# junejunejune/c_orb_slam

Measured on AMD Instinct MI355X. Metric: tracking FPS + ORB matches/sec, KITTI-00 stereo; local-BA iter/sec, higher is better.
Workload: dtype u8

## Files before the change

### c_orb_slam_amd/csrc/ba.hpp

```cpp
#pragma once
#include <functional>
#include <hip/hip_runtime.h>

#include <cstdint>
#include <future>
#include <vector>

#include "../../include/orbslam_gpu.h"
#include "ba_struct.hpp"
#include "ba_struct_gpu.hpp"
#include "ba_types.hpp"
#include "comm.hpp"
#include "ldlt.hpp"
#include "orb_common.hpp"

namespace orbgpu {

constexpr int kBaTiledMinPoses = 24;

struct Se3 {
    double q[4];
    double t[3];
    double pad;
};
// ... 16 lines not shown
    double ni, currentChi, iniChi;
    double trialChi[kLmTrials], trialLam[kLmTrials], solveIni[kLmSolves], solveChi[kLmSolves];
};

struct LinArgs;

class BaEngine {
public:
    ~BaEngine();
    int init();
    int run(const ba_problem* P, const volatile bool* stop, ba_result* R, Comm* comm = nullptr,
            const BaMode* mode = nullptr);
    const BaTrace& trace() const { return trace_; }
    double last_ms[4] = {0, 0, 0, 0};
    int last_dist[4] = {0, 0, 0, 0};
    int last_lm[4] = {0, 0, 0, 0};
    bool edgesGrouped = false;
    bool edgesValidated = false;

private:
    int upload_problem(const ba_problem* P);
    int build_structure(int level);
    int gather_blocks(const std::vector<int64_t>& mine, std::vector<int64_t>* all);
    int optimize(int iterations, const volatile bool* stop, int* its);
    int lm_solve(int iteration, const volatile bool* stop, bool* terminate);
    bool device_lm(int iterations) const;
    int optimize_device(int iterations, const volatile bool* stop, int* its);
    void enqueue_lm_step(bool first);
    int enqueue_lm_step_comm(bool first);
    int allreduce_tiles(int n);
    void launch_scale(double lam, int use_dev, int own, const int* gate);
    void launch_trial_errors(const LinArgs& sys, const int* gate);
    DensePlan dense_;
    bool small_struct() const;
    bool host_lists() const;
    bool smallUp_ = false;
    int32_t *dKp_ = nullptr, *dPtOrd_ = nullptr;
    int32_t* dSmKid_ = nullptr;
    uint8_t* dSmFx_ = nullptr;
    char* dSmallIn_ = nullptr;
    bool deferredUpload_ = false;
    std::vector<char> deferArgs_;
    size_t deferBytes_ = 0;
    int issue_upload();
    double* dLmStage_ = nullptr;
    size_t lmStageCap_ = 0;
    int gate_edges(int final_check, uint8_t* erase);
    int carve(bool commit, size_t* total);
    bool stopped(const volatile bool* stop) const { return comm_ ? stopRed_ : (stop && *stop); }
    int reduce_stop(const volatile bool* stop);
    bool sharded() const { return comm_ && comm_->size() > 1; }
    bool dense_solver(int n) const;

    hipStream_t stream_ = nullptr;
    int nkf_ = 0, npt_ = 0, ne_ = 0;
    Se3 *dT_ = nullptr, *dTbak_ = nullptr;
    double *dX_ = nullptr, *dXbak_ = nullptr;
    EdgeDev* dE_ = nullptr;
    uint8_t *dLevel_ = nullptr, *dRobust_ = nullptr;
    double* dErr_ = nullptr;
    std::vector<int32_t> kfId_, ptId_;
    const int32_t* ePt_ = nullptr;
    const int32_t* eKf_ = nullptr;
    std::vector<uint8_t> kfFixed_, kfLocal_, level_, ptHasEdge_, kfHasEdge_;
    BaStructDev st_{};
    BaHostStruct hs_;
    GpuStructBuilder gs_;
    uint8_t* dKfFixed_ = nullptr;
    int32_t *dKfId_ = nullptr, *dPtId_ = nullptr;
    int32_t* dStruct_ = nullptr;
    size_t dStructCap_ = 0;
    double *dTerms_ = nullptr, *dRc_ = nullptr, *dHpp_ = nullptr, *dBp_ = nullptr, *dHll_ = nullptr, *dBl_ = nullptr;
    double *dB_ = nullptr, *dX2_ = nullptr, *dS_ = nullptr, *dBs_ = nullptr, *dDinv_ = nullptr, *dDb_ = nullptr;
    double *dEmat_ = nullptr, *dCb_ = nullptr, *dScal_ = nullptr, *dScratch_ = nullptr, *dHplA_ = nullptr;
    int32_t* dPePos_ = nullptr;
    Se3* dTn_ = nullptr;
    double* dXn_ = nullptr;
    std::vector<int32_t> hPePos_;
    int blkChunks_ = 1;
    double *tmpA0_ = nullptr, *tmpA1_ = nullptr, *tmpB0_ = nullptr, *tmpB1_ = nullptr;
    unsigned* dCounter_ = nullptr;
    SparseLdlt sp_;
    std::future<int> spEarly_;
    int spEarlyNP_ = -1;
    std::vector<int64_t> spEarlyKeys_;
    int start_early_pose_graph();
    std::future<int> spBuild_;
    int join_sp_build();
    bool tiled_ = false;
    bool distOk_ = false;
    void* arena_ = nullptr;
    size_t arenaCap_ = 0;
    double* hScal_ = nullptr;
    LmDev* dLm_ = nullptr;
    int* hLm_ = nullptr;
    hipEvent_t lmEv_[2] = {nullptr, nullptr};
    void* hStage_ = nullptr;
    size_t hStageCap_ = 0;
    bool uploadPending_ = false;
    void* hStage2_ = nullptr;
    size_t hStage2Cap_ = 0;
    bool stage2Pending_ = false;
    int stage2_reserve(size_t bytes);
    int h2d_sync(void* dst, const void* src, size_t bytes);
    int d2h_sync(void* dst, const void* src, size_t bytes);
    int d2h_poll(void* dst, const void* src, size_t bytes);
    int poll_stream();
    BaHostStruct hs2_;
    bool hsValid_ = false, refineNext_ = false;
    int signalSeq_ = 0;
    int stage_reserve(size_t bytes);
    size_t scratchN_ = 0;
    size_t ldsMax_ = 0;
    Comm* comm_ = nullptr;
    bool stopRed_ = false;
    int nEglob_ = 0, nLglob_ = 0;
    int nTiles_ = 0;
    void* dPack_ = nullptr;
    size_t packCap_ = 0;
    int2* dTiles_ = nullptr;
    double* dPackBuf_ = nullptr;
    BaMode mode_{};
    double lambda_ = 0, ni_ = 2;
    int nBad_ = 0;
    BaTrace trace_;
};

struct PoseEdgeDev;
struct PoseProbDev;

struct PoseProbDev;
class PoseEngine {
public:
    ~PoseEngine();
    int init();
    int run(int count, const pose_problem* P, float* Tcw_out, uint8_t* const* outlier, int* ninliers);
    int run_device(int count, const pose_problem* P, float* const* Tcw_out, uint8_t* const* outlier, int* ninliers);
    int run_frames_device(int count, const pose_frame* F, float* const* Tcw_out, uint8_t* const* outlier,
                          int* ninliers, hipStream_t s = nullptr, DeferredChain* chain = nullptr);
    hipStream_t stream() const { return stream_; }
    void set_timing(bool on) { timing_ = on; }
    int last_timing(float* ms);

private:
    int launch_device(int count, const int* Ns, const std::function<void(int, PoseProbDev&)>& fill,
                      float* const* Tcw_out, uint8_t* const* outlier, int* ninliers, hipStream_t s = nullptr,
                      DeferredChain* chain = nullptr);
    hipStream_t stream_ = nullptr;
    void* dArena_ = nullptr;
    void* hArena_ = nullptr;
    size_t cap_ = 0;
    hipEvent_t lastUse_ = nullptr;
    bool lastUseSet_ = false;
    bool timing_ = false, timed_ = false;
    hipEvent_t tA_ = nullptr, tB_ = nullptr;
};

int debug_ldlt(int n, const double* S, const double* b, double* x, int variant);
int debug_csum(const double* v, int n, double* out);
int debug_ldlt_factor(int n, const double* S, double* out);
int debug_wave_tree(const double* v64, double* out);
int debug_shared_div(const double* a, const double* b, int n, double* out);
int debug_set_csum_lds_max(int v);
int debug_set_scale_small_max(int v);
int debug_set_struct_gpu_min_edges(int v);
int debug_set_posegraph_check(int on);
int debug_prof(unsigned long long* out32);

}
```

### c_orb_slam_amd/csrc/capi_match.cpp

```cpp
#include <cstring>
#include <new>
#include <vector>

#include "capi_handles.hpp"

using orbgpu::FrameDev;
using orbgpu::Matcher;
using orbgpu::SearchDev;


namespace {

size_t al(size_t n) { return (n + 255) & ~(size_t)255; }

template <class T>
T* up(Matcher* m, const T* src, size_t count, hipStream_t s, int* err) {
    if (!src || count == 0) return nullptr;
    void* d = m->arena_alloc(count * sizeof(T));
    if (!d || hipMemcpyAsync(d, src, count * sizeof(T), hipMemcpyHostToDevice, s) != hipSuccess) {
        *err = ORB_E_HIP;
        return nullptr;
    }
    return (T*)d;
}

size_t frame_bytes(const orb_frame* f) {
    if (!f) return 0;
    return al((size_t)f->N * 28) + al((size_t)f->N * 32) + (f->uRight ? al((size_t)f->N * 4) : 0) +
           al((size_t)f->nlevels * 4) + al(64);
}

FrameDev frame_dev(Matcher* m, const orb_frame* f, bool dev, hipStream_t s, int* err) {
    FrameDev d;
    memset(&d, 0, sizeof(d));
    if (!f) return d;
    d.N = f->N;
    d.minX = f->minX; d.maxX = f->maxX; d.minY = f->minY; d.maxY = f->maxY;
    d.gridWInv = f->gridWInv; d.gridHInv = f->gridHInv;
    d.nlevels = f->nlevels;
    d.fx = f->fx; d.fy = f->fy; d.cx = f->cx; d.cy = f->cy; d.bf = f->bf; d.b = f->b;
    if (dev) {
        d.keysUn = (const orbgpu::orb_kp_dev*)f->keysUn;
        d.desc = f->desc;
        d.uRight = f->uRight;
        d.scale = f->scaleFactors;
        d.Tcw = f->Tcw;
    } else {
        d.keysUn = (const orbgpu::orb_kp_dev*)up(m, f->keysUn, (size_t)f->N, s, err);
        d.desc = up(m, f->desc, (size_t)f->N * 32, s, err);
        d.uRight = up(m, f->uRight, f->uRight ? (size_t)f->N : 0, s, err);
        d.scale = up(m, f->scaleFactors, (size_t)f->nlevels, s, err);
        d.Tcw = up(m, f->Tcw, 16, s, err);
    }
    return d;
}

bool frame_ok(const orb_frame* f) {
    return f && f->N >= 0 && f->N <= orbgpu::kMaxFrameKeys && (f->N == 0 || (f->keysUn && f->desc)) &&
           f->scaleFactors && f->Tcw && f->nlevels > 0;
}

}

extern "C" {

int ORBmatcher_create(float nnratio, int checkOri, ORBmatcher_h* out) {
    if (!out) return ORB_E_INVALID;
    *out = nullptr;
    auto* m = new (std::nothrow) Matcher(nnratio, checkOri != 0);
    if (!m) return ORB_E_INVALID;
    int rc = m->init_device();
    if (rc) {
        delete m;
        return rc == -4 ? ORB_E_NODEVICE : ORB_E_HIP;
    }
    *out = new ORBmatcher_t{m};
    return ORB_OK;
}

int ORBmatcher_destroy(ORBmatcher_h h) {
    if (!h) return ORB_E_INVALID;
    delete h->m;
    delete h;
    return ORB_OK;
}

int ORBmatcher_set_device_pointers(ORBmatcher_h h, int on) {
    if (!h) return ORB_E_INVALID;
    h->m->set_device_pointers(on != 0);
    return ORB_OK;
}

void* ORBmatcher_stream(ORBmatcher_h h) { return h ? (void*)h->m->stream() : nullptr; }

int ORBmatcher_enable_timing(ORBmatcher_h h, int on) {
    if (!h) return ORB_E_INVALID;
    return h->m->set_timing(on != 0) ? ORB_E_HIP : ORB_OK;
}

int ORBmatcher_set_deferred(ORBmatcher_h h, int on) {
    if (!h || !h->m->device_pointers()) return ORB_E_INVALID;
    if (!on && h->m->chain().on() && h->m->chain().finish(h->m->stream())) return ORB_E_HIP;
    h->m->chain().set(on != 0);
    return ORB_OK;
}

int ORBmatcher_finish(ORBmatcher_h h) {
    if (!h) return ORB_E_INVALID;
    return h->m->chain().finish(h->m->stream()) ? ORB_E_HIP : ORB_OK;
}

int ORBmatcher_chain_close(ORBmatcher_h h, long long* epoch) {
    if (!h || !epoch || !h->m->chain().on()) return ORB_E_INVALID;
    return h->m->chain().close(h->m->stream(), epoch) ? ORB_E_HIP : ORB_OK;
}

int ORBmatcher_chain_wait(ORBmatcher_h h, long long epoch) {
    if (!h) return ORB_E_INVALID;
    return h->m->chain().wait(epoch) ? ORB_E_HIP : ORB_OK;
}

int ORBmatcher_chain_finish(ORBmatcher_h h, long long epoch) {
    if (!h) return ORB_E_INVALID;
    return h->m->chain().finish_upto(epoch) ? ORB_E_HIP : ORB_OK;
}

int ORBmatcher_last_timings(ORBmatcher_h h, float* ms8, long long* counts8) {
    if (!h || !ms8 || !counts8) return ORB_E_INVALID;
    return h->m->timings(ms8, counts8) ? ORB_E_HIP : ORB_OK;
}

int ORBmatcher_DescriptorDistance(const uint8_t* a, const uint8_t* b) {
    if (!a || !b) return ORB_E_INVALID;
    int dist = 0;
    for (int i = 0; i < 8; i++) {
        uint32_t pa, pb;
        memcpy(&pa, a + 4 * i, 4);
        memcpy(&pb, b + 4 * i, 4);
        dist += __builtin_popcount(pa ^ pb);
    }
    return dist;
}

int ORBmatcher_SearchByProjection_LastFrame_batch(ORBmatcher_h h, int npairs, const orb_frame* cur,
                                                  int32_t* const* cur_mp, const orb_frame* last,
                                                  const orb_kp* const* last_keys, const int32_t* const* last_mp,
                                                  const uint8_t* const* last_outlier, const orb_mappoints* mps,
                                                  float th, int bMono, int* nmatches) {
    if (!h || npairs < 0 || !cur || !cur_mp || !last || !last_keys || !last_mp || !last_outlier || !mps || !nmatches)
        return ORB_E_INVALID;
    Matcher* m = h->m;
    const bool dev = m->device_pointers();
    hipStream_t s = m->stream();
    for (int p = 0; p < npairs; p++) {
        if (!frame_ok(&cur[p]) || !last[p].Tcw || last[p].N < 0 || (last[p].N > 0 && !last[p].keysUn)) return ORB_E_INVALID;
        if (last[p].N > 0 && (!last_keys[p] || !last_mp[p] || !last_outlier[p])) return ORB_E_INVALID;
        if (mps[p].n > 0 && (!mps[p].pos || !mps[p].desc || !mps[p].observations)) return ORB_E_INVALID;
        if (!dev) {
            for (int i = 0; i < last[p].N; i++)
                if (last_mp[p][i] >= mps[p].n) return ORB_E_INVALID;
            for (int i = 0; i < cur[p].N; i++)
                if (cur_mp[p][i] >= mps[p].n) return ORB_E_INVALID;
        }
    }
    int err = 0;
    std::vector<SearchDev> probs(npairs);
    if (!dev) {
        size_t need = 0;
        for (int p = 0; p < npairs; p++) {
            const int nl = last[p].N;
            need += frame_bytes(&cur[p]) + al((size_t)nl * 28) * 2 + al(64) + al((size_t)nl * 4) + al((size_t)nl) +
                    al((size_t)mps[p].n * 12) + al((size_t)mps[p].n * 32) + al((size_t)mps[p].n * 4) +
                    al((size_t)cur[p].N * 4) + al(4);
        }
        if (m->arena_reserve(need + (size_t)npairs * 4 + 4096)) return ORB_E_HIP;
    }
    if (dev && m->arena_reserve((size_t)npairs * 4 + 256)) return ORB_E_HIP;
    int* d_nm = nullptr;
    std::vector<int*> nm_dev(npairs, nullptr);
    for (int p = 0; p < npairs; p++) {
        SearchDev& P = probs[p];
        memset(&P, 0, sizeof(P));
        P.cur = frame_dev(m, &cur[p], dev, s, &err);
        const int nl = last[p].N;
        P.nq = nl;
        P.last.N = nl;
        if (dev) {
            P.last.keysUn = (const orbgpu::orb_kp_dev*)last[p].keysUn;
            P.last.Tcw = last[p].Tcw;
            P.lastKeys = (const orbgpu::orb_kp_dev*)last_keys[p];
            P.lastMP = last_mp[p];
            P.lastOutlier = last_outlier[p];
            P.mpPos = mps[p].pos;
            P.mpDesc = mps[p].desc;
            P.mpObs = mps[p].observations;
            P.curMP = cur_mp[p];
        } else {
            P.last.keysUn = (const orbgpu::orb_kp_dev*)up(m, last[p].keysUn, (size_t)nl, s, &err);
            P.last.Tcw = up(m, last[p].Tcw, 16, s, &err);
            P.lastKeys = (const orbgpu::orb_kp_dev*)up(m, last_keys[p], (size_t)nl, s, &err);
            P.lastMP = up(m, last_mp[p], (size_t)nl, s, &err);
            P.lastOutlier = up(m, last_outlier[p], (size_t)nl, s, &err);
            P.mpPos = up(m, mps[p].pos, (size_t)mps[p].n * 3, s, &err);
            P.mpDesc = up(m, mps[p].desc, (size_t)mps[p].n * 32, s, &err);
            P.mpObs = up(m, mps[p].observations, (size_t)mps[p].n, s, &err);
            P.curMP = (int*)m->arena_alloc((size_t)cur[p].N * 4 + 4);
            if (cur[p].N > 0 && hipMemcpyAsync(P.curMP, cur_mp[p], (size_t)cur[p].N * 4, hipMemcpyHostToDevice, s) != hipSuccess)
                err = ORB_E_HIP;
        }
        nm_dev[p] = nullptr;
    }
    if (err) return err;
    {
        void* d = dev ? m->count_buf((size_t)npairs * 4 + 4) : m->arena_alloc((size_t)npairs * 4 + 4);
        if (!d) return ORB_E_HIP;
        d_nm = (int*)d;
        for (int p = 0; p < npairs; p++) probs[p].nmatches = d_nm + p;
    }
    int rc = m->search_last(probs, th, bMono != 0);
    if (rc) return rc == -1 ? ORB_E_INVALID : ORB_E_HIP;
    if (dev) {
        if (m->d2h_counts(nmatches, d_nm, (size_t)npairs * 4)) return ORB_E_HIP;
        return m->end_call() ? ORB_E_HIP : ORB_OK;
    }
    if (hipMemcpyAsync(nmatches, d_nm, (size_t)npairs * 4, hipMemcpyDeviceToHost, s) != hipSuccess) return ORB_E_HIP;
    {
        for (int p = 0; p < npairs; p++)
            if (cur[p].N > 0 &&
                hipMemcpyAsync(cur_mp[p], probs[p].curMP, (size_t)cur[p].N * 4, hipMemcpyDeviceToHost, s) != hipSuccess)
                return ORB_E_HIP;
    }
    if (orbgpu::stream_wait(s) != hipSuccess) return ORB_E_HIP;
    return ORB_OK;
}

int ORBmatcher_SearchByProjection_LastFrame(ORBmatcher_h h, const orb_frame* cur, int32_t* cur_mp,
                                            const orb_frame* last, const orb_kp* last_keys, const int32_t* last_mp,
                                            const uint8_t* last_outlier, const orb_mappoints* mps, float th, int bMono,
                                            int* nmatches) {
    return ORBmatcher_SearchByProjection_LastFrame_batch(h, 1, cur, &cur_mp, last, &last_keys, &last_mp, &last_outlier,
                                                         mps, th, bMono, nmatches);
}

int ORBmatcher_SearchByProjection_MapPoints(ORBmatcher_h h, const orb_frame* F, int32_t* cur_mp, int n,
                                            const uint8_t* track_in_view, const float* proj_x, const float* proj_xr,
                                            const float* proj_y, const int32_t* level, const float* view_cos,
                                            const int32_t* mp_index, const orb_mappoints* mps, float th,
                                            int* nmatches) {
    if (!h || !frame_ok(F) || !cur_mp || n < 0 || !mps || !nmatches) return ORB_E_INVALID;
    if (n > 0 && (!track_in_view || !proj_x || !proj_xr || !proj_y || !level || !view_cos || !mp_index))
        return ORB_E_INVALID;
    Matcher* m = h->m;
    const bool dev = m->device_pointers();
    hipStream_t s = m->stream();
    if (!dev) {
        for (int j = 0; j < n; j++)
            if (track_in_view[j] && (mp_index[j] < 0 || mp_index[j] >= mps->n || level[j] < 0 || level[j] >= F->nlevels))
                return ORB_E_INVALID;
        for (int i = 0; i < F->N; i++)
            if (cur_mp[i] >= mps->n) return ORB_E_INVALID;
        size_t need = frame_bytes(F) + al((size_t)n) + 4 * al((size_t)n * 4) + al((size_t)n * 4) * 2 +
                      al((size_t)mps->n * 12) + al((size_t)mps->n * 32) + al((size_t)mps->n * 4) +
                      al((size_t)F->N * 4) + al(8);
        if (m->arena_reserve(need + 4096)) return ORB_E_HIP;
    } else {
        if (m->arena_reserve(4096)) return ORB_E_HIP;
    }
    int err = 0;
    std::vector<SearchDev> probs(1);
    SearchDev& P = probs[0];
    memset(&P, 0, sizeof(P));
    P.cur = frame_dev(m, F, dev, s, &err);
    P.nq = n;
    if (dev) {
        P.inView = track_in_view; P.projX = proj_x; P.projXR = proj_xr; P.projY = proj_y;
        P.level = level; P.viewCos = view_cos; P.mpIndex = mp_index;
        P.mpPos = mps->pos; P.mpDesc = mps->desc; P.mpObs = mps->observations;
        P.curMP = cur_mp;
    } else {
        P.inView = up(m, track_in_view, (size_t)n, s, &err);
        P.projX = up(m, proj_x, (size_t)n, s, &err);
        P.projXR = up(m, proj_xr, (size_t)n, s, &err);
        P.projY = up(m, proj_y, (size_t)n, s, &err);
        P.level = up(m, level, (size_t)n, s, &err);
        P.viewCos = up(m, view_cos, (size_t)n, s, &err);
        P.mpIndex = up(m, mp_index, (size_t)n, s, &err);
        P.mpPos = up(m, mps->pos, (size_t)mps->n * 3, s, &err);
        P.mpDesc = up(m, mps->desc, (size_t)mps->n * 32, s, &err);
        P.mpObs = up(m, mps->observations, (size_t)mps->n, s, &err);
        P.curMP = (int*)m->arena_alloc((size_t)F->N * 4 + 4);
        if (F->N > 0 && hipMemcpyAsync(P.curMP, cur_mp, (size_t)F->N * 4, hipMemcpyHostToDevice, s) != hipSuccess)
            err = ORB_E_HIP;
    }
    if (err) return err;
    int* d_nm = (int*)m->arena_alloc(8);
    P.nmatches = d_nm;
    int rc = m->search_local(probs, th);
    if (rc) return rc == -1 ? ORB_E_INVALID : ORB_E_HIP;
    if (hipMemcpyAsync(nmatches, d_nm, 4, hipMemcpyDeviceToHost, s) != hipSuccess) return ORB_E_HIP;
    if (!dev && F->N > 0 && hipMemcpyAsync(cur_mp, P.curMP, (size_t)F->N * 4, hipMemcpyDeviceToHost, s) != hipSuccess)
        return ORB_E_HIP;
    if (orbgpu::stream_wait(s) != hipSuccess) return ORB_E_HIP;
    return ORB_OK;
}

int Frame_isInFrustum_batch(ORBmatcher_h h, int count, const orb_frame* F, const orb_localmap* maps,
                            float viewingCosLimit, float logScaleFactor, uint8_t* const* in_view,
                            float* const* proj_x, float* const* proj_xr, float* const* proj_y, int32_t* const* level,
                            float* const* view_cos, int* nvisible) {
    if (!h || count < 0 || (count > 0 && (!F || !maps || !in_view || !proj_x || !proj_xr || !proj_y || !level ||
                                          !view_cos || !nvisible)))
        return ORB_E_INVALID;
    if (count == 0) return ORB_OK;
    Matcher* m = h->m;
    if (!m->device_pointers()) return ORB_E_INVALID;
    hipStream_t s = m->stream();
    size_t need = al((size_t)count * 4) + al(sizeof(orbgpu::FrustumDev) * count) + 4096;
    for (int p = 0; p < count; p++) {
        const orb_localmap& M = maps[p];
        if (!frame_ok(&F[p]) || !F[p].Tcw || M.n < 0) return ORB_E_INVALID;
        if (M.n > 0 && (!M.pos || !M.max_dist || !M.min_dist || !M.normal || !M.skip || !in_view[p] || !proj_x[p] ||
                        !proj_xr[p] || !proj_y[p] || !level[p] || !view_cos[p]))
            return ORB_E_INVALID;
        need += al((size_t)M.n * 4);
    }
    if (m->arena_reserve(need)) return ORB_E_HIP;
    int err = 0;
    int* d_nv = (int*)m->arena_alloc((size_t)count * 4);
    if (!d_nv || hipMemsetAsync(d_nv, 0, (size_t)count * 4, s) != hipSuccess) return ORB_E_HIP;
    std::vector<SearchDev> probs(count);
    std::vector<orbgpu::FrustumDev> fr(count);
    for (int p = 0; p < count; p++) {
        SearchDev& P = probs[p];
        memset(&P, 0, sizeof(P));
        P.cur = frame_dev(m, &F[p], true, s, &err);
        P.nq = maps[p].n;
        P.mpPos = maps[p].pos;
        orbgpu::FrustumDev& f = fr[p];
        f.maxDist = maps[p].max_dist;
        f.minDist = maps[p].min_dist;
        f.normal = maps[p].normal;
        f.skip = maps[p].skip;
        f.inView = in_view[p];
        f.projX = proj_x[p];
        f.projXR = proj_xr[p];
        f.projY = proj_y[p];
        f.level = level[p];
        f.viewCos = view_cos[p];
        f.mpIndex = (int*)m->arena_alloc((size_t)std::max(maps[p].n, 1) * 4);
        f.nvisible = d_nv + p;
        if (!f.mpIndex) return ORB_E_HIP;
    }
    if (err) return err;
    if (m->frustum(probs, fr, viewingCosLimit, logScaleFactor)) return ORB_E_HIP;
    if (hipMemcpyAsync(nvisible, d_nv, (size_t)count * 4, hipMemcpyDeviceToHost, s) != hipSuccess) return ORB_E_HIP;
    return orbgpu::stream_wait(s) == hipSuccess ? ORB_OK : ORB_E_HIP;
}

int ORBmatcher_SearchLocalPoints_batch(ORBmatcher_h h, int count, const orb_frame* F, int32_t* const* cur_mp,
                                       const orb_localmap* maps, float logScaleFactor, float th, float nnratio,
                                       int* nmatches, int* nvisible) {
    if (!h || count < 0 || (count > 0 && (!F || !cur_mp || !maps || !nmatches || !nvisible))) return ORB_E_INVALID;
    if (count == 0) return ORB_OK;
    Matcher* m = h->m;
    if (!m->device_pointers()) return ORB_E_INVALID;
    hipStream_t s = m->stream();
    size_t need = al((size_t)count * 8) + al(sizeof(orbgpu::FrustumDev) * count) + 4096;
    for (int p = 0; p < count; p++) {
        const orb_localmap& M = maps[p];
        if (!frame_ok(&F[p]) || !F[p].Tcw || M.n < 0 || !cur_mp[p]) return ORB_E_INVALID;
        if (M.n > 0 && (!M.pos || !M.desc || !M.observations || !M.max_dist || !M.min_dist || !M.normal || !M.skip))
            return ORB_E_INVALID;
        need += 7 * al((size_t)M.n * 4) + 256;
    }
    if (m->arena_reserve(need)) return ORB_E_HIP;
    int err = 0;
    int* d_cnt = (int*)m->count_buf((size_t)count * 8);
    if (!d_cnt) return ORB_E_HIP;
    if (hipMemsetAsync(d_cnt, 0, (size_t)count * 8, s) != hipSuccess) return ORB_E_HIP;
    std::vector<SearchDev> probs(count);
    std::vector<orbgpu::FrustumDev> fr(count);
    for (int p = 0; p < count; p++) {
        SearchDev& P = probs[p];
        memset(&P, 0, sizeof(P));
        P.cur = frame_dev(m, &F[p], true, s, &err);
        P.nq = maps[p].n;
        P.mpPos = maps[p].pos;
        P.mpDesc = maps[p].desc;
        P.mpObs = maps[p].observations;
        P.curMP = cur_mp[p];
        P.nmatches = d_cnt + p;
        orbgpu::FrustumDev& f = fr[p];
        memset(&f, 0, sizeof(f));
        f.maxDist = maps[p].max_dist;
        f.minDist = maps[p].min_dist;
        f.normal = maps[p].normal;
        f.skip = maps[p].skip;
        f.nvisible = d_cnt + count + p;
    }
    if (err) return err;
    const int rc = m->search_local_points(probs, fr, 0.5f, logScaleFactor, th, nnratio > 0.f ? nnratio : m->nnratio());
    if (rc) return rc == -1 ? ORB_E_INVALID : ORB_E_HIP;
    if (m->d2h_counts(nmatches, d_cnt, (size_t)count * 4) || m->d2h_counts(nvisible, d_cnt + count, (size_t)count * 4))
        return ORB_E_HIP;
    (void)s;
    return m->end_call() ? ORB_E_HIP : ORB_OK;
}

int ORBmatcher_SearchDense_batch(ORBmatcher_h h, int count, const uint8_t* const* qdesc, const int* nq,
                                 const uint8_t* const* tdesc, const int* nt, int32_t* const* best_idx,
                                 int32_t* const* best_dist, int32_t* const* second_dist) {
    if (!h || count < 0 || (count > 0 && (!qdesc || !nq || !tdesc || !nt || !best_idx || !best_dist || !second_dist)))
        return ORB_E_INVALID;
    for (int p = 0; p < count; p++) {
        if (nq[p] < 0 || nt[p] < 0) return ORB_E_INVALID;
        if (nq[p] > 0 && (!qdesc[p] || !best_idx[p] || !best_dist[p] || !second_dist[p])) return ORB_E_INVALID;
        if (nt[p] > 0 && !tdesc[p]) return ORB_E_INVALID;
    }
    if (count == 0) return ORB_OK;
    Matcher* m = h->m;
    const bool dev = m->device_pointers();
    hipStream_t s = m->stream();
    std::vector<orbgpu::DenseDev> probs;
    if (!dev) {
        size_t need = 4096;
        for (int p = 0; p < count; p++) need += al((size_t)nq[p] * 32) + al((size_t)nt[p] * 32) + 3 * al((size_t)nq[p] * 4);
        if (m->arena_reserve(need)) return ORB_E_HIP;
    }
    int err = 0;
    for (int p = 0; p < count; p++) {
        if (nq[p] == 0) continue;
        orbgpu::DenseDev d;
        d.nq = nq[p];
        d.nt = nt[p];
        if (dev) {
            d.q = qdesc[p];
            d.t = tdesc[p];
            d.best_idx = best_idx[p];
            d.best_dist = best_dist[p];
            d.second_dist = second_dist[p];
        } else {
            d.q = up(m, qdesc[p], (size_t)nq[p] * 32, s, &err);
            d.t = nt[p] ? up(m, tdesc[p], (size_t)nt[p] * 32, s, &err) : nullptr;
            d.best_idx = (int*)m->arena_alloc((size_t)nq[p] * 4);
            d.best_dist = (int*)m->arena_alloc((size_t)nq[p] * 4);
            d.second_dist = (int*)m->arena_alloc((size_t)nq[p] * 4);
            if (!d.best_idx || !d.best_dist || !d.second_dist) err = ORB_E_HIP;
        }
        probs.push_back(d);
    }
    if (err) return err;
    if (m->dense(probs)) return ORB_E_HIP;
    if (dev) return m->end_call() ? ORB_E_HIP : ORB_OK;
    for (int p = 0, k = 0; p < count; p++) {
        if (nq[p] == 0) continue;
        const orbgpu::DenseDev& d = probs[k++];
        if (hipMemcpyAsync(best_idx[p], d.best_idx, (size_t)nq[p] * 4, hipMemcpyDeviceToHost, s) != hipSuccess ||
            hipMemcpyAsync(best_dist[p], d.best_dist, (size_t)nq[p] * 4, hipMemcpyDeviceToHost, s) != hipSuccess ||
            hipMemcpyAsync(second_dist[p], d.second_dist, (size_t)nq[p] * 4, hipMemcpyDeviceToHost, s) != hipSuccess)
            return ORB_E_HIP;
    }
    return orbgpu::stream_wait(s) == hipSuccess ? ORB_OK : ORB_E_HIP;
}

int ORBmatcher_last_dense_timing(ORBmatcher_h h, float* ms, long long* pairs) {
    if (!h || !ms || !pairs) return ORB_E_INVALID;
    return h->m->dense_timing(ms, pairs) ? ORB_E_HIP : ORB_OK;
}

int ORBmatcher_SearchCandidates(ORBmatcher_h h, const uint8_t* qdesc, int nq, const uint8_t* tdesc, int nt,
                                const int32_t* off, const int32_t* cand, int32_t* dist, int32_t* best_idx,
                                int32_t* best_dist, int32_t* second_dist) {
    if (!h || nq < 0 || nt < 0 || !off) return ORB_E_INVALID;
    if (nq == 0) return ORB_OK;
    if (!qdesc || !best_idx || !best_dist || !second_dist) return ORB_E_INVALID;
    Matcher* m = h->m;
    const bool dev = m->device_pointers();
    hipStream_t s = m->stream();
    if (dev) {
        int rc = m->candidates(qdesc, nq, tdesc, nt, off, cand, dist, best_idx, best_dist, second_dist);
        if (rc) return ORB_E_HIP;
        return orbgpu::stream_wait(s) == hipSuccess ? ORB_OK : ORB_E_HIP;
    }
    const int ncand = off[nq];
    if (off[0] != 0 || ncand < 0) return ORB_E_INVALID;
    for (int q = 0; q < nq; q++)
        if (off[q + 1] < off[q]) return ORB_E_INVALID;
    for (int k = 0; k < ncand; k++)
        if (cand[k] < 0 || cand[k] >= nt) return ORB_E_INVALID;
    size_t need = al((size_t)nq * 32) + al((size_t)nt * 32) + al((size_t)(nq + 1) * 4) + 2 * al((size_t)ncand * 4 + 4) +
                  3 * al((size_t)nq * 4);
    if (m->arena_reserve(need + 4096)) return ORB_E_HIP;
    int err = 0;
    const uint8_t* dq = up(m, qdesc, (size_t)nq * 32, s, &err);
    const uint8_t* dt = up(m, tdesc, (size_t)nt * 32, s, &err);
    const int* doff = up(m, off, (size_t)nq + 1, s, &err);
    const int* dc = up(m, cand, (size_t)ncand, s, &err);
    int* dd = (int*)m->arena_alloc((size_t)ncand * 4 + 4);
    int* dbi = (int*)m->arena_alloc((size_t)nq * 4);
    int* dbd = (int*)m->arena_alloc((size_t)nq * 4);
    int* dsd = (int*)m->arena_alloc((size_t)nq * 4);
    if (err || !dd || !dbi || !dbd || !dsd) return ORB_E_HIP;
    if (m->candidates(dq, nq, dt, nt, doff, dc, dd, dbi, dbd, dsd)) return ORB_E_HIP;
    if (dist && ncand > 0 && hipMemcpyAsync(dist, dd, (size_t)ncand * 4, hipMemcpyDeviceToHost, s) != hipSuccess)
        return ORB_E_HIP;
    if (hipMemcpyAsync(best_idx, dbi, (size_t)nq * 4, hipMemcpyDeviceToHost, s) != hipSuccess ||
        hipMemcpyAsync(best_dist, dbd, (size_t)nq * 4, hipMemcpyDeviceToHost, s) != hipSuccess ||
        hipMemcpyAsync(second_dist, dsd, (size_t)nq * 4, hipMemcpyDeviceToHost, s) != hipSuccess)
        return ORB_E_HIP;
    return orbgpu::stream_wait(s) == hipSuccess ? ORB_OK : ORB_E_HIP;
}

}
```

### c_orb_slam_amd/csrc/capi_stereo.cpp

```cpp
#include <algorithm>
#include <cmath>
#include <cstring>
#include <vector>

#include "capi_handles.hpp"
#include "stereo.hpp"

namespace {
size_t al(size_t n) { return (n + 255) & ~(size_t)255; }

template <class T>
T* up(orbgpu::Matcher* m, const T* src, size_t count, hipStream_t s, int* err) {
    if (!src || count == 0) return nullptr;
    void* d = m->arena_alloc(count * sizeof(T));
    if (!d || hipMemcpyAsync(d, src, count * sizeof(T), hipMemcpyHostToDevice, s) != hipSuccess) {
        *err = ORB_E_HIP;
        return nullptr;
    }
    return (T*)d;
}
}

extern "C" {

int ORBmatcher_ComputeStereoMatches_batch(ORBmatcher_h h, ORBextractor_h left, ORBextractor_h right, int npairs,
                                          const int* NL, const orb_kp* const* keysL, const uint8_t* const* descL,
                                          const int* NR, const orb_kp* const* keysR,
                                          const uint8_t* const* descR, float mbf, float mb,
                                          float* const* uRight, float* const* depth, int* nmatches) {
    return ORBmatcher_ComputeStereoMatches_batch_at(h, left, 0, right, 0, npairs, NL, keysL, descL, NR, keysR, descR,
                                                    mbf, mb, uRight, depth, nmatches);
}

int ORBmatcher_ComputeStereoMatches_batch_at(ORBmatcher_h h, ORBextractor_h left, int first_left,
                                             ORBextractor_h right, int first_right, int npairs, const int* NL,
                                             const orb_kp* const* keysL, const uint8_t* const* descL, const int* NR,
                                             const orb_kp* const* keysR, const uint8_t* const* descR, float mbf,
                                             float mb, float* const* uRight, float* const* depth, int* nmatches) {
    if (!h || !left || !right || npairs < 0 || first_left < 0 || first_right < 0 || !NL || !keysL || !descL || !NR ||
        !keysR || !descR || !uRight || !depth || !nmatches)
        return ORB_E_INVALID;
    if (npairs == 0) return ORB_OK;
    const orbgpu::Extractor* EL = left->ex;
    const orbgpu::Extractor* ER = right->ex;
    if (!EL->pyramid_base() || !ER->pyramid_base() || first_left + npairs > EL->last_batch() ||
        first_right + npairs > ER->last_batch())
        return ORB_E_INVALID;
    const auto& LL = EL->levels();
    const auto& LR = ER->levels();
    if (LL.size() != LR.size() || (int)LL.size() > orbgpu::kStereoMaxLevels) return ORB_E_INVALID;
    for (size_t l = 0; l < LL.size(); l++)
        if (LL[l].w != LR[l].w || LL[l].h != LR[l].h || LL[l].pitch != LR[l].pitch || LL[l].off != LR[l].off)
            return ORB_E_INVALID;
    if (!(mb > 0.0f)) return ORB_E_INVALID;
    for (int p = 0; p < npairs; p++) {
        if (NL[p] < 0 || NR[p] < 0 || NL[p] > orbgpu::kStereoMaxKeys || NR[p] > 65535) return ORB_E_INVALID;
        if ((NL[p] && (!keysL[p] || !descL[p] || !uRight[p] || !depth[p])) || (NR[p] && (!keysR[p] || !descR[p])))
            return ORB_E_INVALID;
    }
    orbgpu::Matcher* m = h->m;
    const bool dev = m->device_pointers();
    hipStream_t s = m->stream();
    if (orbgpu::stream_wait(EL->stream()) != hipSuccess ||
        (ER != EL && orbgpu::stream_wait(ER->stream()) != hipSuccess))
        return ORB_E_HIP;
    orbgpu::StereoParams P;
    std::memset(&P, 0, sizeof(P));
    for (size_t l = 0; l < LL.size(); l++) {
        P.lv[l].off = (long long)LL[l].off;
        P.lv[l].pitch = LL[l].pitch;
        P.lv[l].w = LL[l].w;
        P.lv[l].h = LL[l].h;
        P.scale[l] = EL->scale()[l];
        P.invScale[l] = EL->inv_scale()[l];
    }
    P.mbf = mbf;
    P.mb = mb;
    P.rows0 = LL[0].h;
    if (P.rows0 > orbgpu::kStereoMaxRows) return ORB_E_INVALID;
    const int band = (int)std::ceil(4.0f * EL->scale()[LL.size() - 1]) + 3;
    size_t need = al(sizeof(orbgpu::StereoDev) * npairs) + al(4 * (size_t)npairs);
    int maxNL = 0;
    for (int p = 0; p < npairs; p++) {
        need += al(4 * (size_t)NL[p]) + al(4 * ((size_t)P.rows0 + 1)) + al(8 * (size_t)NR[p] * band + 8);
        if (!dev) need += al(28 * (size_t)NL[p]) + al(32 * (size_t)NL[p]) + al(28 * (size_t)NR[p]) +
                          al(32 * (size_t)NR[p]) + 2 * al(4 * (size_t)NL[p]);
        maxNL = std::max(maxNL, NL[p]);
    }
    if (m->arena_reserve(need + 4096)) return ORB_E_HIP;
    int err = 0;
    std::vector<orbgpu::StereoDev> probs(npairs);
    int* d_kept = (int*)(dev ? m->count_buf(4 * (size_t)npairs) : m->arena_alloc(4 * (size_t)npairs));
    for (int p = 0; p < npairs; p++) {
        orbgpu::StereoDev& S = probs[p];
        S.NL = NL[p];
        S.NR = NR[p];
        S.pyrL = EL->pyramid_base() + (size_t)(first_left + p) * EL->pyramid_image_bytes();
        S.pyrR = ER->pyramid_base() + (size_t)(first_right + p) * ER->pyramid_image_bytes();
        S.sad = (int*)m->arena_alloc(4 * (size_t)NL[p] + 4);
        S.rowStart = (int*)m->arena_alloc(4 * ((size_t)P.rows0 + 1));
        S.rowIdx = (int2*)m->arena_alloc(8 * (size_t)NR[p] * band + 8);
        if (!S.sad || !S.rowStart || !S.rowIdx) return ORB_E_HIP;
        S.kept = d_kept + p;
        if (dev) {
            S.kL = (const orbgpu::orb_kp_dev*)keysL[p];
            S.dL = descL[p];
            S.kR = (const orbgpu::orb_kp_dev*)keysR[p];
            S.dR = descR[p];
            S.uRight = uRight[p];
            S.depth = depth[p];
        } else {
            S.kL = (const orbgpu::orb_kp_dev*)up(m, keysL[p], (size_t)NL[p], s, &err);
            S.dL = up(m, descL[p], 32 * (size_t)NL[p], s, &err);
            S.kR = (const orbgpu::orb_kp_dev*)up(m, keysR[p], (size_t)NR[p], s, &err);
            S.dR = up(m, descR[p], 32 * (size_t)NR[p], s, &err);
            S.uRight = (float*)m->arena_alloc(4 * (size_t)NL[p] + 4);
            S.depth = (float*)m->arena_alloc(4 * (size_t)NL[p] + 4);
        }
    }
    if (err || !d_kept) return ORB_E_HIP;
    auto* d_probs = (orbgpu::StereoDev*)m->arena_alloc(sizeof(orbgpu::StereoDev) * npairs);
    if (!d_probs) return ORB_E_HIP;
    if (hipMemcpyAsync(d_probs, m->h2d_src(probs.data(), sizeof(orbgpu::StereoDev) * npairs),
                       sizeof(orbgpu::StereoDev) * npairs, hipMemcpyHostToDevice, s) != hipSuccess)
        return ORB_E_HIP;
    if (orbgpu::stereo_launch(d_probs, npairs, maxNL, P, s, m)) return ORB_E_HIP;
    if (dev) {
        if (m->d2h_counts(nmatches, d_kept, 4 * (size_t)npairs)) return ORB_E_HIP;
        return m->end_call() ? ORB_E_HIP : ORB_OK;
    }
    if (hipMemcpyAsync(nmatches, d_kept, 4 * (size_t)npairs, hipMemcpyDeviceToHost, s) != hipSuccess)
        return ORB_E_HIP;
    if (!dev)
        for (int p = 0; p < npairs; p++)
            if (NL[p] && (hipMemcpyAsync(uRight[p], probs[p].uRight, 4 * (size_t)NL[p], hipMemcpyDeviceToHost, s) !=
                              hipSuccess ||
                          hipMemcpyAsync(depth[p], probs[p].depth, 4 * (size_t)NL[p], hipMemcpyDeviceToHost, s) !=
                              hipSuccess))
                return ORB_E_HIP;
    return orbgpu::stream_wait(s) == hipSuccess ? ORB_OK : ORB_E_HIP;
}

int ORBmatcher_ComputeStereoMatches(ORBmatcher_h h, ORBextractor_h left, ORBextractor_h right, int index, int NL,
                                    const orb_kp* keysL, const uint8_t* descL, int NR, const orb_kp* keysR,
                                    const uint8_t* descR, float mbf, float mb, float* uRight, float* depth,
                                    int* nmatches) {
    if (!h || !left || !right || index < 0) return ORB_E_INVALID;
    if (index != 0) return ORB_E_INVALID;
    return ORBmatcher_ComputeStereoMatches_batch(h, left, right, 1, &NL, &keysL, &descL, &NR, &keysR, &descR, mbf,
                                                 mb, &uRight, &depth, nmatches);
}

int Frame_UnprojectStereo_batch_device(ORBmatcher_h h, int count, const orb_unproject* U) {
    if (!h || count < 0 || (count > 0 && !U)) return ORB_E_INVALID;
    if (count == 0) return ORB_OK;
    std::vector<orbgpu::UnprojDev> P((size_t)count);
    int maxN = 0;
    for (int f = 0; f < count; f++) {
        const orb_unproject& Q = U[f];
        if (Q.N < 0 || (Q.N > 0 && (!Q.keysUn || !Q.depth || !Q.Twc || !Q.x3D))) return ORB_E_INVALID;
        orbgpu::UnprojDev& d = P[f];
        d.N = Q.N;
        d.keys = (const orbgpu::orb_kp_dev*)Q.keysUn;
        d.depth = Q.depth;
        d.Twc = Q.Twc;
        d.fx = Q.fx; d.fy = Q.fy; d.cx = Q.cx; d.cy = Q.cy;
        d.invfx = 1.0f / Q.fx;
        d.invfy = 1.0f / Q.fy;
        d.x3D = Q.x3D;
        d.mp = Q.mp;
        maxN = std::max(maxN, Q.N);
    }
    (void)maxN;
    return orbgpu::unproject_batch(P.data(), count, h->m->stream()) ? ORB_E_HIP : ORB_OK;
}

static int fill_undist(const orb_undistort& q, orbgpu::UndistDev& d) {
    if (q.N < 0 || q.N > (1 << 24) || (q.N > 0 && (!q.keys || !q.keysUn))) return ORB_E_INVALID;
    if (q.ndist != 4 && q.ndist != 5 && q.ndist != 8) return ORB_E_INVALID;
    std::memset(&d, 0, sizeof(d));
    d.N = q.N;
    d.keys = (const orbgpu::orb_kp_dev*)q.keys;
    d.keysUn = (orbgpu::orb_kp_dev*)q.keysUn;
    d.has_dist = q.dist[0] != 0.0f;
    for (int i = 0; i < 9; i++) d.A[i] = (double)q.K[i];
    for (int i = 0; i < 8; i++) d.k[i] = i < q.ndist ? (double)q.dist[i] : 0.0;
    return ORB_OK;
}

int Frame_UndistortKeyPoints_batch(ORBmatcher_h h, int count, const orb_undistort* U) {
    if (!h || count < 0 || (count > 0 && !U)) return ORB_E_INVALID;
    if (count == 0) return ORB_OK;
    std::vector<orbgpu::UndistDev> P((size_t)count);
    for (int f = 0; f < count; f++)
        if (int e = fill_undist(U[f], P[f])) return e;
    hipStream_t s = h->m->stream();
    if (h->m->device_pointers()) return orbgpu::undistort_batch(P.data(), count, s) ? ORB_E_HIP : ORB_OK;
    size_t tot = 0;
    for (int f = 0; f < count; f++) tot += (size_t)P[f].N;
    if (tot == 0) return ORB_OK;
    void* d = nullptr;
    if (hipMalloc(&d, 2 * tot * sizeof(orb_kp)) != hipSuccess) return ORB_E_HIP;
    orbgpu::orb_kp_dev* dk = (orbgpu::orb_kp_dev*)d;
    int rc = ORB_OK;
    size_t o = 0;
    for (int f = 0; f < count && rc == ORB_OK; f++) {
        if (P[f].N && hipMemcpyAsync(dk + o, U[f].keys, P[f].N * sizeof(orb_kp), hipMemcpyHostToDevice, s) != hipSuccess)
            rc = ORB_E_HIP;
        P[f].keys = dk + o;
        P[f].keysUn = dk + tot + o;
        o += (size_t)P[f].N;
    }
    if (rc == ORB_OK && orbgpu::undistort_batch(P.data(), count, s)) rc = ORB_E_HIP;
    o = 0;
    for (int f = 0; f < count && rc == ORB_OK; f++) {
        if (P[f].N && hipMemcpyAsync(U[f].keysUn, dk + tot + o, P[f].N * sizeof(orb_kp), hipMemcpyDeviceToHost, s) !=
                          hipSuccess)
            rc = ORB_E_HIP;
        o += (size_t)P[f].N;
    }
    if (orbgpu::stream_wait(s) != hipSuccess) rc = ORB_E_HIP;
    (void)hipFree(d);
    return rc;
}

int Frame_UndistortKeyPoints(ORBmatcher_h h, const orb_undistort* U) {
    if (!h || !U) return ORB_E_INVALID;
    if (h->m->device_pointers()) {
        const int e = Frame_UndistortKeyPoints_batch(h, 1, U);
        if (e) return e;
        return orbgpu::stream_wait(h->m->stream()) == hipSuccess ? ORB_OK : ORB_E_HIP;
    }
    return Frame_UndistortKeyPoints_batch(h, 1, U);
}

int Frame_ComputeImageBounds(ORBmatcher_h h, int cols, int rows, const float* K, const float* dist, int ndist,
                             float* bounds) {
    if (!h || !K || !dist || !bounds || cols <= 0 || rows <= 0) return ORB_E_INVALID;
    if (ndist != 4 && ndist != 5 && ndist != 8) return ORB_E_INVALID;
    if (dist[0] != 0.0f) {
        orb_kp c[4];
        std::memset(c, 0, sizeof(c));
        c[1].x = (float)cols;
        c[2].y = (float)rows;
        c[3].x = (float)cols; c[3].y = (float)rows;
        orb_kp u[4];
        orb_undistort q;
        std::memset(&q, 0, sizeof(q));
        q.N = 4;
        q.keys = c;
        q.keysUn = u;
        std::memcpy(q.K, K, sizeof(q.K));
        for (int i = 0; i < ndist; i++) q.dist[i] = dist[i];
        q.ndist = ndist;
        const bool dev = h->m->device_pointers();
        h->m->set_device_pointers(false);
        const int e = Frame_UndistortKeyPoints_batch(h, 1, &q);
        h->m->set_device_pointers(dev);
        if (e) return e;
        bounds[0] = std::min(u[0].x, u[2].x);
        bounds[1] = std::max(u[1].x, u[3].x);
        bounds[2] = std::min(u[0].y, u[1].y);
        bounds[3] = std::max(u[2].y, u[3].y);
    } else {
        bounds[0] = 0.0f;
        bounds[1] = (float)cols;
        bounds[2] = 0.0f;
        bounds[3] = (float)rows;
    }
    bounds[4] = static_cast<float>(64) / static_cast<float>(bounds[1] - bounds[0]);
    bounds[5] = static_cast<float>(48) / static_cast<float>(bounds[3] - bounds[2]);
    return ORB_OK;
}

int MapPoint_CreateStereo_batch_device(ORBmatcher_h h, int count, const orb_newpoints* Q) {
    if (!h || count < 0 || (count > 0 && !Q)) return ORB_E_INVALID;
    if (count == 0) return ORB_OK;
    std::vector<orbgpu::UnprojDev> P((size_t)count);
    for (int f = 0; f < count; f++) {
        const orb_newpoints& q = Q[f];
        if (q.N < 0 || (q.N > 0 && (!q.keysUn || !q.depth || !q.Twc || !q.x3D || !q.row || !q.normal ||
                                    !q.max_dist || !q.min_dist || !q.scaleFactors || q.nlevels <= 0)))
            return ORB_E_INVALID;
        orbgpu::UnprojDev& d = P[f];
        std::memset(&d, 0, sizeof(d));
        d.N = q.N;
        d.keys = (const orbgpu::orb_kp_dev*)q.keysUn;
        d.depth = q.depth;
        d.Twc = q.Twc;
        d.fx = q.fx; d.fy = q.fy; d.cx = q.cx; d.cy = q.cy;
        d.invfx = 1.0f / q.fx;
        d.invfy = 1.0f / q.fy;
        d.x3D = q.x3D;
        d.mp = q.row;
        d.mp_base = q.row_base;
        d.normal = q.normal;
        d.maxDist = q.max_dist;
        d.minDist = q.min_dist;
        d.scale = q.scaleFactors;
        d.nlevels = q.nlevels;
    }
    return orbgpu::unproject_batch(P.data(), count, h->m->stream()) ? ORB_E_HIP : ORB_OK;
}

int Tracking_PrepareLocalSearch_batch_device(ORBmatcher_h h, int count, const orb_localprep* Q) {
    if (!h || count < 0 || (count > 0 && !Q)) return ORB_E_INVALID;
    if (count == 0) return ORB_OK;
    orbgpu::Matcher* m = h->m;
    std::vector<orbgpu::LocalPrepDev> P((size_t)count);
    for (int f = 0; f < count; f++) {
        const orb_localprep& q = Q[f];
        if (q.N < 0 || q.n < 0 || (q.N > 0 && (!q.cur_mp || !q.outlier)) || (q.n > 0 && (!q.row || !q.skip)))
            return ORB_E_INVALID;
        P[f] = orbgpu::LocalPrepDev{q.N, q.cur_mp, q.outlier, q.n, q.row, q.skip};
    }
    if (m->arena_reserve(sizeof(orbgpu::LocalPrepDev) * count + 256)) return ORB_E_HIP;
    void* d = m->arena_alloc(sizeof(orbgpu::LocalPrepDev) * count);
    hipStream_t s = m->stream();
    if (!d || hipMemcpyAsync(d, m->h2d_src(P.data(), sizeof(orbgpu::LocalPrepDev) * count),
                             sizeof(orbgpu::LocalPrepDev) * count, hipMemcpyHostToDevice, s) != hipSuccess)
        return ORB_E_HIP;
    if (orbgpu::local_prep_batch((const orbgpu::LocalPrepDev*)d, count, s)) return ORB_E_HIP;
    return m->end_call() ? ORB_E_HIP : ORB_OK;
}

}
```

### c_orb_slam_amd/csrc/octree.hip

```cpp
#include "octree.hpp"

#include <cstdlib>

namespace orbgpu {

constexpr int OCT_TMAX = 1024;
constexpr int kOctCellsMax = kOctKMax / 2;

struct OctShared {
    int16_t x0[2 * kOctNMax], y0[2 * kOctNMax], x1[2 * kOctNMax], y1[2 * kOctNMax];
    uint16_t cnt[2 * kOctNMax], seq[2 * kOctNMax], kbeg[2 * kOctNMax];
    int16_t prv[2 * kOctNMax], nxt[2 * kOctNMax];
    int ia[4 * kOctNMax];
    uint16_t vpos[4 * kOctNMax];
    uint16_t er[kOctNMax], eidx[kOctNMax];
    uint16_t vs[kOctNMax], vs2[kOctNMax];
    uint32_t sk[kOctNMax];
    uint16_t knode[kOctKMax], arena[kOctKMax];
    alignas(16) uint16_t tmp[kOctKMax];
    int wsum[OCT_TMAX / 64];
    int head, size, nfree, m, newm, seqctr, flag;
};

template <int T, class Flag, class Put>
// ... 331 lines not shown
                mm, [&](int j) { return (int)S.cnt[S.vs2[j]]; }, [&](int j, int ex) { S.er[j] = (uint16_t)ex; },
                S.wsum);
            auto owner = [&](int t) {
                int lo = 0, hi = mm - 1;
                while (lo < hi) {
                    const int mid = (lo + hi + 1) >> 1;
                    if ((int)S.er[mid] <= t) lo = mid;
                    else hi = mid - 1;
                }
                return lo;
            };
            for (int t = tid; t < tot; t += T) {
                const int j = owner(t), p = S.vs2[j], pos = S.kbeg[p] + (t - S.er[j]);
                const int k = arena[pos];
                const int q = oct_quadrant(S, p, src[k]);
                tmp[t] = (uint16_t)k;
                knode[t] = (uint16_t)(4 * j + q);
                atomicAdd(&S.ia[4 * j + q], 1);
            }
            __syncthreads();
            for (int j = tid; j < mm; j += T) {
                int start = S.kbeg[S.vs2[j]];
#pragma unroll
                for (int q = 0; q < 4; q++) {
                    S.vpos[4 * j + q] = (uint16_t)start;
                    start += S.ia[4 * j + q];
                    S.ia[4 * j + q] = 0;
                }
            }
            __syncthreads();
            for (int t = tid; t < tot; t += T) {
                const int v = knode[t];
                arena[S.vpos[v] + atomicAdd(&S.ia[v], 1)] = tmp[t];
            }
            __syncthreads();
            ORBGPU_PROF_MARK(4);
            if (tid == 0) {
                int head = S.head, size = S.size, nfree = S.nfree, seqctr = S.seqctr, newm = 0, flag = 0;
                for (int j = mm - 1; j >= 0; j--) {
                    const int p = S.vs2[j];
                    int c4[4];
#pragma unroll
                    for (int q = 0; q < 4; q++) c4[q] = S.ia[4 * j + q];
                    for (int q = 0; q < 4; q++) {
                        const int c = c4[q];
                        if (c > 0) {
                            const int id = nfree++;
                            if (nfree > 2 * kOctNMax || id == cur) {
                                flag = 1;
                                break;
                            }
                            int a0, b0, a1, b1;
                            oct_child_rect(S, p, q, a0, b0, a1, b1);
                            S.x0[id] = (int16_t)a0;
                            S.y0[id] = (int16_t)b0;
                            S.x1[id] = (int16_t)a1;
                            S.y1[id] = (int16_t)b1;
                            S.cnt[id] = (uint16_t)c;
                            S.seq[id] = (uint16_t)(seqctr++);
                            S.kbeg[id] = S.vpos[4 * j + q];
                            S.prv[id] = -1;
                            S.nxt[id] = (int16_t)head;
                            if (head >= 0) S.prv[head] = (int16_t)id;
                            head = id;
                            size++;
                            if (c > 1) S.vs[newm++] = (uint16_t)id;
                        }
                    }
                    if (flag) break;
                    const int pp = S.prv[p], pn = S.nxt[p];
                    if (pp >= 0) S.nxt[pp] = (int16_t)pn;
                    else head = pn;
                    if (pn >= 0) S.prv[pn] = (int16_t)pp;
                    S.prv[p] = -2;
                    size--;
                    if (size >= N) break;
                }
                S.head = head;
                S.size = size;
                S.nfree = nfree;
                S.seqctr = seqctr;
                S.newm = newm;
                S.flag = flag;
            }
            __syncthreads();
            ORBGPU_PROF_MARK(5);
            if (S.flag) {
                if (tid == 0) {
                    jobcnt[job] = 0;
                    atomicOr(err, 8);
                }
                return;
            }
            if (S.size >= N || S.size == prevSize) break;
            if (tid == 0) S.m = S.newm;
            __syncthreads();
        }
        const int n2 = S.nfree - nb;
        const int sz = oct_scan<T>(
            n2 + Sz,
            [&](int u) {
                const int id = u < n2 ? nb + n2 - 1 - u : cur + (u - n2);
                return S.prv[id] != -2;
            },
            [&](int u, int r) { S.vpos[r] = (uint16_t)(u < n2 ? nb + n2 - 1 - u : cur + (u - n2)); }, S.wsum);
        if (sz > jcap) {
            if (tid == 0) {
                jobcnt[job] = 0;
                atomicOr(err, 16);
            }
            return;
        }
        for (int i = tid; i < sz; i += T) {
            const int id = S.vpos[i];
            const int kb = S.kbeg[id], kc = S.cnt[id];
            for (int t = 0; t < kc; t++) tmp[kb + t] = (uint16_t)i;
            S.ia[i] = -1;
        }
        __syncthreads();
        for (int pos = tid; pos < n; pos += T) {
            const int k = arena[pos];
            atomicMax(&S.ia[tmp[pos]], oct_best_key(src[k], k));
        }
        __syncthreads();
        for (int i = tid; i < sz; i += T) {
            const int k = 0xffff - (S.ia[i] & 0xffff);
            jobsel[(size_t)job * jcap + i] = src[k];
        }
        if (tid == 0) jobcnt[job] = sz;
        ORBGPU_PROF_MARK(6);
        return;
    }
    if (Sz > jcap) {
        if (tid == 0) {
            jobcnt[job] = 0;
            atomicOr(err, 16);
        }
        return;
    }
    for (int i = tid; i < Sz; i += T) S.ia[i] = -1;
    __syncthreads();
    for (int k = tid; k < n; k += T) atomicMax(&S.ia[knode[k]], oct_best_key(src[k], k));
    __syncthreads();
    for (int i = tid; i < Sz; i += T) {
        const int k = 0xffff - (S.ia[i] & 0xffff);
        jobsel[(size_t)job * jcap + i] = src[k];
    }
    if (tid == 0) jobcnt[job] = Sz;
    ORBGPU_PROF_MARK(7);
}

__global__ void __launch_bounds__(64) k_sel_build(const uint32_t* __restrict__ jobsel, const int* __restrict__ jobcnt,
                                                  int nlevels, int jcap, int cap, int2* __restrict__ sel, int selcap,
                                                  int* __restrict__ nout, int* __restrict__ err) {
    const int b = blockIdx.x, lane = threadIdx.x;
    const int c = lane < nlevels ? jobcnt[b * nlevels + lane] : 0;
    int incl = c;
#pragma unroll
    for (int o = 1; o < 64; o <<= 1) {
        const int y = __shfl_up(incl, o, 64);
        if (lane >= o) incl += y;
    }
    const int total = __shfl(incl, 63, 64);
    if (lane == 0) {
        nout[b] = total;
        if (total > cap || total > selcap) atomicOr(err, 1);
    }
    if (total > cap || total > selcap) return;
    for (int l = 0; l < nlevels; l++) {
        const int cl = __shfl(c, l, 64), off = __shfl(incl - c, l, 64);
        const uint32_t* js = jobsel + (size_t)(b * nlevels + l) * jcap;
        for (int i = lane; i < cl; i += 64)
            sel[(size_t)b * selcap + off + i] = make_int2((int)js[i], (b << 20) | (l << 16) | (off + i));
    }
}

int octree_prof_read(unsigned long long* out16) {
#ifdef ORBGPU_PROF
    unsigned long long v[32];
    ORB_HIP_CHECK(hipMemcpyFromSymbol(v, HIP_SYMBOL(g_orbgpu_prof), sizeof(v)));
    for (int i = 0; i < 16; i++) out16[i] = v[i];
    unsigned long long z[32] = {};
    ORB_HIP_CHECK(hipMemcpyToSymbol(HIP_SYMBOL(g_orbgpu_prof), z, sizeof(z)));
    return 0;
#else
    (void)out16;
    return -1;
#endif
}

int octree_launch(const OctInput& in, int B, int nlevels, const OctLevelDev* lv, uint32_t* jobsel, int* jobcnt, int jcap,
                  uint16_t* gscratch, size_t gstride, int cap, int2* sel, int selcap, int* nout, int* err,
                  hipStream_t s) {
    static const int nt = [] {
        const char* e = getenv("ORBGPU_OCT_T");
        const int v = e ? atoi(e) : 512;
        return v == 256 || v == 1024 ? v : 512;
    }();
    if (nt == 1024)
        hipLaunchKernelGGL(k_octree<1024>, dim3(B * nlevels), dim3(1024), 0, s, in, nlevels, lv, jobsel, jobcnt,
                           jcap, gscratch, gstride, err);
    else if (nt == 512)
        hipLaunchKernelGGL(k_octree<512>, dim3(B * nlevels), dim3(512), 0, s, in, nlevels, lv, jobsel, jobcnt,
                           jcap, gscratch, gstride, err);
    else
        hipLaunchKernelGGL(k_octree<256>, dim3(B * nlevels), dim3(256), 0, s, in, nlevels, lv, jobsel, jobcnt,
                           jcap, gscratch, gstride, err);
    hipLaunchKernelGGL(k_sel_build, dim3(B), dim3(64), 0, s, (const uint32_t*)jobsel, (const int*)jobcnt, nlevels,
                       jcap, cap, sel, selcap, nout, err);
    ORB_HIP_CHECK(hipGetLastError());
    return 0;
}

}
```

### c_orb_slam_amd/csrc/octree.hpp

```cpp
#pragma once
#include <hip/hip_runtime.h>

#include <cstdint>

#include "orb_common.hpp"

namespace orbgpu {

constexpr int kOctNMax = 640;
constexpr int kOctKMax = 4096;

struct OctLevelDev {
    int minX, maxX, minY, maxY, N;
};

int octree_prof_read(unsigned long long* out16);

struct OctInput {
    const uint32_t* slots;
    size_t slots_per_image;
    const int* counts;
    const int* cell_slot;
    const int* lcb;
    int ncells;
    uint32_t* packed;
    int* g_total;
};

int octree_launch(const OctInput& in, int B, int nlevels, const OctLevelDev* lv, uint32_t* jobsel, int* jobcnt, int jcap,
                  uint16_t* gscratch, size_t gstride, int cap, int2* sel, int selcap, int* nout, int* err,
                  hipStream_t s);

}
```

### c_orb_slam_amd/csrc/orb_extract.hip

```cpp
#include "orb_extract.hpp"

#include <algorithm>
#include <atomic>
#include <chrono>
#include <cmath>
#include <cstring>
#include <thread>

namespace orbgpu {

__constant__ int8_t c_pattern[256 * 4];
__constant__ int8_t c_disc[2 * 1024];
__constant__ int c_ndisc;
__constant__ int c_umax[16];
__constant__ int c_gauss[7];

static const int8_t kPattern[256 * 4] = {
#include "brief_pattern.inc"
};

__device__ __forceinline__ int xcd_tile(int bid, int nb) { return (bid & 7) * (nb >> 3) + (bid >> 3); }
static inline unsigned grid8(int n) { return (unsigned)((n + 7) & ~7); }
constexpr int kFastSplitLevel = 3;

// ... 1353 lines not shown
            const LevelHost& D = levels_[l];
            auto refl = [](int p, int len) {
                if (len == 1) return 0;
                while (p < 0 || p >= len) p = p < 0 ? -p : 2 * len - p - 2;
                return p;
            };
          for (int v = 0; v < 2; v++) {
            ptile_begin_[v * (nlevels_ + 1) + l] = (int)ptiles_.size();
            auto make = [&](int py0, int px0, int nrow, PyrTile& t) {
                int r0 = 1 << 30, r1 = -1, c0 = 1 << 30, c1 = -1;
                for (int py = py0; py < std::min(py0 + nrow, D.ph); py++) {
                    const int y = refl(py - kEdge, dh);
                    r0 = std::min(r0, yr[2 * y]);
                    r1 = std::max(r1, yr[2 * y + 1]);
                }
                for (int px = px0; px < std::min(px0 + PT_W, D.pitch); px++) {
                    const int x = refl(px - kEdge, dw);
                    c0 = std::min(c0, xofs[x]);
                    c1 = std::max(c1, xofs[x] + 1);
                }
                t.py0 = py0; t.px0 = px0; t.nrow = std::min(nrow, D.ph - py0);
                t.sr0 = r0; t.nsr = r1 - r0 + 1;
                t.sc0 = (c0 + kEdge) & ~3;
                t.nsw = (c1 + kEdge - t.sc0) / 4 + 1;
                return (size_t)t.nsr * t.nsw * 4 <= (size_t)kPyrLdsMax;
            };
            int nrow = kPyrTileH[v];
            for (bool ok = false; !ok;) {
                ok = true;
                for (int py0 = 0; py0 < D.ph && ok; py0 += nrow)
                    for (int px0 = 0; px0 < D.pitch && ok; px0 += PT_W) {
                        PyrTile t;
                        ok = make(py0, px0, nrow, t);
                    }
                if (!ok && --nrow < 1) return -1;
            }
            size_t lds = 0;
            for (int py0 = 0; py0 < D.ph; py0 += nrow)
                for (int px0 = 0; px0 < D.pitch; px0 += PT_W) {
                    PyrTile t;
                    make(py0, px0, nrow, t);
                    if ((size_t)(t.sc0 + 4 * t.nsw) > (size_t)levels_[l - 1].pitch) return -1;
                    lds = std::max(lds, (size_t)t.nsr * t.nsw * 4);
                    ptiles_.push_back(t);
                }
            plds_[v * nlevels_ + l] = (int)lds;
            ptile_th_[v * nlevels_ + l] = nrow;
            ptile_n_[v * nlevels_ + l] = (int)ptiles_.size() - ptile_begin_[v * (nlevels_ + 1) + l];
          }
        }
        yrAll[l] = yr;
        xofsAll_[l] = xofs;
        xalAll_[l] = xal;
        tab_off_[l][0] = push(xofs.data(), xofs.size() * 4);
        tab_off_[l][1] = push(xal.data(), xal.size() * 2);
        tab_off_[l][2] = push(yr.data(), yr.size() * 4);
        tab_off_[l][3] = push(yb.data(), yb.size() * 2);
    }
    if (plan_chain(yrAll)) return -1;
    auto F = [](void*& p) { if (p) (void)hipFree(p); p = nullptr; };
    F(d_pyr_); F(d_blur_); F(d_slots_); F(d_counts_); F(d_cells_); F(d_tiles_); F(d_lcb_); F(d_work_); F(d_groups_);
    F(d_cellslot_);
    work_B_ = -1;
    F(d_packed_); F(d_hdr_); F(d_sel_); F(d_levels_); F(d_tabs_); F(d_ptiles_);
    const int B = maxB_;
    if (d_chain_) (void)hipFree(d_chain_);
    d_chain_ = nullptr;
    if (chain_) {
        ORB_HIP_CHECK(hipMalloc(&d_chain_, chainTab_.size()));
        ORB_HIP_CHECK(hipMemcpy(d_chain_, chainTab_.data(), chainTab_.size(), hipMemcpyHostToDevice));
    }
    ORB_HIP_CHECK(hipMalloc(&d_ptiles_, std::max<size_t>(ptiles_.size(), 1) * sizeof(PyrTile)));
    if (!ptiles_.empty())
        ORB_HIP_CHECK(hipMemcpy(d_ptiles_, ptiles_.data(), ptiles_.size() * sizeof(PyrTile), hipMemcpyHostToDevice));
    if (d_flowcnt_) (void)hipFree(d_flowcnt_);
    d_flowcnt_ = nullptr;
    for (int v = 0; v < 2; v++) {
        ptile_th_[v * nlevels_] = kPyrTileH[v];
        int nb = 0, lds = 0;
        for (int l = 0; l < nlevels_; l++) {
            nb += (levels_[l].ph + ptile_th_[v * nlevels_ + l] - 1) / ptile_th_[v * nlevels_ + l];
            lds = std::max(lds, plds_[v * nlevels_ + l]);
        }
        flowBands_[v] = nb;
        flowLds_[v] = lds;
    }
    ORB_HIP_CHECK(hipMalloc(&d_flowcnt_, (size_t)std::max(flowBands_[0], flowBands_[1]) * B * 4));
    ORB_HIP_CHECK(hipMalloc(&d_pyr_, img_bytes_ * B));
    ORB_HIP_CHECK(hipMalloc(&d_blur_, blur_bytes_ * B));
    ORB_HIP_CHECK(hipMemset(d_blur_, 0, blur_bytes_ * B));
    ORB_HIP_CHECK(hipMalloc(&d_slots_, slots_per_image_ * 4 * B));
    ORB_HIP_CHECK(hipMalloc(&d_counts_, cells_.size() * 4 * B));
    ORB_HIP_CHECK(hipMalloc(&d_cells_, cells_.size() * sizeof(CellDesc)));
    ORB_HIP_CHECK(hipMemcpy(d_cells_, cells_.data(), cells_.size() * sizeof(CellDesc), hipMemcpyHostToDevice));
    ORB_HIP_CHECK(hipMalloc(&d_groups_, groups_.size() * sizeof(CellGroup)));
    ORB_HIP_CHECK(hipMemcpy(d_groups_, groups_.data(), groups_.size() * sizeof(CellGroup), hipMemcpyHostToDevice));
    ORB_HIP_CHECK(hipMalloc(&d_tiles_, tiles_.size() * sizeof(BlurTile)));
    ORB_HIP_CHECK(hipMemcpy(d_tiles_, tiles_.data(), tiles_.size() * sizeof(BlurTile), hipMemcpyHostToDevice));
    {
        std::vector<int> cs(cells_.size());
        for (size_t c = 0; c < cells_.size(); c++) cs[c] = cells_[c].slot_off;
        ORB_HIP_CHECK(hipMalloc(&d_cellslot_, std::max<size_t>(cs.size(), 1) * 4));
        ORB_HIP_CHECK(hipMemcpy(d_cellslot_, cs.data(), cs.size() * 4, hipMemcpyHostToDevice));
    }
    ORB_HIP_CHECK(hipMalloc(&d_lcb_, level_cell_begin_.size() * 4));
    ORB_HIP_CHECK(hipMemcpy(d_lcb_, level_cell_begin_.data(), level_cell_begin_.size() * 4, hipMemcpyHostToDevice));
    if (slots_per_image_ * B > ((size_t)1 << 30)) return -1;
    packed_cap_ = (int)(slots_per_image_ * B);
    ORB_HIP_CHECK(hipMalloc(&d_packed_, (size_t)packed_cap_ * 4));
    ORB_HIP_CHECK(hipMalloc(&d_hdr_, (size_t)B * (nlevels_ + 2) * 4 + 64));
    d_gtotal_ = (int*)((char*)d_hdr_ + (size_t)B * (nlevels_ + 2) * 4);
    d_gtotal_alias_ = true;
    sel_cap_ = B * std::max(nfeatures_ * 2 + 64, 256);
    ORB_HIP_CHECK(hipMalloc(&d_sel_, (size_t)sel_cap_ * sizeof(int2)));
    std::vector<LevelDev> ld(nlevels_);
    for (int l = 0; l < nlevels_; l++) {
        ld[l].off = levels_[l].off;
        ld[l].pitch = levels_[l].pitch;
        ld[l].scale = scale_[l];
        ld[l].boff = levels_[l].boff;
        ld[l].bpitch = levels_[l].bpitch;
        ld[l].kp_size = (float)(int)(kPatch * scale_[l]);
    }
    if (nlevels_ > kMaxLevels) return -1;
    for (int l = 0; l < nlevels_; l++) levelArgs_.lv[l] = ld[l];
    ORB_HIP_CHECK(hipMalloc(&d_levels_, ld.size() * sizeof(LevelDev)));
    ORB_HIP_CHECK(hipMemcpy(d_levels_, ld.data(), ld.size() * sizeof(LevelDev), hipMemcpyHostToDevice));
    ORB_HIP_CHECK(hipMalloc(&d_tabs_, std::max<size_t>(tabs.size(), 16)));
    if (!tabs.empty()) ORB_HIP_CHECK(hipMemcpy(d_tabs_, tabs.data(), tabs.size(), hipMemcpyHostToDevice));
    F(d_jobsel_); F(d_jobcnt_); F(d_octlv_); F(d_gscr_); F(d_nout_);
    jcap_ = 0;
    std::vector<OctLevelDev> ol(nlevels_);
    for (int l = 0; l < nlevels_; l++) {
        ol[l].minX = kEdge - 3;
        ol[l].maxX = levels_[l].w - kEdge + 3;
        ol[l].minY = kEdge - 3;
        ol[l].maxY = levels_[l].h - kEdge + 3;
        ol[l].N = nPerLevel_[l];
        jcap_ = std::max(jcap_, nPerLevel_[l] + 8);
    }
    if (jcap_ > kOctNMax) return -1;
    selcap_ = jcap_ * nlevels_;
    ORB_HIP_CHECK(hipMalloc(&d_octlv_, ol.size() * sizeof(OctLevelDev)));
    ORB_HIP_CHECK(hipMemcpy(d_octlv_, ol.data(), ol.size() * sizeof(OctLevelDev), hipMemcpyHostToDevice));
    ORB_HIP_CHECK(hipMalloc(&d_jobsel_, (size_t)B * nlevels_ * jcap_ * 4));
    ORB_HIP_CHECK(hipMalloc(&d_jobcnt_, (size_t)B * nlevels_ * 4));
    ORB_HIP_CHECK(hipMalloc(&d_gscr_, (size_t)packed_cap_ * 3 * 2));
    ORB_HIP_CHECK(hipMalloc(&d_nout_, (size_t)(B + 1) * 4));
    ORB_HIP_CHECK(hipFree(d_sel_));
    d_sel_ = nullptr;
    sel_cap_ = selcap_ * B;
    ORB_HIP_CHECK(hipMalloc(&d_sel_, (size_t)sel_cap_ * sizeof(int2)));
    if (h_nout_) (void)hipHostFree(h_nout_);
    ORB_HIP_CHECK(hipHostMalloc((void**)&h_nout_, (size_t)(B + 1) * 4));
    geomW_ = W;
    geomH_ = H;
    return 0;
}

int Extractor::extract(const uint8_t* imgs, int B, int W, int H, int step, size_t img_stride,
                       bool imgs_on_device, orb_kp* kps, uint8_t* desc, int cap, bool out_on_device,
                       int* n_out, const uint8_t* const* list) {
    if (B <= 0 || B > maxB_ || W <= 0 || H <= 0) return -1;
    if (W > maxW_ || H > maxH_) return -1;
    if (int e = setup_geometry(W, H)) return e;
    hipStream_t s = stream_;
    const uint8_t* src = imgs;
    if (!imgs_on_device) {
        const size_t need = img_stride * (B - 1) + (size_t)step * (H - 1) + W;
        if (need > in_cap_) {
            if (d_in_) (void)hipFree(d_in_);
            ORB_HIP_CHECK(hipMalloc(&d_in_, need));
            in_cap_ = need;
        }
        if (h_in_) ORB_HIP_CHECK(hipEventSynchronize(ev_[0]));
        if (need > h_in_cap_) {
            if (h_in_) (void)hipHostFree(h_in_);
            h_in_ = nullptr;
            h_in_cap_ = 0;
            ORB_HIP_CHECK(hipHostMalloc(&h_in_, need));
            h_in_cap_ = need;
        }
        if (list) {
            const size_t one = (size_t)step * (H - 1) + W;
            for (int b = 0; b < B; b++) std::memcpy((uint8_t*)h_in_ + img_stride * b, list[b], one);
        } else {
            std::memcpy(h_in_, imgs, need);
        }
        ORB_HIP_CHECK(hipMemcpyAsync(d_in_, h_in_, need, hipMemcpyHostToDevice, s));
        src = (const uint8_t*)d_in_;
    }
    ORB_HIP_CHECK(hipEventRecord(ev_[0], s));
    const int ncells = (int)cells_.size();
    if (work_B_ != B && build_work(B)) return -2;
    const bool split = fastSplit_ && work_part_[0] > 0 && work_part_[1] > 0;
    {
        const LevelHost& L0 = levels_[0];
        const int n = (L0.pitch / 16) * L0.ph;
        const bool flow = flow_ && !split && !chain_;
        if (flow) {
            const int v = B >= 8 ? 1 : 0;
            ORB_HIP_CHECK(hipMemsetAsync(d_flowcnt_, 0, (size_t)flowBands_[v] * B * 4, s));
            const FlowArgs A = flow_args(v, B);
            int tasks = 0;
            for (int l = 0; l < nlevels_; l++) tasks += B * A.L[l].ntiles;
            auto kern = v ? k_pyr_flow<kPyrTileH[1]> : k_pyr_flow<kPyrTileH[0]>;
            hipLaunchKernelGGL(kern, dim3(tasks), dim3(256), flowLds_[v], s, src, img_stride, step, W, H,
                               (uint8_t*)d_pyr_, img_bytes_, A, (const PyrTile*)d_ptiles_, (const uint8_t*)d_tabs_,
                               d_flowcnt_, 1, d_gtotal_, (int*)d_nout_ + B);
        } else {
            hipLaunchKernelGGL(k_pyr_level0, dim3((n + 255) / 256, B), dim3(256), 0, s, src, img_stride, step, W, H,
                               (uint8_t*)d_pyr_, img_bytes_, L0.pitch, L0.ph, d_gtotal_, (int*)d_nout_ + B);
        }
        const int lend = flow ? 1 : chain_ && !split ? chainFrom_ : nlevels_;
        for (int l = 1; l < lend; l++) {
            if (split && l == kFastSplitLevel) {
                ORB_HIP_CHECK(hipEventRecord(evPyrA_, s));
                ORB_HIP_CHECK(hipStreamWaitEvent(side_, evPyrA_, 0));
                hipLaunchKernelGGL(k_fast_cells, dim3(work_part_[0]), dim3(256), 0, side_, (const uint8_t*)d_pyr_,
                                   img_bytes_, (const CellGroup*)d_groups_, iniTh_, minTh_, (uint32_t*)d_slots_,
                                   slots_per_image_, (int*)d_counts_, ncells, (const int*)d_work_);
                ORB_HIP_CHECK(hipEventRecord(evFastA_, side_));
            }
            const LevelHost& L = levels_[l];
            const LevelHost& P = levels_[l - 1];
            const uint8_t* T = (const uint8_t*)d_tabs_;
            const int v = B >= 8 ? 1 : 0, pb = v * (nlevels_ + 1) + l;
            const int nt = ptile_n_[v * nlevels_ + l];
            auto kern = v ? k_pyr_resize<kPyrTileH[1]> : k_pyr_resize<kPyrTileH[0]>;
            hipLaunchKernelGGL(kern, dim3(grid8(nt), B), dim3(256), plds_[v * nlevels_ + l], s, (uint8_t*)d_pyr_, img_bytes_,
                               P.off, P.pitch, L.off, L.pitch, L.ph, L.w, L.h,
                               (const int*)(T + tab_off_[l][0]), (const short2*)(T + tab_off_[l][1]),
                               (const int2*)(T + tab_off_[l][2]), (const short2*)(T + tab_off_[l][3]),
                               (const PyrTile*)d_ptiles_ + ptile_begin_[pb], nt);
        }
        if (!flow && lend < nlevels_) {
            const uint8_t* T = (const uint8_t*)d_chain_;
            const LevelHost& P = levels_[lend - 1];
            hipLaunchKernelGGL(k_pyr_chain, dim3(chainK_, B), dim3(256), chainLds_, s, (uint8_t*)d_pyr_, img_bytes_,
                               (long long)P.off, P.pitch, P.w, (const ChainLevel*)T, nlevels_ - lend,
                               (const int4*)(T + chainStripOff_), (const uint16_t*)(T + chainRowOff_),
                               (const uint8_t*)d_tabs_, chainSrcLds_, chainSrcRp_);
        }
    }
    ORB_HIP_CHECK(hipGetLastError());
    ORB_HIP_CHECK(hipEventRecord(ev_[1], s));
    static const bool blurEarly = [] {
        const char* e = getenv("ORBGPU_BLUR_EARLY");
        return e && e[0] == '1';
    }();
    if (blurEarly && !evBlur_)
        hipLaunchKernelGGL(k_blur7, dim3(grid8((int)tiles_.size()), B), dim3(256), 0, s, (const uint8_t*)d_pyr_,
                           (uint8_t*)d_blur_, img_bytes_, blur_bytes_, (const BlurTile*)d_tiles_, (int)tiles_.size());
    if (evBlur_) {
        ORB_HIP_CHECK(hipStreamWaitEvent(side_, ev_[1], 0));
        hipLaunchKernelGGL(k_blur7, dim3(grid8((int)tiles_.size()), B), dim3(256), 0, side_, (const uint8_t*)d_pyr_,
                           (uint8_t*)d_blur_, img_bytes_, blur_bytes_, (const BlurTile*)d_tiles_, (int)tiles_.size());
        ORB_HIP_CHECK(hipEventRecord(evBlur_, side_));
    }
    if (split) {
        hipLaunchKernelGGL(k_fast_cells, dim3(work_part_[1]), dim3(256), 0, s, (const uint8_t*)d_pyr_, img_bytes_,
                           (const CellGroup*)d_groups_, iniTh_, minTh_, (uint32_t*)d_slots_, slots_per_image_,
                           (int*)d_counts_, ncells, (const int*)d_work_ + work_part_[0]);
        ORB_HIP_CHECK(hipStreamWaitEvent(s, evFastA_, 0));
    } else {
        hipLaunchKernelGGL(k_fast_cells, dim3(work_n_), dim3(256), 0, s, (const uint8_t*)d_pyr_, img_bytes_,
                           (const CellGroup*)d_groups_, iniTh_, minTh_, (uint32_t*)d_slots_, slots_per_image_,
                           (int*)d_counts_, ncells, (const int*)d_work_);
    }
    ORB_HIP_CHECK(hipGetLastError());
    ORB_HIP_CHECK(hipEventRecord(ev_[3], s));
    ORB_HIP_CHECK(hipEventRecord(ev_[4], s));
    int* d_err = (int*)d_nout_ + B;
    OctInput oin{(const uint32_t*)d_slots_, slots_per_image_, (const int*)d_counts_, (const int*)d_cellslot_,
                 (const int*)d_lcb_, ncells, (uint32_t*)d_packed_, d_gtotal_};
    if (int e = octree_launch(oin, B, nlevels_, (const OctLevelDev*)d_octlv_, (uint32_t*)d_jobsel_, (int*)d_jobcnt_,
                              jcap_, (uint16_t*)d_gscr_, (size_t)packed_cap_, cap, (int2*)d_sel_, selcap_,
                              (int*)d_nout_, d_err, s))
        return e;
    ORB_HIP_CHECK(hipEventRecord(ev_[5], s));
    if (evBlur_)
        ORB_HIP_CHECK(hipStreamWaitEvent(s, evBlur_, 0));
    else if (!blurEarly)
        hipLaunchKernelGGL(k_blur7, dim3(grid8((int)tiles_.size()), B), dim3(256), 0, s, (const uint8_t*)d_pyr_,
                           (uint8_t*)d_blur_, img_bytes_, blur_bytes_, (const BlurTile*)d_tiles_, (int)tiles_.size());
    ORB_HIP_CHECK(hipEventRecord(ev_[2], s));
    orb_kp_dev* okps = (orb_kp_dev*)kps;
    uint8_t* odesc = desc;
    if (!out_on_device) {
        const size_t nk = (size_t)B * cap;
        if (nk > out_cap_) {
            if (d_kps_) (void)hipFree(d_kps_);
            if (d_desc_) (void)hipFree(d_desc_);
            ORB_HIP_CHECK(hipMalloc(&d_kps_, nk * sizeof(orb_kp_dev)));
            ORB_HIP_CHECK(hipMalloc(&d_desc_, nk * 32));
            out_cap_ = nk;
        }
        okps = (orb_kp_dev*)d_kps_;
        odesc = (uint8_t*)d_desc_;
    }
    {
        const int gx = (selcap_ + 3) / 4;
        const int nwg = B >= 8 ? gx * 8 * ((B + 7) / 8) : gx * B;
        hipLaunchKernelGGL(k_orient_desc, dim3(nwg), dim3(256), 0, s, (const uint8_t*)d_pyr_,
                           (const uint8_t*)d_blur_, img_bytes_, blur_bytes_, (const int2*)d_sel_, selcap_,
                           (const int*)d_nout_, levelArgs_, okps, odesc, cap, gx, B);
    }
    ORB_HIP_CHECK(hipGetLastError());
    ORB_HIP_CHECK(hipMemcpyAsync(h_nout_, d_nout_, (size_t)(B + 1) * 4, hipMemcpyDeviceToHost, s));
    ORB_HIP_CHECK(hipEventRecord(ev_[6], s));
    ORB_HIP_CHECK(stream_wait(s));
    const int err = h_nout_[B];
    for (int b = 0; b < B; b++) n_out[b] = h_nout_[b];
    if (err & 1) return -3;
    if (err) return -1;
    if (!out_on_device) {
        for (int b = 0; b < B; b++) {
            if (n_out[b] == 0) continue;
            ORB_HIP_CHECK(hipMemcpyAsync(kps + (size_t)b * cap, okps + (size_t)b * cap, (size_t)n_out[b] * sizeof(orb_kp_dev),
                                         hipMemcpyDeviceToHost, s));
            ORB_HIP_CHECK(hipMemcpyAsync(desc + (size_t)b * cap * 32, odesc + (size_t)b * cap * 32, (size_t)n_out[b] * 32,
                                         hipMemcpyDeviceToHost, s));
        }
        ORB_HIP_CHECK(stream_wait(s));
    }
    last_B_ = B;
    return 0;
}

int Extractor::corner_total(long long* total) {
    if (last_B_ <= 0 || !d_gtotal_) return -1;
    int v = 0;
    ORB_HIP_CHECK(hipStreamSynchronize(stream_));
    ORB_HIP_CHECK(hipMemcpy(&v, d_gtotal_, 4, hipMemcpyDeviceToHost));
    *total = v;
    return 0;
}

int Extractor::get_blurred(int index, int level, uint8_t* dst, int dst_step, int* w, int* h) {
    if (level < 0 || level >= nlevels_ || index < 0 || index >= last_B_ || !d_blur_) return -1;
    const LevelHost& L = levels_[level];
    *w = L.w;
    *h = L.h;
    if (!dst) return 0;
    ORB_HIP_CHECK(hipMemcpy2D(dst, dst_step, (const uint8_t*)d_blur_ + (size_t)index * blur_bytes_ + L.boff, L.bpitch,
                              L.w, L.h, hipMemcpyDeviceToHost));
    return 0;
}

int debug_prof_extract(unsigned long long* out32) {
#ifdef ORBGPU_PROF
    ORB_HIP_CHECK(hipMemcpyFromSymbol(out32, HIP_SYMBOL(g_orbgpu_prof), sizeof(unsigned long long) * 16));
    unsigned long long z[32] = {};
    ORB_HIP_CHECK(hipMemcpyToSymbol(HIP_SYMBOL(g_orbgpu_prof), z, sizeof(z)));
    return octree_prof_read(out32 + 16);
#else
    (void)out32;
    return -1;
#endif
}

int Extractor::timings(float* ms6) {
    float t[6] = {0};
    (void)hipEventElapsedTime(&t[0], ev_[0], ev_[1]);
    (void)hipEventElapsedTime(&t[1], ev_[5], ev_[2]);
    (void)hipEventElapsedTime(&t[2], ev_[1], ev_[3]);
    (void)hipEventElapsedTime(&t[3], ev_[3], ev_[4]);
    (void)hipEventElapsedTime(&t[4], ev_[4], ev_[5]);
    (void)hipEventElapsedTime(&t[5], ev_[2], ev_[6]);
    for (int i = 0; i < 6; i++) ms6[i] = t[i];
    return 0;
}

int Extractor::get_level(int index, int level, uint8_t* dst, int dst_step, int* w, int* h) {
    if (level < 0 || level >= nlevels_ || index < 0 || index >= last_B_ || !d_pyr_) return -1;
    const LevelHost& L = levels_[level];
    *w = L.w;
    *h = L.h;
    if (!dst) return 0;
    ORB_HIP_CHECK(hipMemcpy2D(dst, dst_step, (const uint8_t*)d_pyr_ + (size_t)index * img_bytes_ + L.off, L.pitch,
                              L.pw, L.ph, hipMemcpyDeviceToHost));
    return 0;
}

}
```

### c_orb_slam_amd/csrc/orb_extract.hpp

```cpp
#pragma once
#include <atomic>
#include <condition_variable>
#include <cstddef>
#include <cstdint>
#include <mutex>
#include <thread>
#include <vector>
#include <array>

#include "orb_common.hpp"
#include "octree.hpp"
#include "../../include/orbslam_gpu.h"

namespace orbgpu {

struct orb_kp_dev {
    float x, y, size, angle, response;
    int32_t octave, class_id;
};
static_assert(sizeof(orb_kp_dev) == 28, "cv::KeyPoint layout");

struct CellDesc {
    int r0, r1, c0, c1;
    int offx, offy;
    int pitch, cap, slot_off, level;
    long long lvl_off;
};

struct CellGroup {
    int r0, c0, rows, cols;
    int rsplit, csplit;
    int pitch, pad;
    long long lvl_off;
    int cell[4], cap[4], slot_off[4];
    int xadd[4], yadd[4];
};

struct BlurTile {
    long long off, boff;
    int pitch, bpitch, w, h, tx, ty;
};

constexpr int PT_W = 256, kPyrLdsMax = 48 * 1024;
struct PyrTile {
    int py0, px0, nrow, sr0, nsr, sc0, nsw, pad;
};

struct ChainLevel {
    long long off;
    int w, h, pitch, rp, lds, xofs, xal, yr, yb, nph;
};
constexpr int kChainLdsMax = 64 * 1024;

struct FlowLevel {
    long long off;
    int pitch, ph, w, h;
    int task0, ntiles;
    int tile0;
    int band0, th, ncol;
    int xofs, xal, yr, yb;
};
struct FlowArgs {
    FlowLevel L[16];
    int nl, nbands;
};

struct LevelDev {
    long long off, boff;
    int pitch, bpitch;
    float scale, kp_size;
};
constexpr int kMaxLevels = 16;
struct LevelArgs {
    LevelDev lv[kMaxLevels];
};

struct LevelHost {
    int w, h, pw, ph, pitch, bpitch;
    size_t off, boff;
};

class Extractor {
public:
    Extractor(int nfeatures, float scaleFactor, int nlevels, int iniTh, int minTh);
    ~Extractor();
    int init_device(int maxW, int maxH, int maxBatch);
    int extract(const uint8_t* imgs, int B, int W, int H, int step, size_t img_stride, bool imgs_on_device,
                orb_kp* kps, uint8_t* desc, int cap, bool out_on_device, int* n_out,
                const uint8_t* const* list = nullptr);
    int get_level(int index, int level, uint8_t* dst, int dst_step, int* w, int* h);
    int get_blurred(int index, int level, uint8_t* dst, int dst_step, int* w, int* h);
    int timings(float* ms6);
    int corner_total(long long* total);
    hipStream_t stream() const { return stream_; }
    int reserve_cus(int one_in_n);
    int share_stream(Extractor* with);
    int build_work(int B);
    const uint8_t* pyramid_base() const { return (const uint8_t*)d_pyr_; }
    size_t pyramid_image_bytes() const { return img_bytes_; }
    const std::vector<LevelHost>& levels() const { return levels_; }
    int last_batch() const { return last_B_; }

    int nlevels() const { return nlevels_; }
    float scale_factor() const { return scaleFactor_; }
    const std::vector<float>& scale() const { return scale_; }
    const std::vector<float>& inv_scale() const { return invScale_; }
    const std::vector<float>& sigma2() const { return sigma2_; }
    const std::vector<float>& inv_sigma2() const { return invSigma2_; }
    const std::vector<int>& n_per_level() const { return nPerLevel_; }

private:
    static void gaussian_taps(int taps[7]);
    int setup_geometry(int W, int H);
    void release();

    int nfeatures_;
    double scaleFactorD_;
    float scaleFactor_;
    int nlevels_, iniTh_, minTh_;
    std::vector<float> scale_, invScale_, sigma2_, invSigma2_;
    std::vector<int> nPerLevel_, umax_;

    int maxW_ = 0, maxH_ = 0, maxB_ = 0;
    int geomW_ = -1, geomH_ = -1;
    std::vector<LevelHost> levels_;
    LevelArgs levelArgs_{};
    std::vector<CellDesc> cells_;
    std::vector<CellGroup> groups_;
    std::vector<int> level_cell_begin_;
    std::vector<BlurTile> tiles_;
    std::vector<PyrTile> ptiles_;
    std::vector<int> ptile_begin_, ptile_n_, plds_;
    std::vector<int> ptile_th_;
    bool flow_ = false;
    int* d_flowcnt_ = nullptr;
    int flowBands_[2] = {0, 0}, flowLds_[2] = {0, 0};
    FlowArgs flow_args(int v, int B) const;
    int plan_chain(const std::vector<std::vector<int>>& yr);
    bool chain_ = false;
    int chainK_ = 0, chainLds_ = 0, chainFrom_ = 0, chainSrcLds_ = 0, chainSrcRp_ = 0;
    std::vector<std::vector<int>> xofsAll_;
    std::vector<std::vector<short>> xalAll_;
    size_t chainStripOff_ = 0, chainRowOff_ = 0;
    std::vector<uint8_t> chainTab_;
    void* d_chain_ = nullptr;
    void* d_cellslot_ = nullptr;
    std::vector<std::array<size_t, 4>> tab_off_;
    size_t img_bytes_ = 0, blur_bytes_ = 0, slots_per_image_ = 0;
    int packed_cap_ = 0, sel_cap_ = 0;
    int last_B_ = 0;

    hipStream_t stream_ = nullptr;
    bool ownStream_ = true;
    int lent_ = 0;
    hipEvent_t ev_[7] = {};
    hipStream_t side_ = nullptr;
    hipEvent_t evBlur_ = nullptr;
    bool fastSplit_ = false;
    hipEvent_t evPyrA_ = nullptr, evFastA_ = nullptr;
    void *d_in_ = nullptr, *d_pyr_ = nullptr, *d_blur_ = nullptr, *d_slots_ = nullptr, *d_counts_ = nullptr;
    void *d_ptiles_ = nullptr;
    void *d_cells_ = nullptr, *d_tiles_ = nullptr, *d_lcb_ = nullptr, *d_packed_ = nullptr, *d_hdr_ = nullptr;
    void *d_sel_ = nullptr, *d_levels_ = nullptr, *d_tabs_ = nullptr, *d_kps_ = nullptr, *d_desc_ = nullptr;
    int* d_gtotal_ = nullptr;
    void* d_work_ = nullptr;
    void* d_groups_ = nullptr;
    int work_B_ = -1, work_n_ = 0;
    int work_part_[2] = {0, 0};
    bool d_gtotal_alias_ = false;
    size_t in_cap_ = 0, out_cap_ = 0;
    void* h_in_ = nullptr;
    size_t h_in_cap_ = 0;
    void *d_jobsel_ = nullptr, *d_jobcnt_ = nullptr, *d_octlv_ = nullptr, *d_gscr_ = nullptr, *d_nout_ = nullptr;
    int jcap_ = 0, selcap_ = 0;
    int* h_nout_ = nullptr;

};

int debug_prof_extract(unsigned long long* out32);

}
```

### c_orb_slam_amd/csrc/orb_match.hip

```cpp
#define ORBGPU_PROF_BLOCK 20
#include "orb_match.hpp"

#include <chrono>
#include <cstdlib>

#include <cstring>

#include "detmath.hpp"

namespace orbgpu {

constexpr int TH_HIGH = 100;
constexpr int kSelectLocalThreads = 1024;
constexpr int HISTO_LENGTH = 30;

__device__ __forceinline__ int hamming32(const uint8_t* a, const uint8_t* b) {
    const uint4* pa = reinterpret_cast<const uint4*>(a);
    const uint4* pb = reinterpret_cast<const uint4*>(b);
    const uint4 a0 = pa[0], a1 = pa[1], b0 = pb[0], b1 = pb[1];
    return __popc(a0.x ^ b0.x) + __popc(a0.y ^ b0.y) + __popc(a0.z ^ b0.z) + __popc(a0.w ^ b0.w) +
           __popc(a1.x ^ b1.x) + __popc(a1.y ^ b1.y) + __popc(a1.z ^ b1.z) + __popc(a1.w ^ b1.w);
}

struct Desc32 {
// ... 605 lines not shown
        cnt[s] = -1;
        ch[s] = -1;
#pragma unroll
        for (int j = 0; j < 4; j++) tk[s][j] = 0u;
        if (qs[s] >= 0) {
            const int q = qs[s];
            const int c = P.qinfo[q].x;
            cnt[s] = c;
            if (c > 0) {
                if (obs_of(q)) obsm |= 1u << s;
                const int4* t4 = reinterpret_cast<const int4*>(P.topk + (size_t)q * kTopK);
                const int4 a = t4[0], b = t4[1];
                tk[s][0] = ((uint32_t)a.x << 16) | (uint32_t)a.y;
                tk[s][1] = ((uint32_t)a.z << 16) | (uint32_t)a.w;
                tk[s][2] = ((uint32_t)b.x << 16) | (uint32_t)b.y;
                tk[s][3] = ((uint32_t)b.z << 16) | (uint32_t)b.w;
            }
        }
    }
    __syncthreads();
    ORBGPU_PROF_MARK(LAST ? 0 : 8);
    constexpr int need = LAST ? 1 : 2;
    auto decide = [&](int s) -> int {
        const int q = qs[s];
        const int c = cnt[s];
        if (c <= 0) return -1;
        const int kk = c < kTopK ? c : kTopK;
        int bestDist = 256, bestIdx = -1, bestDist2 = 256, idx2 = -1, nfree = 0;
#pragma unroll
        for (int j = 0; j < 4; j++) {
            if (j < kk && nfree < need) {
                const int idx = (int)(tk[s][j] & 0xffffu), d = (int)(tk[s][j] >> 16);
                if (!(s_occ0[idx] != 0 || s_owner[idx] < q)) {
                    if (nfree == 0) { bestDist = d; bestIdx = idx; }
                    else { bestDist2 = d; idx2 = idx; }
                    nfree++;
                }
            }
        }
        if (nfree < need && kk > 4)
            return select_slow<LAST>(Pp, q, c, s_occ0, s_owner, s_oct, th, bF, bB, nnratio);
        if (bestDist > TH_HIGH) return -1;
        if (!LAST) {
            const int bestLevel = s_oct[bestIdx];
            const int bestLevel2 = idx2 >= 0 ? (int)s_oct[idx2] : -1;
            if (bestLevel == bestLevel2 && (float)bestDist > nnratio * (float)bestDist2) return -1;
        }
        return bestIdx;
    };
    auto decide_g = [&](int q) -> int {
        const int c = P.qinfo[q].x;
        return c > 0 ? select_slow<LAST>(Pp, q, c, s_occ0, s_owner, s_oct, th, bF, bB, nnratio) : -1;
    };
    for (int k = NT * Q + tid; k < nact; k += NT) {
        const int q = list ? list[k] : k;
        P.qinfo[q].z = (P.qinfo[q].x > 0 && obs_of(q)) ? 1 : 0;
        P.qinfo[q].y = decide_g(q);
    }
#pragma unroll
    for (int s = 0; s < Q; s++) ch[s] = decide(s);
    for (int round = 0; round <= nq; round++) {
        __syncthreads();
        for (int i = tid; i < N; i += NT) s_owner[i] = INT_MAX;
        if (tid == 0) s_changed = 0;
        __syncthreads();
#pragma unroll
        for (int s = 0; s < Q; s++)
            if (ch[s] >= 0 && ((obsm >> s) & 1u)) atomicMin(&s_owner[ch[s]], qs[s]);
        for (int k = NT * Q + tid; k < nact; k += NT) {
            const int q = list ? list[k] : k;
            const int4 qi = P.qinfo[q];
            if (qi.y >= 0 && qi.z) atomicMin(&s_owner[qi.y], q);
        }
        __syncthreads();
        bool chg = false;
#pragma unroll
        for (int s = 0; s < Q; s++) {
            const int c = decide(s);
            if (c != ch[s]) { ch[s] = c; chg = true; }
        }
        for (int k = NT * Q + tid; k < nact; k += NT) {
            const int q = list ? list[k] : k;
            const int c = decide_g(q);
            if (c != P.qinfo[q].y) { P.qinfo[q].y = c; chg = true; }
        }
        if (chg) s_changed = 1;
        __syncthreads();
        ORBGPU_PROF_COUNT(LAST ? 6 : 14);
        if (!s_changed) break;
    }
    ORBGPU_PROF_MARK(LAST ? 1 : 9);
    int nm = 0;
#pragma unroll
    for (int s = 0; s < Q; s++)
        if (ch[s] >= 0) { atomicMax(&s_lastq[ch[s]], qs[s]); nm++; }
    for (int k = NT * Q + tid; k < nact; k += NT) {
        const int q = list ? list[k] : k;
        const int c = P.qinfo[q].y;
        if (c >= 0) { atomicMax(&s_lastq[c], q); nm++; }
    }
    atomicAdd(&s_nm, nm);
    __syncthreads();
    if (LAST && checkOri) {
        int bins[Q];
#pragma unroll
        for (int s = 0; s < Q; s++) {
            bins[s] = -1;
            const int bi = ch[s];
            if (bi < 0) continue;
            float rot = P.last.keysUn[qs[s]].angle - P.cur.keysUn[bi].angle;
            if (rot < 0.0f) rot += 360.0f;
            int bin = (int)roundf(rot * (1.0f / HISTO_LENGTH));
            if (bin == HISTO_LENGTH) bin = 0;
            atomicAdd(&s_hsz[bin], 1);
            bins[s] = bin;
        }
        __syncthreads();
        if (tid == 0) {
            int max1 = 0, max2 = 0, max3 = 0, ind1 = -1, ind2 = -1, ind3 = -1;
            for (int i = 0; i < HISTO_LENGTH; i++) {
                const int sz = s_hsz[i];
                if (sz > max1) { max3 = max2; max2 = max1; max1 = sz; ind3 = ind2; ind2 = ind1; ind1 = i; }
                else if (sz > max2) { max3 = max2; max2 = sz; ind3 = ind2; ind2 = i; }
                else if (sz > max3) { max3 = sz; ind3 = i; }
            }
            if (max2 < 0.1f * (float)max1) { ind2 = -1; ind3 = -1; }
            else if (max3 < 0.1f * (float)max1) { ind3 = -1; }
            s_ind[0] = ind1;
            s_ind[1] = ind2;
            s_ind[2] = ind3;
        }
        __syncthreads();
        const int ind1 = s_ind[0], ind2 = s_ind[1], ind3 = s_ind[2];
        int removed = 0;
#pragma unroll
        for (int s = 0; s < Q; s++) {
            if (ch[s] < 0) continue;
            const int b = bins[s];
            if (b != ind1 && b != ind2 && b != ind3) {
                s_rm[ch[s]] = 1;
                removed++;
            }
        }
        atomicAdd(&s_rmcnt, removed);
    }
    __syncthreads();
    ORBGPU_PROF_MARK(LAST ? 2 : 10);
    for (int i = tid; i < N; i += NT) {
        const int lq = s_lastq[i];
        if (s_rm[i]) P.curMP[i] = -1;
        else if (lq >= 0) P.curMP[i] = LAST ? P.lastMP[lq] : P.mpIndex[lq];
    }
    if (tid == 0) *P.nmatches = s_nm - s_rmcnt;
    ORBGPU_PROF_MARK(LAST ? 3 : 11);
}

__global__ void __launch_bounds__(256) k_csr_hamming(const uint8_t* __restrict__ q, int nq, const uint8_t* __restrict__ t,
                                                     const int* __restrict__ off, const int* __restrict__ cand,
                                                     int* __restrict__ dist, int* __restrict__ best_idx,
                                                     int* __restrict__ best_dist, int* __restrict__ second_dist,
                                                     unsigned long long* counters) {
    const int lane = threadIdx.x & 63;
    const int qi = blockIdx.x * 4 + (threadIdx.x >> 6);
    if (qi >= nq) return;
    const int b = off[qi], e = off[qi + 1];
    const uint8_t* qd = q + 32 * (size_t)qi;
    unsigned long long k1 = ~0ull, k2 = ~0ull;
    for (int k = b + lane; k < e; k += 64) {
        const int d = hamming32(qd, t + 32 * (size_t)cand[k]);
        if (dist) dist[k] = d;
        const unsigned long long key = ((unsigned long long)d << 32) | (unsigned)(k - b);
        if (key < k1) { k2 = k1; k1 = key; }
        else if (key < k2) k2 = key;
    }
    for (int o = 32; o > 0; o >>= 1) {
        const unsigned long long o1 = __shfl_xor(k1, o, 64), o2 = __shfl_xor(k2, o, 64);
        const unsigned long long n1 = o1 < k1 ? o1 : k1;
        const unsigned long long hi = o1 < k1 ? k1 : o1;
        unsigned long long n2 = o2 < k2 ? o2 : k2;
        n2 = hi < n2 ? hi : n2;
        k1 = n1;
        k2 = n2;
    }
    if (lane == 0) {
        if (counters) {
            const int sl = blockIdx.x & (kCountSlots - 1);
            atomicAdd(&counters[4 * kCountSlots + sl], (unsigned long long)(e - b));
            atomicAdd(&counters[5 * kCountSlots + sl], 1ull);
        }
        best_idx[qi] = k1 == ~0ull ? -1 : cand[b + (int)(k1 & 0xffffffffu)];
        best_dist[qi] = k1 == ~0ull ? 256 : (int)(k1 >> 32);
        second_dist[qi] = k2 == ~0ull ? 256 : (int)(k2 >> 32);
    }
}

constexpr int kDenseBlock = 256;
constexpr int kDenseQ = 256;

struct DenseJob {
    int prob, q0, t0, part;
};

template <int TB>
__global__ void __launch_bounds__(kDenseQ) k_dense_hamming(const DenseDev* __restrict__ probs,
                                                           const DenseJob* __restrict__ jobs,
                                                           unsigned long long* __restrict__ part,
                                                           unsigned long long* counters) {
    __shared__ uint4 tl[TB * 2];
    const DenseJob J = jobs[blockIdx.x];
    const DenseDev P = probs[J.prob];
    const int tid = threadIdx.x;
    const int nt = min(TB, P.nt - J.t0);
    const uint4* src = reinterpret_cast<const uint4*>(P.t + 32 * (size_t)J.t0);
    for (int k = tid; k < 2 * nt; k += kDenseQ) tl[k] = src[k];
    const int qi = J.q0 + tid;
    uint4 a0 = make_uint4(0, 0, 0, 0), a1 = a0;
    if (qi < P.nq) {
        a0 = reinterpret_cast<const uint4*>(P.q + 32 * (size_t)qi)[0];
        a1 = reinterpret_cast<const uint4*>(P.q + 32 * (size_t)qi)[1];
    }
    __syncthreads();
    unsigned b1 = 0xffffffffu, b2 = 0xffffffffu;
    auto dist = [&](const uint4& t0, const uint4& t1) {
        return __popc(a0.x ^ t0.x) + __popc(a0.y ^ t0.y) + __popc(a0.z ^ t0.z) + __popc(a0.w ^ t0.w) +
               __popc(a1.x ^ t1.x) + __popc(a1.y ^ t1.y) + __popc(a1.z ^ t1.z) + __popc(a1.w ^ t1.w);
    };
    auto take = [&](unsigned key) {
        b2 = min(b2, max(b1, key));
        b1 = min(b1, key);
    };
    int j = 0;
    for (; j + 4 <= nt; j += 4) {
        const uint4 t0 = tl[2 * j], t1 = tl[2 * j + 1], t2 = tl[2 * j + 2], t3 = tl[2 * j + 3];
        const uint4 t4 = tl[2 * j + 4], t5 = tl[2 * j + 5], t6 = tl[2 * j + 6], t7 = tl[2 * j + 7];
        const unsigned d0 = dist(t0, t1), d1 = dist(t2, t3), d2 = dist(t4, t5), d3 = dist(t6, t7);
        take((d0 << 16) | (unsigned)j);
        take((d1 << 16) | (unsigned)(j + 1));
        take((d2 << 16) | (unsigned)(j + 2));
        take((d3 << 16) | (unsigned)(j + 3));
    }
    for (; j < nt; j++) take((dist(tl[2 * j], tl[2 * j + 1]) << 16) | (unsigned)j);
    if (qi < P.nq) {
        unsigned long long* o = part + 2 * ((size_t)J.part * kDenseQ + tid);
        o[0] = b1 == 0xffffffffu ? ~0ull : ((unsigned long long)(b1 >> 16) << 32) | (unsigned)(J.t0 + (int)(b1 & 0xffffu));
        o[1] = b2 == 0xffffffffu ? ~0ull : ((unsigned long long)(b2 >> 16) << 32) | 0xffffffffu;
    }
    if (counters && tid == 0) {
        const int sl = blockIdx.x & (kCountSlots - 1);
        atomicAdd(&counters[6 * kCountSlots + sl], (unsigned long long)nt * (unsigned long long)min(kDenseQ, P.nq - J.q0));
    }
}

__global__ void __launch_bounds__(256) k_dense_merge(const DenseDev* __restrict__ probs, const int* __restrict__ qjob,
                                                     const DenseJob* __restrict__ jobs, int nblk_per_q,
                                                     const unsigned long long* __restrict__ part, int nq_blocks,
                                                     int njobs) {
    const int g = blockIdx.x * blockDim.x + threadIdx.x;
    const int qb = g / kDenseQ, tq = g % kDenseQ;
    if (qb >= nq_blocks) return;
    const DenseJob J0 = jobs[qjob[qb]];
    const DenseDev P = probs[J0.prob];
    const int qi = J0.q0 + tq;
    if (qi >= P.nq) return;
    unsigned long long k1 = ~0ull, k2 = ~0ull;
    for (int b = 0; b < nblk_per_q && qjob[qb] + b < njobs; b++) {
        const DenseJob J = jobs[qjob[qb] + b];
        if (J.prob != J0.prob || J.q0 != J0.q0) break;
        const unsigned long long* o = part + 2 * ((size_t)J.part * kDenseQ + tq);
        const unsigned long long o1 = o[0], o2 = o[1];
        const unsigned long long n1 = o1 < k1 ? o1 : k1, hi = o1 < k1 ? k1 : o1;
        unsigned long long n2 = o2 < k2 ? o2 : k2;
        n2 = hi < n2 ? hi : n2;
        k1 = n1;
        k2 = n2;
    }
    P.best_idx[qi] = k1 == ~0ull ? -1 : (int)(k1 & 0xffffffffu);
    P.best_dist[qi] = k1 == ~0ull ? 256 : (int)(k1 >> 32);
    P.second_dist[qi] = k2 == ~0ull ? 256 : (int)(k2 >> 32);
}

__global__ void __launch_bounds__(256) k_area_count(const SearchDev* __restrict__ probs, const AreaQuery* __restrict__ q,
                                                    int nq, int* __restrict__ cnt) {
    const int i = blockIdx.x * blockDim.x + threadIdx.x;
    if (i >= nq) return;
    const AreaQuery a = q[i];
    int c = 0;
    if (a.qd >= 0) {
        QueryWin w{a.x, a.y, a.r, a.minLevel, a.maxLevel};
        for_features_in_area(probs[0], w, [&](int) { c++; });
    }
    cnt[i] = c;
}

__global__ void __launch_bounds__(256) k_area_fill(const SearchDev* __restrict__ probs, const AreaQuery* __restrict__ q,
                                                   int nq, const uint8_t* __restrict__ qdesc, const int* __restrict__ off,
                                                   int2* __restrict__ out) {
    const int i = blockIdx.x * blockDim.x + threadIdx.x;
    if (i >= nq) return;
    const AreaQuery a = q[i];
    if (a.qd < 0) return;
    const SearchDev& P = probs[0];
    const uint8_t* d0 = qdesc + 32 * (size_t)a.qd;
    int k = off[i];
    QueryWin w{a.x, a.y, a.r, a.minLevel, a.maxLevel};
    for_features_in_area(P, w, [&](int idx) { out[k++] = make_int2(idx, hamming32(d0, P.cur.desc + 32 * (size_t)idx)); });
}

int Matcher::area_candidates(const SearchDev& frame, const AreaQuery* d_q, int nq, const uint8_t* d_qdesc,
                             std::vector<int>& off, std::vector<int2>& cand) {
    off.assign((size_t)nq + 1, 0);
    cand.clear();
    if (frame.cur.N > kMaxFrameKeys || frame.cur.N < 0) return -1;
    const size_t grid = ((size_t)(kGridCells + 1 + frame.cur.N) * 4 + 255) & ~(size_t)255;
    const size_t need = grid + 2 * (((size_t)nq + 1) * 4 + 256) + sizeof(SearchDev) + 256;
    if (need > scratch_cap_) {
        if (d_scratch_) (void)hipFree(d_scratch_);
        scratch_cap_ = need * 2;
        ORB_HIP_CHECK(hipMalloc(&d_scratch_, scratch_cap_));
    }
    char* s = (char*)d_scratch_;
    SearchDev P = frame;
    P.gridStart = (int*)s;
    P.gridIdx = P.gridStart + kGridCells + 1;
    s += grid;
    int* d_cnt = (int*)s;
    s += (((size_t)nq + 1) * 4 + 255) & ~(size_t)255;
    int* d_off = (int*)s;
    s += (((size_t)nq + 1) * 4 + 255) & ~(size_t)255;
    SearchDev* dp = (SearchDev*)s;
    ORB_HIP_CHECK(hipMemcpyAsync(dp, &P, sizeof(SearchDev), hipMemcpyHostToDevice, stream_));
    hipLaunchKernelGGL(k_build_grid, dim3(1), dim3(256), grid_lds_bytes(frame.cur.N), stream_, dp, 0);
    if (nq == 0) return stream_wait(stream_) == hipSuccess ? 0 : -2;
    hipLaunchKernelGGL(k_area_count, dim3((nq + 255) / 256), dim3(256), 0, stream_, dp, d_q, nq, d_cnt);
    ORB_HIP_CHECK(hipGetLastError());
    ORB_HIP_CHECK(hipMemcpyAsync(off.data() + 1, d_cnt, sizeof(int) * nq, hipMemcpyDeviceToHost, stream_));
    ORB_HIP_CHECK(stream_wait(stream_));
    for (int i = 0; i < nq; i++) off[i + 1] += off[i];
    const int total = off[nq];
    cand.resize((size_t)std::max(total, 1));
    if (total == 0) return 0;
    if ((size_t)total * sizeof(int2) > cand_cap_) {
        if (d_cand_) (void)hipFree(d_cand_);
        cand_cap_ = (size_t)total * sizeof(int2) * 2;
        ORB_HIP_CHECK(hipMalloc(&d_cand_, cand_cap_));
    }
    ORB_HIP_CHECK(hipMemcpyAsync(d_off, off.data(), sizeof(int) * ((size_t)nq + 1), hipMemcpyHostToDevice, stream_));
    hipLaunchKernelGGL(k_area_fill, dim3((nq + 255) / 256), dim3(256), 0, stream_, dp, d_q, nq, d_qdesc, d_off,
                       (int2*)d_cand_);
    ORB_HIP_CHECK(hipGetLastError());
    ORB_HIP_CHECK(hipMemcpyAsync(cand.data(), d_cand_, sizeof(int2) * (size_t)total, hipMemcpyDeviceToHost, stream_));
    ORB_HIP_CHECK(stream_wait(stream_));
    return 0;
}

Matcher::~Matcher() {
    for (int i = 0; i < 16; i++)
        if (ev_[i]) (void)hipEventDestroy(ev_[i]);
    if (d_count_) (void)hipFree(d_count_);
    if (d_cand_) (void)hipFree(d_cand_);
    if (d_dense_) (void)hipFree(d_dense_);
    if (d_scratch_) (void)hipFree(d_scratch_);
    if (d_probs_) (void)hipFree(d_probs_);
    if (d_arena_) (void)hipFree(d_arena_);
    if (stream_) (void)hipStreamDestroy(stream_);
}

int Matcher::init_device() {
    int n = 0;
    if (hipGetDeviceCount(&n) != hipSuccess || n <= 0) return -4;
    const char* pe = std::getenv("ORBGPU_MATCH_STREAM_PRIO");
    if (pe && pe[0] == '1') {
        int lo = 0, hi = 0;
        ORB_HIP_CHECK(hipDeviceGetStreamPriorityRange(&lo, &hi));
        ORB_HIP_CHECK(hipStreamCreateWithPriority(&stream_, hipStreamNonBlocking, hi));
    } else {
        ORB_HIP_CHECK(hipStreamCreateWithFlags(&stream_, hipStreamNonBlocking));
    }
    return 0;
}

int Matcher::arena_reserve(size_t bytes) {
    arena_used_ = 0;
    if (bytes <= arena_cap_) return 0;
    if (d_arena_) (void)hipFree(d_arena_);
    d_arena_ = nullptr;
    arena_cap_ = 0;
    ORB_HIP_CHECK(hipMalloc(&d_arena_, bytes));
    arena_cap_ = bytes;
    return 0;
}

void* Matcher::arena_alloc(size_t bytes) {
    bytes = (bytes + 255) & ~(size_t)255;
    if (arena_used_ + bytes > arena_cap_) return nullptr;
    void* p = (char*)d_arena_ + arena_used_;
    arena_used_ += bytes;
    return p;
}

static inline int cand_gx(int maxq, int nt) { return (maxq + nt - 1) / nt; }
static inline dim3 cand_grid(int maxq, int nt, int np) { return xcd_grid(cand_gx(maxq, nt), np); }

int Matcher::run(std::vector<SearchDev>& probs, float th, bool bMono, bool lastMode, float nnratio) {
    const int np = (int)probs.size();
    if (np == 0) return 0;
    size_t need = 0;
    int maxq = 0, maxN = 1;
    const bool vis = frustum_ != nullptr;
    for (auto& p : probs) {
        if (p.cur.N > kMaxFrameKeys || p.cur.N < 0 || p.nq < 0) return -1;
        maxN = std::max(maxN, p.cur.N);
        need += ((size_t)(kGridCells + 1 + p.cur.N) * 4 + 255) & ~(size_t)255;
        need += ((size_t)p.nq * (kTopK * 8 + 16 + 8) + 255) & ~(size_t)255;
        if (vis) need += ((size_t)p.nq * 4 + 255) & ~(size_t)255;
        maxq = std::max(maxq, p.nq);
    }
    if (vis) need += ((size_t)np * 4 + 255) & ~(size_t)255;
    if (need > scratch_cap_) {
        if (d_scratch_) (void)hipFree(d_scratch_);
        scratch_cap_ = need * 2;
        ORB_HIP_CHECK(hipMalloc(&d_scratch_, scratch_cap_));
    }
    char* s = (char*)d_scratch_;
    int* visCounts = nullptr;
    if (vis) {
        visCounts = (int*)s;
        s += ((size_t)np * 4 + 255) & ~(size_t)255;
    }
    for (size_t k = 0; k < probs.size(); k++) {
        SearchDev& p = probs[k];
        p.gridStart = (int*)s;
        p.gridIdx = p.gridStart + kGridCells + 1;
        s += ((size_t)(kGridCells + 1 + p.cur.N) * 4 + 255) & ~(size_t)255;
        p.topk = (int2*)s;
        p.qinfo = (int4*)(p.topk + (size_t)p.nq * kTopK);
        p.hist = (int2*)(p.qinfo + p.nq);
        s += ((size_t)p.nq * (kTopK * 8 + 16 + 8) + 255) & ~(size_t)255;
        p.visList = nullptr;
        p.visCount = nullptr;
        if (vis) {
            p.visList = (int*)s;
            p.visCount = visCounts + k;
            s += ((size_t)p.nq * 4 + 255) & ~(size_t)255;
        }
    }
    if (vis) ORB_HIP_CHECK(hipMemsetAsync(visCounts, 0, (size_t)np * 4, stream_));
    const size_t pb = sizeof(SearchDev) * np;
    if (pb > probs_cap_) {
        if (d_probs_) (void)hipFree(d_probs_);
        probs_cap_ = pb * 2;
        ORB_HIP_CHECK(hipMalloc(&d_probs_, probs_cap_));
    }
    ORB_HIP_CHECK(hipMemcpyAsync(d_probs_, h2d_src(probs.data(), pb), pb, hipMemcpyHostToDevice, stream_));
    SearchDev* dp = (SearchDev*)d_probs_;
    if (frustum_ && maxq > 0) {
        mark(8);
        hipLaunchKernelGGL(k_frustum, cand_grid(maxq, 256, np), dim3(256), 0, stream_, (const SearchDev*)dp,
                           frustum_, frustumCos_, frustumLsf_, np, cand_gx(maxq, 256));
        mark(9);
    }
    if (timing_) {
        if (int e = zero_counters(0, 2)) return e;
        mark(0);
    }
    hipLaunchKernelGGL(k_build_grid, dim3(np), dim3(256), grid_lds_bytes(maxN), stream_, dp, 1);
    mark(1);
    if (maxq > 0) {
        if (lastMode) {
            if (maxN <= kStageMaxN && stage_threads() == 256)
                hipLaunchKernelGGL((k_candidates<true, true, 256>), cand_grid(maxq, 256, np), dim3(256), kStageLds,
                                   stream_, dp, np, cand_gx(maxq, 256), th, (int)bMono, counters());
            else if (maxN <= kStageMaxN)
                hipLaunchKernelGGL((k_candidates<true, true, kStageThreads>), cand_grid(maxq, kStageThreads, np),
                                   dim3(kStageThreads), kStageLds,
                                   stream_, dp, np, cand_gx(maxq, kStageThreads), th, (int)bMono, counters());
            else
                hipLaunchKernelGGL((k_candidates<true, false, 256>), cand_grid(maxq, 256, np), dim3(256), 0, stream_, dp,
                                   np, cand_gx(maxq, 256), th, (int)bMono, counters());
            mark(2);
            hipLaunchKernelGGL((k_select_r<true, 512, kSelQLast>), dim3(np), dim3(512), select_lds_bytes(maxN), stream_, dp,
                               th, (int)bMono, nnratio, (int)checkOri_, maxN);
        } else {
            if (maxN <= kStageMaxN && cand_local_stage() && stage_threads() == 256)
                hipLaunchKernelGGL((k_candidates<false, true, 256>), cand_grid(maxq, 256, np), dim3(256), kStageLds,
                                   stream_, dp, np, cand_gx(maxq, 256), th, 0, counters());
            else if (maxN <= kStageMaxN && cand_local_stage())
                hipLaunchKernelGGL((k_candidates<false, true, kStageThreads>), cand_grid(maxq, kStageThreads, np),
                                   dim3(kStageThreads), kStageLds,
                                   stream_, dp, np, cand_gx(maxq, kStageThreads), th, 0, counters());
            else
                hipLaunchKernelGGL((k_candidates<false, false, 256>), cand_grid(maxq, 256, np), dim3(256), 0, stream_, dp,
                                   np, cand_gx(maxq, 256), th, 0, counters());
            mark(2);
            if (select_local_threads() == 512)
                hipLaunchKernelGGL((k_select_r<false, 512, 2 * kSelQLocal>), dim3(np), dim3(512), select_lds_bytes(maxN),
                                   stream_, dp, th, 0, nnratio, 0, maxN);
            else
                hipLaunchKernelGGL((k_select_r<false, kSelectLocalThreads, kSelQLocal>), dim3(np),
                                   dim3(kSelectLocalThreads), select_lds_bytes(maxN), stream_, dp, th, 0, nnratio, 0, maxN);
        }
    } else {
        mark(2);
    }
    mark(3);
    ORB_HIP_CHECK(hipGetLastError());
    return 0;
}

int Matcher::search_last(std::vector<SearchDev>& probs, float th, bool bMono) {
    return run(probs, th, bMono, true, nnratio_);
}

int Matcher::frustum(std::vector<SearchDev>& probs, const std::vector<FrustumDev>& fr, float viewingCosLimit,
                     float logScaleFactor) {
    const int np = (int)probs.size();
    int maxq = 0;
    for (auto& p : probs) maxq = std::max(maxq, p.nq);
    if (np == 0 || maxq == 0) return 0;
    const size_t pb = sizeof(SearchDev) * np;
    if (pb > probs_cap_) {
        if (d_probs_) (void)hipFree(d_probs_);
        probs_cap_ = pb * 2;
        ORB_HIP_CHECK(hipMalloc(&d_probs_, probs_cap_));
    }
    FrustumDev* dfr = (FrustumDev*)arena_alloc(sizeof(FrustumDev) * np);
    if (!dfr) return -2;
    ORB_HIP_CHECK(hipMemcpyAsync(d_probs_, probs.data(), pb, hipMemcpyHostToDevice, stream_));
    ORB_HIP_CHECK(hipMemcpyAsync(dfr, fr.data(), sizeof(FrustumDev) * np, hipMemcpyHostToDevice, stream_));
    mark(8);
    hipLaunchKernelGGL(k_frustum, cand_grid(maxq, 256, np), dim3(256), 0, stream_, (const SearchDev*)d_probs_, dfr,
                       viewingCosLimit, logScaleFactor, np, cand_gx(maxq, 256));
    mark(9);
    ORB_HIP_CHECK(hipGetLastError());
    return 0;
}

int Matcher::search_local_points(std::vector<SearchDev>& probs, std::vector<FrustumDev>& fr, float viewingCosLimit,
                                 float logScaleFactor, float th, float nnratio) {
    const int np = (int)probs.size();
    if (np == 0) return 0;
    int maxq = 0;
    for (auto& p : probs) maxq = std::max(maxq, p.nq);
    if (maxq > 0) {
        size_t need = sizeof(FrustumDev) * np + 256;
        for (auto& p : probs) need += 7 * ((((size_t)p.nq * 4) + 255) & ~(size_t)255);
        char* base = (char*)arena_alloc(need);
        if (!base) return -2;
        char* o = base + ((sizeof(FrustumDev) * np + 255) & ~(size_t)255);
        for (int k = 0; k < np; k++) {
            const size_t b = (((size_t)probs[k].nq * 4) + 255) & ~(size_t)255;
            FrustumDev& f = fr[k];
            f.inView = (uint8_t*)o; o += b;
            f.projX = (float*)o; o += b;
            f.projXR = (float*)o; o += b;
            f.projY = (float*)o; o += b;
            f.level = (int*)o; o += b;
            f.viewCos = (float*)o; o += b;
            f.mpIndex = (int*)o; o += b;
            SearchDev& P = probs[k];
            P.inView = f.inView; P.projX = f.projX; P.projXR = f.projXR; P.projY = f.projY;
            P.level = f.level; P.viewCos = f.viewCos; P.mpIndex = f.mpIndex;
        }
        ORB_HIP_CHECK(hipMemcpyAsync(base, h2d_src(fr.data(), sizeof(FrustumDev) * np), sizeof(FrustumDev) * np,
                                     hipMemcpyHostToDevice, stream_));
        frustum_ = (const FrustumDev*)base;
        frustumCos_ = viewingCosLimit;
        frustumLsf_ = logScaleFactor;
    }
    const int rc = run(probs, th, false, false, nnratio);
    frustum_ = nullptr;
    return rc;
}
int Matcher::search_local(std::vector<SearchDev>& probs, float th) { return run(probs, th, false, false, nnratio_); }

int Matcher::candidates(const uint8_t* q, int nq, const uint8_t* t, int nt, const int* off, const int* cand, int* dist,
                        int* best_idx, int* best_dist, int* second_dist) {
    (void)nt;
    if (nq <= 0) return 0;
    if (timing_) {
        if (int e = zero_counters(4, 2)) return e;
        mark(12);
    }
    hipLaunchKernelGGL(k_csr_hamming, dim3((nq + 3) / 4), dim3(256), 0, stream_, q, nq, t, off, cand, dist, best_idx,
                       best_dist, second_dist, counters());
    mark(13);
    ORB_HIP_CHECK(hipGetLastError());
    return 0;
}

static int dense_block() {
    static const int v = [] {
        const char* e = std::getenv("ORBGPU_DENSE_TB");
        const int b = e ? std::atoi(e) : kDenseBlock;
        return b == 64 || b == 128 ? b : kDenseBlock;
    }();
    return v;
}

int Matcher::dense(const std::vector<DenseDev>& probs) {
    const int np = (int)probs.size();
    if (np == 0) return 0;
    const int TB = dense_block();
    std::vector<DenseJob> jobs;
    std::vector<int> qjob;
    int maxBlk = 0;
    for (int p = 0; p < np; p++) {
        const int nb = std::max(1, (probs[p].nt + TB - 1) / TB);
        maxBlk = std::max(maxBlk, nb);
        for (int q0 = 0; q0 < probs[p].nq; q0 += kDenseQ) {
            qjob.push_back((int)jobs.size());
            for (int b = 0; b < nb; b++) jobs.push_back(DenseJob{p, q0, b * TB, (int)jobs.size()});
        }
    }
    const size_t bP = (sizeof(DenseDev) * np + 255) & ~(size_t)255, bJ = (sizeof(DenseJob) * jobs.size() + 255) & ~(size_t)255;
    const size_t bQ = (sizeof(int) * qjob.size() + 255) & ~(size_t)255;
    const size_t bPart = sizeof(unsigned long long) * 2 * kDenseQ * std::max<size_t>(jobs.size(), 1);
    const size_t need = bP + bJ + bQ + bPart;
    if (need > dense_cap_) {
        if (d_dense_) (void)hipFree(d_dense_);
        d_dense_ = nullptr;
        dense_cap_ = 0;
        ORB_HIP_CHECK(hipMalloc(&d_dense_, need * 2));
        dense_cap_ = need * 2;
    }
    char* b = (char*)d_dense_;
    DenseDev* dP = (DenseDev*)b;
    DenseJob* dJ = (DenseJob*)(b + bP);
    int* dQ = (int*)(b + bP + bJ);
    unsigned long long* dPart = (unsigned long long*)(b + bP + bJ + bQ);
    std::vector<char> h(bP + bJ + bQ, 0);
    std::memcpy(h.data(), probs.data(), sizeof(DenseDev) * np);
    if (!jobs.empty()) std::memcpy(h.data() + bP, jobs.data(), sizeof(DenseJob) * jobs.size());
    if (!qjob.empty()) std::memcpy(h.data() + bP + bJ, qjob.data(), sizeof(int) * qjob.size());
    ORB_HIP_CHECK(hipMemcpyAsync(b, h2d_src(h.data(), h.size()), h.size(), hipMemcpyHostToDevice, stream_));
    if (timing_) {
        if (int e = zero_counters(6, 1)) return e;
        mark(14);
    }
    if (!jobs.empty()) {
        if (TB == 64)
            hipLaunchKernelGGL(k_dense_hamming<64>, dim3((unsigned)jobs.size()), dim3(kDenseQ), 0, stream_,
                               (const DenseDev*)dP, (const DenseJob*)dJ, dPart, counters());
        else if (TB == 128)
            hipLaunchKernelGGL(k_dense_hamming<128>, dim3((unsigned)jobs.size()), dim3(kDenseQ), 0, stream_,
                               (const DenseDev*)dP, (const DenseJob*)dJ, dPart, counters());
        else
            hipLaunchKernelGGL(k_dense_hamming<kDenseBlock>, dim3((unsigned)jobs.size()), dim3(kDenseQ), 0, stream_,
                               (const DenseDev*)dP, (const DenseJob*)dJ, dPart, counters());
    }
    if (!qjob.empty())
        hipLaunchKernelGGL(k_dense_merge, dim3((unsigned)((qjob.size() * kDenseQ + 255) / 256)), dim3(256), 0, stream_,
                           (const DenseDev*)dP, (const int*)dQ, (const DenseJob*)dJ, maxBlk, dPart, (int)qjob.size(),
                           (int)jobs.size());
    mark(15);
    ORB_HIP_CHECK(hipGetLastError());
    if (!chain_.on()) ORB_HIP_CHECK(stream_wait(stream_));
    return 0;
}

int Matcher::dense_timing(float* ms, long long* pairs) {
    *ms = -1.0f;
    *pairs = -1;
    if (!d_count_) return 0;
    ORB_HIP_CHECK(stream_wait(stream_));
    if (evSet_[14] && evSet_[15]) (void)hipEventElapsedTime(ms, ev_[14], ev_[15]);
    std::vector<unsigned long long> c(kCountSlots);
    ORB_HIP_CHECK(hipMemcpy(c.data(), d_count_ + 6 * kCountSlots, sizeof(unsigned long long) * kCountSlots,
                            hipMemcpyDeviceToHost));
    *pairs = 0;
    for (unsigned long long v : c) *pairs += (long long)v;
    return 0;
}

int Matcher::set_timing(bool on) {
    if (on && !d_count_) {
        for (int i = 0; i < 16; i++) ORB_HIP_CHECK(hipEventCreate(&ev_[i]));
        ORB_HIP_CHECK(hipMalloc(&d_count_, sizeof(unsigned long long) * 8 * kCountSlots));
        ORB_HIP_CHECK(hipMemset(d_count_, 0, sizeof(unsigned long long) * 8 * kCountSlots));
    }
    timing_ = on;
    return 0;
}

void Matcher::mark(int i) {
    if (!timing_) return;
    (void)hipEventRecord(ev_[i], stream_);
    evSet_[i] = true;
}

int Matcher::zero_counters(int first, int n) {
    ORB_HIP_CHECK(hipMemsetAsync(d_count_ + (size_t)first * kCountSlots, 0, sizeof(unsigned long long) * n * kCountSlots,
                                 stream_));
    return 0;
}

int Matcher::timings(float* ms8, long long* cnt8) {
    for (int i = 0; i < 8; i++) {
        ms8[i] = -1.0f;
        cnt8[i] = -1;
    }
    if (!d_count_) return 0;
    ORB_HIP_CHECK(stream_wait(stream_));
    const int pairs[8][2] = {{0, 1}, {1, 2}, {2, 3}, {4, 5}, {5, 6}, {6, 7}, {12, 13}, {8, 9}};
    for (int k = 0; k < 8; k++) {
        const int a = pairs[k][0], b = pairs[k][1];
        if (evSet_[a] && evSet_[b]) (void)hipEventElapsedTime(&ms8[k], ev_[a], ev_[b]);
    }
    std::vector<unsigned long long> c(8 * kCountSlots);
    ORB_HIP_CHECK(hipMemcpy(c.data(), d_count_, sizeof(unsigned long long) * c.size(), hipMemcpyDeviceToHost));
    for (int i = 0; i < 8; i++) {
        cnt8[i] = 0;
        for (int k = 0; k < kCountSlots; k++) cnt8[i] += (long long)c[(size_t)i * kCountSlots + k];
    }
    return 0;
}

int debug_prof_match(unsigned long long* out32) {
#ifdef ORBGPU_PROF
// ... 12 lines not shown
```

### c_orb_slam_amd/csrc/orb_match.hpp

```cpp
#pragma once
#include <cstdint>
#include <vector>

#include "orb_common.hpp"
#include "orb_extract.hpp"

namespace orbgpu {

constexpr int kGridCols = 64;
constexpr int kGridRows = 48;
constexpr int kGridCells = kGridCols * kGridRows;
constexpr int kTopK = 8;
constexpr int kMaxFrameKeys = 4096;

struct FrameDev {
    int N;
    const orb_kp_dev* keysUn;
    const uint8_t* desc;
    const float* uRight;
    float minX, maxX, minY, maxY, gridWInv, gridHInv;
    const float* scale;
    int nlevels;
    float fx, fy, cx, cy, bf, b;
    const float* Tcw;
};

struct SearchDev {
    FrameDev cur;
    FrameDev last;
    const orb_kp_dev* lastKeys;
    const int* lastMP;
    const uint8_t* lastOutlier;
    const uint8_t* inView;
    const float* projX;
    const float* projXR;
    const float* projY;
    const int* level;
    const float* viewCos;
    const int* mpIndex;
    int nq;
    const float* mpPos;
    const uint8_t* mpDesc;
    const int* mpObs;
    int* curMP;
    int* nmatches;
    int* gridStart;
    int* gridIdx;
    int2* topk;
    int4* qinfo;
    int2* hist;
    int* visList;
    int* visCount;
};

struct FrustumDev {
    const float* maxDist;
    const float* minDist;
    const float* normal;
    const uint8_t* skip;
    uint8_t* inView;
    float* projX;
    float* projXR;
    float* projY;
    int* level;
    float* viewCos;
    int* mpIndex;
    int* nvisible;
};

struct DenseDev {
    const uint8_t* q;
    const uint8_t* t;
    int nq, nt;
    int* best_idx;
    int* best_dist;
    int* second_dist;
};

struct AreaQuery {
    float x, y, r;
    int minLevel, maxLevel;
    int qd;
};

constexpr int kCountSlots = 64;

class Matcher {
public:
    Matcher(float nnratio, bool checkOri) : nnratio_(nnratio), checkOri_(checkOri) {}
    ~Matcher();
    int init_device();
    void set_device_pointers(bool on) { device_ptrs_ = on; }
    bool device_pointers() const { return device_ptrs_; }
    int search_last(std::vector<SearchDev>& probs, float th, bool bMono);
    int search_local(std::vector<SearchDev>& probs, float th);
    int search_local_points(std::vector<SearchDev>& probs, std::vector<FrustumDev>& fr, float viewingCosLimit,
                            float logScaleFactor, float th, float nnratio);
    int frustum(std::vector<SearchDev>& probs, const std::vector<FrustumDev>& fr, float viewingCosLimit,
                float logScaleFactor);
    int candidates(const uint8_t* q, int nq, const uint8_t* t, int nt, const int* off, const int* cand, int* dist,
                   int* best_idx, int* best_dist, int* second_dist);
    int dense(const std::vector<DenseDev>& probs);
    int dense_timing(float* ms, long long* pairs);
    hipStream_t stream() const { return stream_; }
    DeferredChain& chain() { return chain_; }
    const void* h2d_src(const void* host, size_t bytes) { return chain_.on() ? chain_.stage(host, bytes) : host; }
    void* count_buf(size_t bytes) { return chain_.on() ? chain_.dev_counts(bytes) : arena_alloc(bytes); }
    int d2h_counts(void* user, const void* dev, size_t bytes) {
        if (chain_.on()) {
            chain_.land_dev(user, dev, bytes);
            return 0;
        }
        ORB_HIP_CHECK(hipMemcpyAsync(user, dev, bytes, hipMemcpyDeviceToHost, stream_));
        return 0;
    }
    int end_call() {
        if (chain_.on()) return 0;
        ORB_HIP_CHECK(hipStreamSynchronize(stream_));
        return 0;
    }
    float nnratio() const { return nnratio_; }
    bool check_ori() const { return checkOri_; }

    int area_candidates(const SearchDev& frame, const AreaQuery* d_q, int nq, const uint8_t* d_qdesc,
                        std::vector<int>& off, std::vector<int2>& cand);
    int arena_reserve(size_t bytes);
    void* arena_alloc(size_t bytes);

    int set_timing(bool on);
    bool timing() const { return timing_; }
    int timings(float* ms8, long long* cnt8);
    void mark(int i);
    unsigned long long* counters() const { return timing_ ? d_count_ : nullptr; }
    int zero_counters(int first, int n);

private:
    int run(std::vector<SearchDev>& probs, float th, bool bMono, bool lastMode, float nnratio);
    float nnratio_;
    bool checkOri_;
    bool device_ptrs_ = false;
    hipStream_t stream_ = nullptr;
    DeferredChain chain_;
    void* d_scratch_ = nullptr;
    size_t scratch_cap_ = 0;
    void* d_probs_ = nullptr;
    size_t probs_cap_ = 0;
    void* d_arena_ = nullptr;
    size_t arena_cap_ = 0, arena_used_ = 0;
    void* d_cand_ = nullptr;
    size_t cand_cap_ = 0;
    void* d_dense_ = nullptr;
    size_t dense_cap_ = 0;
    bool timing_ = false;
    const FrustumDev* frustum_ = nullptr;
    float frustumCos_ = 0.5f, frustumLsf_ = 0.f;
    hipEvent_t ev_[16] = {};
    bool evSet_[16] = {};
    unsigned long long* d_count_ = nullptr;
};

int debug_prof_match(unsigned long long* out32);

}
```

### c_orb_slam_amd/csrc/pose_opt.hip

```cpp
#include <algorithm>
#include <cstdlib>
#include <cstring>
#include <functional>
#include <vector>

#include "ba.hpp"
#include "ba_math.hpp"
#include "orb_common.hpp"

namespace orbgpu {

struct PoseEdgeDev {
    float Xw[3], obs[3];
    float info;
    int meta;
};

struct PoseProbDev {
    int ne, e0;
    int nbad, N;
    Se3 T0;
    Se3 T;
    double fx, fy, cx, cy, bf;
    const float* Tcw;
// ... 278 lines not shown
    }
    if (!(sign == 1 || sign == 0)) return false;
    double y[6];
#pragma unroll
    for (int i = 0; i < 6; i++) y[i] = bs[ord[i]];
#pragma unroll
    for (int i = 0; i < 6; i++)
#pragma unroll
        for (int j = 0; j < i; j++) y[i] -= A[i * 6 + j] * y[j];
    {
        double den[6], q[6];
#pragma unroll
        for (int i = 0; i < 6; i++) den[i] = A[i * 6 + i];
        lane_div<6>(y, den, q);
#pragma unroll
        for (int i = 0; i < 6; i++) y[i] = fabs(A[i * 6 + i]) > DBL_MIN ? q[i] : 0.0;
    }
#pragma unroll
    for (int i = 5; i >= 0; i--)
#pragma unroll
        for (int j = 5; j > i; j--) y[i] -= A[j * 6 + i] * y[j];
#pragma unroll
    for (int j = 0; j < 6; j++) {
        double v = 0.0;
#pragma unroll
        for (int p = 0; p < 6; p++)
            if (ord[p] == j) v = y[p];
        x[j] = v;
    }
    return true;
}

__device__ __forceinline__ bool pose_solve_l(const double* Hs, const double* bs, double lambda, double* x,
                                             double* scr) {
    double dv[6];
#pragma unroll
    for (int i = 0; i < 6; i++) dv[i] = fabs(Hs[DIAG21[i]] + lambda);
    bool distinct = true;
    int rank[6];
#pragma unroll
    for (int j = 0; j < 6; j++) {
        int r = 0;
        distinct = distinct && dv[j] == dv[j];
#pragma unroll
        for (int i = 0; i < 6; i++)
            if (i != j) {
                r += dv[i] > dv[j] ? 1 : 0;
                distinct = distinct && dv[i] != dv[j];
            }
        rank[j] = r;
    }
    int ord[6];
#pragma unroll
    for (int r = 0; r < 6; r++) {
        int o = 0;
#pragma unroll
        for (int j = 0; j < 6; j++) o = rank[j] == r ? j : o;
        ord[r] = o;
    }
    const double a00 = Hs[DIAG21[ord[0]]] + lambda;
    if (!distinct || !(fabs(a00) > 0.0)) {
        double Hd[36], bb[6];
#pragma unroll
        for (int r = 0, q = 0; r < 6; r++)
#pragma unroll
            for (int cc = r; cc < 6; cc++, q++) {
                double h = Hs[q];
                if (cc == r) h += lambda;
                Hd[r * 6 + cc] = h;
                Hd[cc * 6 + r] = h;
            }
#pragma unroll
        for (int j = 0; j < 6; j++) bb[j] = bs[j];
        return ldlt_pivot6(Hd, bb, x);
    }
    const int lane = threadIdx.x & 63, row = lane < 6 ? lane : 5;
    int orow = ord[0];
#pragma unroll
    for (int p = 1; p < 6; p++) orow = row == p ? ord[p] : orow;
    double a[6];
#pragma unroll
    for (int c = 0; c < 6; c++) {
        const int i0 = min(orow, ord[c]), i1 = max(orow, ord[c]);
        double h = Hs[i0 * 6 - (i0 * (i0 - 1)) / 2 + (i1 - i0)];
        if (row == c) h += lambda;
        a[c] = h;
    }
    double d[6];
    bool anyNeg = false;
#pragma unroll
    for (int k = 0; k < 6; k++) {
        if (k > 0) {
            double tmp[6];
#pragma unroll
            for (int j = 0; j < k; j++) tmp[j] = d[j] * lane_bcast(a[j], k);
            double u = 0;
#pragma unroll
            for (int j = 0; j < k; j++) u += a[j] * tmp[j];
            const double ak = a[k] - u;
            a[k] = row >= k ? ak : a[k];
        }
        const double akk = lane_bcast(a[k], k);
        d[k] = akk;
        if (k < 5) {
            const double q = a[k] / akk;
            a[k] = (fabs(akk) > 0.0 && row > k) ? q : a[k];
        }
        anyNeg = anyNeg || akk < 0;
    }
    if (anyNeg) return false;
    double y = bs[orow];
#pragma unroll
    for (int j = 0; j < 5; j++) {
        const double yj = lane_bcast(y, j);
        const double v = y - a[j] * yj;
        y = row > j ? v : y;
    }
    double arr = a[0];
#pragma unroll
    for (int c = 1; c < 6; c++) arr = row == c ? a[c] : arr;
    {
        const double q = y / arr;
        y = fabs(arr) > DBL_MIN ? q : 0.0;
    }
    if (lane < 6)
#pragma unroll
        for (int c = 0; c < 6; c++) scr[lane * 6 + c] = a[c];
    __builtin_amdgcn_s_waitcnt(0xc07f);
    __builtin_amdgcn_wave_barrier();
    double col[6];
#pragma unroll
    for (int j = 0; j < 6; j++) col[j] = scr[j * 6 + row];
#pragma unroll
    for (int j = 5; j >= 1; j--) {
        const double xj = lane_bcast(y, j);
        const double v = y - col[j] * xj;
        y = row < j ? v : y;
    }
    double yb[6];
#pragma unroll
    for (int p = 0; p < 6; p++) yb[p] = lane_bcast(y, p);
#pragma unroll
    for (int j = 0; j < 6; j++) {
        double v = 0.0;
#pragma unroll
        for (int p = 0; p < 6; p++)
            if (ord[p] == j) v = yb[p];
        x[j] = v;
    }
    return true;
}

template <int NT>
__global__ void __launch_bounds__(NT) k_pose_opt(PoseProbDev* probs, const PoseEdgeDev* __restrict__ Eall,
                                                 double* errAll, uint8_t* outlAll) {
    ORBGPU_LATENCY_WAVE();
    constexpr int kPosePer = kPoseMaxEdges / NT;
    PoseProbDev& P = probs[blockIdx.x];
    const int ne = P.ne;
    const PoseEdgeDev* E = Eall + P.e0;
    (void)errAll;
    uint8_t* outl = outlAll + P.e0;
    __shared__ uint8_t fl[kPoseMaxEdges];
    __shared__ uint16_t aE[kPoseMaxEdges];
    __shared__ double cs[28][kPoseMaxEdges / 64];
    __shared__ double red[32];
    constexpr int kPoseSpec = 3;
    __shared__ Se3 T, Terr, Tbase, Tc[kPoseSpec + 1];
    __shared__ double xc[kPoseSpec + 1][6];
    __shared__ int okc[kPoseSpec + 1];
    __shared__ double scrSolve[kPoseSpec + 1][36];
    __shared__ double xs[6], Hs[21], bs[6], sysN[28];
    __shared__ double lambda, ni, currentChi, iniChi;
    __shared__ int nA, nBadLM, qmax, again, term, nBad, haveSys, specPass, wsum[16];
    const int tid = threadIdx.x;
    const double dM = (double)(float)sqrt(5.991), dS = (double)(float)sqrt(7.815);
    if (ne < 0) {
        if (tid == 0 && P.ninl) *P.ninl = -1;
        return;
    }
    if (ne < 3) {
        if (tid == 0) {
            P.T = P.T0;
            P.nbad = -1;
            if (P.ninl) *P.ninl = 0;
        }
        if (P.Tcw_out) {
            if (tid < 16) P.Tcw_out[tid] = P.Tcw[tid];
            for (int i = tid; i < ne; i += blockDim.x) P.outlier[E[i].meta & 0x7fffffff] = 0;
            if (tid < 16) __threadfence_system();
        }
        return;
    }
    for (int i = tid; i < ne; i += blockDim.x) {
        fl[i] = 2;
        outl[i] = 0;
    }
    __syncthreads();
    const float chi2Mono = 5.991f, chi2Stereo = 7.815f;
    for (int it = 0; it < 4; it++) {
        if (tid == 0) {
            T = P.T0;
            for (int j = 0; j < 6; j++) xs[j] = 0.0;
        }
        {
            const int base = tid * kPosePer;
            int c = 0;
            for (int j = 0; j < kPosePer; j++) c += (base + j < ne && (fl[base + j] & 1) == 0) ? 1 : 0;
            int incl = c;
            for (int o = 1; o < 64; o <<= 1) {
                const int t = __shfl_up(incl, o, 64);
                if ((tid & 63) >= o) incl += t;
            }
            if ((tid & 63) == 63) wsum[tid >> 6] = incl;
            __syncthreads();
            int off = 0;
            for (int w = 0; w < (tid >> 6); w++) off += wsum[w];
            int pos = off + incl - c;
            for (int j = 0; j < kPosePer; j++)
                if (base + j < ne && (fl[base + j] & 1) == 0) aE[pos++] = (uint16_t)(base + j);
            if (tid == blockDim.x - 1) nA = off + incl;
            __syncthreads();
        }
        const int na = nA;
        const int myIdx = tid < na ? aE[tid] : 0;
        const PoseEdgeD myE = pose_edge_load(E, myIdx, dM, dS);
        if (na > 0) {
            ORBGPU_PROF_START;
            auto sys_terms = [&](const PoseEdgeD& e, int i, const Se3& X, double* v) {
                double p[3];
                se3_map(X, e.X, p);
                const SharedDiv dz(p[2]);
                double e3[3];
                pose_err_p(e, p, dz, P, e3);
                const double c = pose_chi2(e, e3);
                const bool rb = (fl[i] & 2) != 0;
                v[0] = pose_rho0(e, c, rb);
                const double x = p[0], y = p[1], invz = dz.div(1.0), invz_2 = invz * invz;
                double J[18];
                J[0] = ((x * y) * invz_2) * P.fx;
                J[1] = (-(1 + ((x * x) * invz_2))) * P.fx;
                J[2] = (y * invz) * P.fx;
                J[3] = (-invz) * P.fx;
                J[4] = 0;
                J[5] = (x * invz_2) * P.fx;
                J[6] = (1 + ((y * y) * invz_2)) * P.fy;
                J[7] = (((-x) * y) * invz_2) * P.fy;
                J[8] = ((-x) * invz) * P.fy;
                J[9] = 0;
                J[10] = (-invz) * P.fy;
                J[11] = (y * invz_2) * P.fy;
                J[12] = J[0] - ((P.bf * y) * invz_2);
                J[13] = J[1] + ((P.bf * x) * invz_2);
                J[14] = J[2];
                J[15] = J[3];
                J[16] = 0;
                J[17] = J[5] - (P.bf * invz_2);
#pragma unroll
                for (int j = 12; j < 18; j++) J[j] = e.stereo ? J[j] : 0.0;
                double r1 = 1.;
                if (rb && !(c <= e.dsqr)) r1 = e.delta / sqrt(c);
                const double wgt = rb ? r1 * e.info : e.info;
                double omr[3];
#pragma unroll
                for (int kk = 0; kk < 3; kk++) {
                    omr[kk] = -(e.info * e3[kk]);
                    if (rb) omr[kk] *= r1;
                }
#pragma unroll
                for (int r = 0; r < 6; r++) {
                    double sb = 0;
#pragma unroll
                    for (int kk = 0; kk < 3; kk++) sb += J[kk * 6 + r] * omr[kk];
                    v[22 + r] = sb;
#pragma unroll
                    for (int cc = r; cc < 6; cc++) {
                        double hh = 0;
#pragma unroll
                        for (int kk = 0; kk < 3; kk++) hh += (J[kk * 6 + r] * wgt) * J[kk * 6 + cc];
                        v[1 + r * 6 - (r * (r - 1)) / 2 + (cc - r)] = hh;
                    }
                }
            };
            if (tid == 0) haveSys = 0;
            __syncthreads();
            int kit = 0;
            bool sysPhase = true;
            for (;;) {
                if (!sysPhase) {
                    ORBGPU_PROF_MARK(10);
                    if (tid < 64 * (kPoseSpec + 1)) {
                        const int L = tid >> 6;
                        double ls = lambda, ns = ni;
                        for (int j = 0; j < L; j++) {
                            ls *= ns;
                            ns *= 2;
                        }
                        double xn[6];
#ifndef ORBGPU_POSE_SOLVE_W
                        const bool ok = pose_solve_l(Hs, bs, ls, xn, scrSolve[L]);
#else
                        const bool ok = pose_solve_w(Hs, bs, ls, xn);
#endif
                        ORBGPU_PROF_MARK(5);
                        ORBGPU_PROF_COUNT(9);
                        double xl[6];
#pragma unroll
                        for (int j = 0; j < 6; j++) xl[j] = (ok || L > 0) ? xn[j] : xs[j];
                        Se3 r = Tbase;
                        if (ok || L == 0) {
                            Se3 d;
                            se3_exp(xl, d);
                            se3_mul(d, Tbase, r);
                        }
                        if ((tid & 63) == 0) {
                            Tc[L] = r;
#pragma unroll
                            for (int j = 0; j < 6; j++) xc[L][j] = xl[j];
                            okc[L] = ok ? 1 : 0;
                        }
                    }
                    __syncthreads();
                    ORBGPU_PROF_MARK(2);
                } else {
                    ORBGPU_PROF_MARK(0);
                    ORBGPU_PROF_COUNT(8);
                }
                auto trial = [&](int j, double tempChi) {
                    if (!okc[j]) tempChi = DBL_MAX;
#pragma unroll
                    for (int q = 0; q < 6; q++) xs[q] = xc[j][q];
                    double rho = currentChi - tempChi;
                    double sv[6];
                    for (int q = 0; q < 6; q++) sv[q] = xs[q] * (lambda * xs[q] + bs[q]);
                    double scale = tree64_local([&](int q) { return sv[q]; }, 6);
                    scale += 1e-3;
                    rho /= scale;
                    Terr = Tc[j];
                    if (rho > 0 && isfinite(tempChi)) {
                        const double a3 = 2 * rho - 1;
                        double alpha = 1. - (a3 * a3) * a3;
                        alpha = fmin(alpha, 2. / 3.);
                        const double scaleFactor = fmax(1. / 3., alpha);
                        lambda *= scaleFactor;
                        ni = 2;
                        currentChi = tempChi;
                        T = Tc[j];
                        if (j == 0) haveSys = 1;
                    } else {
                        lambda *= ni;
                        ni *= 2;
                        T = Tbase;
                    }
                    qmax++;
                    again = (rho < 0 && qmax < 10) ? 1 : 0;
                    if (!again) {
                        if (qmax == 10 || rho == 0) {
                            term = 1;
                        } else {
                            if ((iniChi - currentChi) * 1e3 < iniChi) nBadLM++;
                            else nBadLM = 0;
                            term = nBadLM >= 3 ? 1 : 0;
                        }
                    }
                };
                {
                    const Se3& X = sysPhase ? T : Tc[0];
                    pose_pass_post<28>([&](const PoseEdgeD& e, int i, double* v) { sys_terms(e, i, X, v); }, na, aE, E,
                                       dM, dS, cs, red, myE, myIdx, [&] {
                                           if (!sysPhase) {
                                               trial(0, red[0]);
                                               specPass = again && okc[1] ? 1 : 0;
                                           }
                                       });
                }
                if (sysPhase) {
                    ORBGPU_PROF_MARK(1);
                    if (tid < 28) {
                        if (tid == 0) currentChi = iniChi = red[0];
                        else if (tid < 22) Hs[tid - 1] = red[tid];
                        else bs[tid - 22] = red[tid];
                    }
                } else {
                    ORBGPU_PROF_MARK(3);
                    if (haveSys && tid < 28) sysN[tid] = red[tid];
                    if (specPass) {
                        pose_pass<kPoseSpec>([&](const PoseEdgeD& e, int i, double* v) {
#pragma unroll
                            for (int L = 1; L <= kPoseSpec; L++) {
                                double e3[3];
                                pose_err(e, Tc[L], P, e3);
                                v[L - 1] = pose_rho0(e, pose_chi2(e, e3), (fl[i] & 2) != 0);
                            }
                        }, na, aE, E, dM, dS, cs, red, myE, myIdx);
                        if (tid == 0)
                            for (int j = 1; j <= kPoseSpec && again && okc[j]; j++) trial(j, red[j - 1]);
                        __syncthreads();
                    }
                    ORBGPU_PROF_MARK(4);
                    if (again) continue;
                    __syncthreads();
                    if (term || ++kit == 10) break;
                    if (!haveSys) {
                        sysPhase = true;
                        continue;
                    }
                    if (tid < 28) {
                        if (tid == 0) currentChi = iniChi = sysN[0];
                        else if (tid < 22) Hs[tid - 1] = sysN[tid];
                        else bs[tid - 22] = sysN[tid];
                    }
                }
                __syncthreads();
                if (tid == 0) {
                    if (kit == 0) {
                        double mx = 0.;
                        for (int j = 0; j < 6; j++) mx = fmax(fabs(Hs[DIAG21[j]]), mx);
                        lambda = 1e-5 * mx;
                        ni = 2;
                        nBadLM = 0;
                    }
                    qmax = 0;
                    haveSys = 0;
                    Tbase = T;
                }
                sysPhase = false;
                __syncthreads();
            }
        }
        if (tid == 0) nBad = 0;
        __syncthreads();
        int mybad = 0;
        for (int i = tid; i < ne; i += blockDim.x) {
            const PoseEdgeD e = pose_edge_load(E, i, dM, dS);
            double e3[3];
            pose_err(e, outl[i] ? T : Terr, P, e3);
            const float chi2 = (float)pose_chi2(e, e3);
            uint8_t f = fl[i];
            if (chi2 > (e.stereo ? chi2Stereo : chi2Mono)) {
                outl[i] = 1;
                f |= 1;
                mybad++;
            } else {
                outl[i] = 0;
                f &= 2;
            }
            if (it == 2) f &= 1;
            fl[i] = f;
        }
        if (mybad) atomicAdd(&nBad, mybad);
        __syncthreads();
        if (ne < 10) break;
    }
    if (tid == 0) {
        P.T = T;
        P.nbad = nBad;
        if (P.ninl) *P.ninl = ne - nBad;
    }
    if (P.Tcw_out) {
        if (tid == 0) {
            double R[9];
            quat_to_R(T.q, R);
            float* o = P.Tcw_out;
            for (int r = 0; r < 3; r++) {
                for (int c = 0; c < 3; c++) o[r * 4 + c] = (float)R[r * 3 + c];
                o[r * 4 + 3] = (float)T.t[r];
            }
            o[12] = o[13] = o[14] = 0.f;
            o[15] = 1.f;
            __threadfence_system();
        }
        for (int i = tid; i < ne; i += blockDim.x) P.outlier[E[i].meta & 0x7fffffff] = outl[i];
    }
}

constexpr int kPackThreads = 256;
__global__ void __launch_bounds__(kPackThreads) k_pose_pack(PoseProbDev* probs, PoseEdgeDev* Eall) {
    ORBGPU_LATENCY_WAVE();
    PoseProbDev& P = probs[blockIdx.x];
    const int N = P.N, tid = threadIdx.x;
    PoseEdgeDev* E = Eall + P.e0;
    __shared__ int wsum[kPackThreads / 64], base;
    if (tid == 0) {
        base = 0;
        double R[9];
        for (int r = 0; r < 3; r++)
            for (int c = 0; c < 3; c++) R[r * 3 + c] = (double)P.Tcw[r * 4 + c];
        quat_from_R(R, P.T0.q);
        for (int r = 0; r < 3; r++) P.T0.t[r] = (double)P.Tcw[r * 4 + 3];
        P.T0.pad = 0;
        se3_normalize(P.T0);
    }
    __syncthreads();
    for (int c0 = 0; c0 < N; c0 += kPackThreads) {
        const int i = c0 + tid;
        const int f = i < N ? (P.mpidx ? (P.mpidx[i] >= 0 ? 1 : 0) : (P.has_mp[i] ? 1 : 0)) : 0;
        int incl = f;
        for (int o = 1; o < 64; o <<= 1) {
            const int t = __shfl_up(incl, o, 64);
            if ((tid & 63) >= o) incl += t;
        }
        if ((tid & 63) == 63) wsum[tid >> 6] = incl;
        __syncthreads();
        int off = base;
        for (int w = 0; w < (tid >> 6); w++) off += wsum[w];
        if (f) {
            const int k = off + incl - 1;
            if (k < kPoseMaxEdges) {
                PoseEdgeDev e;
                if (P.mpidx) {
                    const size_t m = (size_t)P.mpidx[i];
                    for (int j = 0; j < 3; j++) e.Xw[j] = P.mp_pos[3 * m + j];
                    e.obs[0] = P.keys[7 * (size_t)i];
                    e.obs[1] = P.keys[7 * (size_t)i + 1];
                    e.obs[2] = P.uR[i];
                    const int oct = min(max(__float_as_int(P.keys[7 * (size_t)i + 5]), 0), P.nlev - 1);
                    e.info = P.isig_tab[oct];
                } else {
                    for (int j = 0; j < 3; j++) {
                        e.Xw[j] = P.Xw[3 * i + j];
                        e.obs[j] = P.obs[3 * i + j];
                    }
                    e.info = P.inv_sigma2[i];
                }
                e.meta = i | (!(e.obs[2] < 0) ? (int)0x80000000u : 0);
                E[k] = e;
            }
        }
        __syncthreads();
        if (tid == kPackThreads - 1) base = off + incl;
        __syncthreads();
    }
    if (tid == 0) P.ne = base > kPoseMaxEdges ? -1 : base;
}

int PoseEngine::run_device(int count, const pose_problem* P, float* const* Tcw_out, uint8_t* const* outlier,
                           int* ninliers) {
    std::vector<int> Ns(count);
    for (int f = 0; f < count; f++) Ns[f] = P[f].N;
    return launch_device(count, Ns.data(), [&](int f, PoseProbDev& pp) {
        const pose_problem& Q = P[f];
        pp.fx = Q.fx; pp.fy = Q.fy; pp.cx = Q.cx; pp.cy = Q.cy; pp.bf = Q.bf;
        pp.Tcw = Q.Tcw; pp.has_mp = Q.has_mp; pp.Xw = Q.Xw; pp.obs = Q.obs; pp.inv_sigma2 = Q.inv_sigma2;
    }, Tcw_out, outlier, ninliers);
}

int PoseEngine::run_frames_device(int count, const pose_frame* F, float* const* Tcw_out, uint8_t* const* outlier,
                                  int* ninliers, hipStream_t s, DeferredChain* chain) {
    std::vector<int> Ns(count);
    for (int f = 0; f < count; f++) Ns[f] = F[f].N;
    return launch_device(count, Ns.data(), [&](int f, PoseProbDev& pp) {
        const pose_frame& Q = F[f];
        pp.fx = Q.fx; pp.fy = Q.fy; pp.cx = Q.cx; pp.cy = Q.cy; pp.bf = Q.bf;
        pp.Tcw = Q.Tcw;
        pp.mpidx = Q.mp; pp.mp_pos = Q.mp_pos; pp.keys = (const float*)Q.keysUn; pp.uR = Q.uRight;
        pp.isig_tab = Q.invLevelSigma2; pp.nlev = Q.nlevels;
    }, Tcw_out, outlier, ninliers, s, chain);
}

int PoseEngine::launch_device(int count, const int* Ns, const std::function<void(int, PoseProbDev&)>& fill,
                              float* const* Tcw_out, uint8_t* const* outlier, int* ninliers, hipStream_t s,
                              DeferredChain* chain) {
    hipStream_t st = s ? s : stream_;
    size_t nmax = 0;
    for (int f = 0; f < count; f++) nmax += (size_t)std::min(Ns[f], kPoseMaxEdges + 1);
    const auto al = [](size_t b) { return (b + 255) & ~(size_t)255; };
    const size_t bProb = al(sizeof(PoseProbDev) * count), bEdge = al(sizeof(PoseEdgeDev) * std::max<size_t>(nmax, 1));
    const size_t bOut = al(std::max<size_t>(nmax, 1)), bNin = al(sizeof(int) * count);
    const size_t need = bProb + bEdge + bOut + bNin;
    if (need > cap_) {
        if (lastUseSet_) ORB_HIP_CHECK(hipEventSynchronize(lastUse_));
        if (dArena_) (void)hipFree(dArena_);
        if (hArena_) (void)hipHostFree(hArena_);
        dArena_ = hArena_ = nullptr;
        cap_ = 0;
        ORB_HIP_CHECK(hipMalloc(&dArena_, need));
        ORB_HIP_CHECK(hipHostMalloc(&hArena_, need));
        cap_ = need;
    }
    char* d = (char*)dArena_;
    int* dNin = chain ? (int*)chain->dev_counts(sizeof(int) * count) : (int*)(d + bProb + bEdge + bOut);
    if (!dNin) return -2;
    std::vector<PoseProbDev> tmp;
    PoseProbDev* hp = (PoseProbDev*)hArena_;
    if (chain) {
        tmp.resize(count);
        hp = tmp.data();
    }
    size_t e0 = 0;
    for (int f = 0; f < count; f++) {
        PoseProbDev& pp = hp[f];
        memset(&pp, 0, sizeof(pp));
        pp.N = Ns[f];
        pp.e0 = (int)e0;
        e0 += (size_t)std::min(Ns[f], kPoseMaxEdges + 1);
        fill(f, pp);
        pp.Tcw_out = Tcw_out[f];
        pp.outlier = outlier[f];
        pp.ninl = dNin + f;
    }
    PoseProbDev* dp = (PoseProbDev*)d;
    PoseEdgeDev* dE = (PoseEdgeDev*)(d + bProb);
    const void* src = chain ? chain->stage(hp, sizeof(PoseProbDev) * count) : (const void*)hp;
    if (!src) return -2;
    if (lastUseSet_) ORB_HIP_CHECK(hipStreamWaitEvent(st, lastUse_, 0));
    ORB_HIP_CHECK(hipMemcpyAsync(d, src, sizeof(PoseProbDev) * count, hipMemcpyHostToDevice, st));
    hipLaunchKernelGGL(k_pose_pack, dim3(count), dim3(kPackThreads), 0, st, dp, dE);
    if (timing_) ORB_HIP_CHECK(hipEventRecord(tA_, st));
    if (count <= pose_wide_max())
        hipLaunchKernelGGL(k_pose_opt<kPoseThreadsWide>, dim3(count), dim3(kPoseThreadsWide),
                           pose_lds_pad((const void*)k_pose_opt<kPoseThreadsWide>), st, dp, (const PoseEdgeDev*)dE,
                           nullptr, (uint8_t*)(d + bProb + bEdge));
    else
        hipLaunchKernelGGL(k_pose_opt<kPoseThreads>, dim3(count), dim3(kPoseThreads),
                           pose_lds_pad((const void*)k_pose_opt<kPoseThreads>), st, dp, (const PoseEdgeDev*)dE, nullptr,
                           (uint8_t*)(d + bProb + bEdge));
    ORB_HIP_CHECK(hipGetLastError());
    if (timing_) {
        ORB_HIP_CHECK(hipEventRecord(tB_, st));
        timed_ = true;
    }
    if (chain) {
        chain->land_dev(ninliers, dNin, sizeof(int) * count);
        ORB_HIP_CHECK(hipEventRecord(lastUse_, st));
        lastUseSet_ = true;
        return 0;
    }
    ORB_HIP_CHECK(hipMemcpyAsync(hp, d, bProb, hipMemcpyDeviceToHost, st));
    ORB_HIP_CHECK(hipEventRecord(lastUse_, st));
    lastUseSet_ = true;
    ORB_HIP_CHECK(stream_wait(st));
    int rc = 0;
    for (int f = 0; f < count; f++) {
        const PoseProbDev& pp = hp[f];
        if (pp.ne < 0) rc = -3;
        ninliers[f] = pp.ne < 0 || pp.nbad < 0 ? 0 : pp.ne - pp.nbad;
    }
    return rc;
}

int PoseEngine::last_timing(float* ms) {
    if (!timed_) return -1;
    ORB_HIP_CHECK(hipEventSynchronize(tB_));
    ORB_HIP_CHECK(hipEventElapsedTime(ms, tA_, tB_));
    return 0;
}

PoseEngine::~PoseEngine() {
    if (lastUseSet_) (void)hipEventSynchronize(lastUse_);
    if (lastUse_) (void)hipEventDestroy(lastUse_);
    if (tA_) (void)hipEventDestroy(tA_);
    if (tB_) (void)hipEventDestroy(tB_);
    if (dArena_) (void)hipFree(dArena_);
    if (hArena_) (void)hipHostFree(hArena_);
    if (stream_) (void)hipStreamDestroy(stream_);
}

int PoseEngine::init() {
    int n = 0;
    if (hipGetDeviceCount(&n) != hipSuccess || n <= 0) return -4;
    ORB_HIP_CHECK(hipStreamCreateWithFlags(&stream_, hipStreamNonBlocking));
    ORB_HIP_CHECK(hipEventCreateWithFlags(&lastUse_, hipEventDisableTiming));
    ORB_HIP_CHECK(hipEventCreate(&tA_));
    ORB_HIP_CHECK(hipEventCreate(&tB_));
    return 0;
}

int PoseEngine::run(int count, const pose_problem* P, float* Tcw_out, uint8_t* const* outlier, int* ninliers) {
    size_t ne = 0;
    std::vector<int> nE(count);
    for (int f = 0; f < count; f++) {
        int c = 0;
        for (int i = 0; i < P[f].N; i++) c += P[f].has_mp[i] ? 1 : 0;
        if (c > kPoseMaxEdges) return -3;
        nE[f] = c;
        ne += c;
    }
    const auto al = [](size_t b) { return (b + 255) & ~(size_t)255; };
    const size_t bProb = al(sizeof(PoseProbDev) * count), bEdge = al(sizeof(PoseEdgeDev) * std::max<size_t>(ne, 1));
    const size_t bErr = al(sizeof(double) * 3 * std::max<size_t>(ne, 1)), bOut = al(std::max<size_t>(ne, 1));
    const size_t need = bProb + bEdge + bErr + bOut;
    if (lastUseSet_) ORB_HIP_CHECK(hipEventSynchronize(lastUse_));
    if (need > cap_) {
        if (dArena_) (void)hipFree(dArena_);
        if (hArena_) (void)hipHostFree(hArena_);
        dArena_ = hArena_ = nullptr;
        cap_ = 0;
        ORB_HIP_CHECK(hipMalloc(&dArena_, need));
        ORB_HIP_CHECK(hipHostMalloc(&hArena_, need));
        cap_ = need;
    }
    char* h = (char*)hArena_;
    char* d = (char*)dArena_;
    PoseProbDev* hp = (PoseProbDev*)h;
    PoseEdgeDev* he = (PoseEdgeDev*)(h + bProb);
    uint8_t* hOut = (uint8_t*)(h + bProb + bEdge + bErr);
    int e0 = 0;
    for (int f = 0; f < count; f++) {
        const pose_problem& Q = P[f];
        PoseProbDev& pp = hp[f];
        memset(&pp, 0, sizeof(pp));
        pp.ne = nE[f];
        pp.e0 = e0;
        host_se3_from_Tcw(Q.Tcw, pp.T0);
        pp.fx = Q.fx; pp.fy = Q.fy; pp.cx = Q.cx; pp.cy = Q.cy; pp.bf = Q.bf;
        for (int i = 0; i < Q.N; i++) {
            if (!Q.has_mp[i]) continue;
            PoseEdgeDev& e = he[e0++];
            for (int j = 0; j < 3; j++) {
                e.Xw[j] = Q.Xw[3 * i + j];
                e.obs[j] = Q.obs[3 * i + j];
            }
            e.info = Q.inv_sigma2[i];
            e.meta = i | (!(Q.obs[3 * i + 2] < 0) ? (int)0x80000000u : 0);
        }
    }
    PoseProbDev* dp = (PoseProbDev*)d;
    ORB_HIP_CHECK(hipMemcpyAsync(d, h, bProb + sizeof(PoseEdgeDev) * ne, hipMemcpyHostToDevice, stream_));
    if (count > 0)
    {
        if (count <= pose_wide_max())
            hipLaunchKernelGGL(k_pose_opt<kPoseThreadsWide>, dim3(count), dim3(kPoseThreadsWide), 0, stream_, dp, (const PoseEdgeDev*)(d + bProb),
                               (double*)(d + bProb + bEdge), (uint8_t*)(d + bProb + bEdge + bErr));
        else
            hipLaunchKernelGGL(k_pose_opt<kPoseThreads>, dim3(count), dim3(kPoseThreads), 0, stream_, dp, (const PoseEdgeDev*)(d + bProb),
                               (double*)(d + bProb + bEdge), (uint8_t*)(d + bProb + bEdge + bErr));
    }
    ORB_HIP_CHECK(hipGetLastError());
    ORB_HIP_CHECK(hipMemcpyAsync(h, d, bProb, hipMemcpyDeviceToHost, stream_));
    if (ne) ORB_HIP_CHECK(hipMemcpyAsync(hOut, d + bProb + bEdge + bErr, ne, hipMemcpyDeviceToHost, stream_));
    ORB_HIP_CHECK(hipEventRecord(lastUse_, stream_));
    lastUseSet_ = true;
    ORB_HIP_CHECK(hipStreamSynchronize(stream_));
    for (int f = 0; f < count; f++) {
        const pose_problem& Q = P[f];
        const PoseProbDev& pp = hp[f];
        const uint8_t* o = hOut + pp.e0;
        for (int i = 0, k = 0; i < Q.N; i++)
            if (Q.has_mp[i]) {
                outlier[f][i] = pp.nbad < 0 ? 0 : o[k];
                k++;
            }
        if (pp.nbad < 0) {
            memcpy(Tcw_out + 16 * (size_t)f, Q.Tcw, sizeof(float) * 16);
            ninliers[f] = 0;
        } else {
            host_se3_to_Tcw(pp.T, Tcw_out + 16 * (size_t)f);
            ninliers[f] = pp.ne - pp.nbad;
        }
    }
    return 0;
}

}
```

Before: 44720.

## Trim per-frame host overhead: reuse host tables, fuse pose pack, drop syncs and memsets

Replaces per-call std::vector allocations with tables cached on the matcher and pose engine. Stereo matching now waits on the extractor's completion event instead of blocking the host on its stream. The octree kernel writes per-image counts and error flags straight to coherent pinned host memory, so the final device-to-host copy goes away. Other changes: the pose pack kernel is folded into the pose optimiser, visibility counters live in a persistent buffer that the kernel resets, the frustum table rides in the same upload as the search table, and redundant cross-stream waits are skipped. The risks are ordering and visibility hazards around the coherent-memory writes and the counters that reset themselves.

```diff
diff --git a/c_orb_slam_amd/csrc/ba.hpp b/c_orb_slam_amd/csrc/ba.hpp
--- a/c_orb_slam_amd/csrc/ba.hpp
+++ b/c_orb_slam_amd/csrc/ba.hpp
@@ -192,6 +192,9 @@
     size_t cap_ = 0;
     hipEvent_t lastUse_ = nullptr;
     bool lastUseSet_ = false;
+    hipStream_t lastStream_ = nullptr;
+    std::vector<double> hostTab_;
+    std::vector<int> Ns_;
     bool timing_ = false, timed_ = false;
     hipEvent_t tA_ = nullptr, tB_ = nullptr;
 };
diff --git a/c_orb_slam_amd/csrc/capi_match.cpp b/c_orb_slam_amd/csrc/capi_match.cpp
--- a/c_orb_slam_amd/csrc/capi_match.cpp
+++ b/c_orb_slam_amd/csrc/capi_match.cpp
@@ -1,3 +1,4 @@
+#include <algorithm>
 #include <cstring>
 #include <new>
 #include <vector>
@@ -164,7 +165,7 @@
         }
     }
     int err = 0;
-    std::vector<SearchDev> probs(npairs);
+    std::vector<SearchDev>& probs = m->search_table(npairs);
     if (!dev) {
         size_t need = 0;
         for (int p = 0; p < npairs; p++) {
@@ -177,7 +178,6 @@
     }
     if (dev && m->arena_reserve((size_t)npairs * 4 + 256)) return ORB_E_HIP;
     int* d_nm = nullptr;
-    std::vector<int*> nm_dev(npairs, nullptr);
     for (int p = 0; p < npairs; p++) {
         SearchDev& P = probs[p];
         memset(&P, 0, sizeof(P));
@@ -208,7 +208,6 @@
             if (cur[p].N > 0 && hipMemcpyAsync(P.curMP, cur_mp[p], (size_t)cur[p].N * 4, hipMemcpyHostToDevice, s) != hipSuccess)
                 err = ORB_E_HIP;
         }
-        nm_dev[p] = nullptr;
     }
     if (err) return err;
     {
@@ -377,9 +376,11 @@
     int err = 0;
     int* d_cnt = (int*)m->count_buf((size_t)count * 8);
     if (!d_cnt) return ORB_E_HIP;
-    if (hipMemsetAsync(d_cnt, 0, (size_t)count * 8, s) != hipSuccess) return ORB_E_HIP;
-    std::vector<SearchDev> probs(count);
-    std::vector<orbgpu::FrustumDev> fr(count);
+    int maxn = 0;
+    for (int p = 0; p < count; p++) maxn = std::max(maxn, maps[p].n);
+    if (maxn == 0 && hipMemsetAsync(d_cnt, 0, (size_t)count * 8, s) != hipSuccess) return ORB_E_HIP;
+    std::vector<SearchDev>& probs = m->search_table(count);
+    std::vector<orbgpu::FrustumDev>& fr = m->frustum_table(count);
     for (int p = 0; p < count; p++) {
         SearchDev& P = probs[p];
         memset(&P, 0, sizeof(P));
diff --git a/c_orb_slam_amd/csrc/capi_stereo.cpp b/c_orb_slam_amd/csrc/capi_stereo.cpp
--- a/c_orb_slam_amd/csrc/capi_stereo.cpp
+++ b/c_orb_slam_amd/csrc/capi_stereo.cpp
@@ -61,8 +61,8 @@
     orbgpu::Matcher* m = h->m;
     const bool dev = m->device_pointers();
     hipStream_t s = m->stream();
-    if (orbgpu::stream_wait(EL->stream()) != hipSuccess ||
-        (ER != EL && orbgpu::stream_wait(ER->stream()) != hipSuccess))
+    if (!EL->drained() && hipStreamWaitEvent(s, EL->done_event(), 0) != hipSuccess) return ORB_E_HIP;
+    if (ER != EL && !ER->drained() && hipStreamWaitEvent(s, ER->done_event(), 0) != hipSuccess)
         return ORB_E_HIP;
     orbgpu::StereoParams P;
     std::memset(&P, 0, sizeof(P));
@@ -89,7 +89,7 @@
     }
     if (m->arena_reserve(need + 4096)) return ORB_E_HIP;
     int err = 0;
-    std::vector<orbgpu::StereoDev> probs(npairs);
+    orbgpu::StereoDev* probs = m->host_table<orbgpu::StereoDev>(npairs);
     int* d_kept = (int*)(dev ? m->count_buf(4 * (size_t)npairs) : m->arena_alloc(4 * (size_t)npairs));
     for (int p = 0; p < npairs; p++) {
         orbgpu::StereoDev& S = probs[p];
@@ -121,7 +121,7 @@
     if (err || !d_kept) return ORB_E_HIP;
     auto* d_probs = (orbgpu::StereoDev*)m->arena_alloc(sizeof(orbgpu::StereoDev) * npairs);
     if (!d_probs) return ORB_E_HIP;
-    if (hipMemcpyAsync(d_probs, m->h2d_src(probs.data(), sizeof(orbgpu::StereoDev) * npairs),
+    if (hipMemcpyAsync(d_probs, m->h2d_src(probs, sizeof(orbgpu::StereoDev) * npairs),
                        sizeof(orbgpu::StereoDev) * npairs, hipMemcpyHostToDevice, s) != hipSuccess)
         return ORB_E_HIP;
     if (orbgpu::stereo_launch(d_probs, npairs, maxNL, P, s, m)) return ORB_E_HIP;
@@ -276,7 +276,7 @@
 int MapPoint_CreateStereo_batch_device(ORBmatcher_h h, int count, const orb_newpoints* Q) {
     if (!h || count < 0 || (count > 0 && !Q)) return ORB_E_INVALID;
     if (count == 0) return ORB_OK;
-    std::vector<orbgpu::UnprojDev> P((size_t)count);
+    orbgpu::UnprojDev* P = h->m->host_table<orbgpu::UnprojDev>((size_t)count);
     for (int f = 0; f < count; f++) {
         const orb_newpoints& q = Q[f];
         if (q.N < 0 || (q.N > 0 && (!q.keysUn || !q.depth || !q.Twc || !q.x3D || !q.row || !q.normal ||
@@ -300,14 +300,14 @@
         d.scale = q.scaleFactors;
         d.nlevels = q.nlevels;
     }
-    return orbgpu::unproject_batch(P.data(), count, h->m->stream()) ? ORB_E_HIP : ORB_OK;
+    return orbgpu::unproject_batch(P, count, h->m->stream()) ? ORB_E_HIP : ORB_OK;
 }
 
 int Tracking_PrepareLocalSearch_batch_device(ORBmatcher_h h, int count, const orb_localprep* Q) {
     if (!h || count < 0 || (count > 0 && !Q)) return ORB_E_INVALID;
     if (count == 0) return ORB_OK;
     orbgpu::Matcher* m = h->m;
-    std::vector<orbgpu::LocalPrepDev> P((size_t)count);
+    orbgpu::LocalPrepDev* P = m->host_table<orbgpu::LocalPrepDev>((size_t)count);
     for (int f = 0; f < count; f++) {
         const orb_localprep& q = Q[f];
         if (q.N < 0 || q.n < 0 || (q.N > 0 && (!q.cur_mp || !q.outlier)) || (q.n > 0 && (!q.row || !q.skip)))
@@ -317,7 +317,7 @@
     if (m->arena_reserve(sizeof(orbgpu::LocalPrepDev) * count + 256)) return ORB_E_HIP;
     void* d = m->arena_alloc(sizeof(orbgpu::LocalPrepDev) * count);
     hipStream_t s = m->stream();
-    if (!d || hipMemcpyAsync(d, m->h2d_src(P.data(), sizeof(orbgpu::LocalPrepDev) * count),
+    if (!d || hipMemcpyAsync(d, m->h2d_src(P, sizeof(orbgpu::LocalPrepDev) * count),
                              sizeof(orbgpu::LocalPrepDev) * count, hipMemcpyHostToDevice, s) != hipSuccess)
         return ORB_E_HIP;
     if (orbgpu::local_prep_batch((const orbgpu::LocalPrepDev*)d, count, s)) return ORB_E_HIP;
diff --git a/c_orb_slam_amd/csrc/octree.hip b/c_orb_slam_amd/csrc/octree.hip
--- a/c_orb_slam_amd/csrc/octree.hip
+++ b/c_orb_slam_amd/csrc/octree.hip
@@ -507,7 +507,7 @@
 
 __global__ void __launch_bounds__(64) k_sel_build(const uint32_t* __restrict__ jobsel, const int* __restrict__ jobcnt,
                                                   int nlevels, int jcap, int cap, int2* __restrict__ sel, int selcap,
-                                                  int* __restrict__ nout, int* __restrict__ err) {
+                                                  int* __restrict__ nout, int* err, int* __restrict__ host) {
     const int b = blockIdx.x, lane = threadIdx.x;
     const int c = lane < nlevels ? jobcnt[b * nlevels + lane] : 0;
     int incl = c;
@@ -519,7 +519,13 @@
     const int total = __shfl(incl, 63, 64);
     if (lane == 0) {
         nout[b] = total;
-        if (total > cap || total > selcap) atomicOr(err, 1);
+        const bool over = total > cap || total > selcap;
+        const int e = over ? (atomicOr(err, 1) | 1) : __hip_atomic_load(err, __ATOMIC_RELAXED, __HIP_MEMORY_SCOPE_AGENT);
+        if (host) {
+            host[b] = total;
+            host[gridDim.x + b] = e;
+            __threadfence_system();
+        }
     }
     if (total > cap || total > selcap) return;
     for (int l = 0; l < nlevels; l++) {
@@ -546,7 +552,7 @@
 
 int octree_launch(const OctInput& in, int B, int nlevels, const OctLevelDev* lv, uint32_t* jobsel, int* jobcnt, int jcap,
                   uint16_t* gscratch, size_t gstride, int cap, int2* sel, int selcap, int* nout, int* err,
-                  hipStream_t s) {
+                  int* host_out, hipStream_t s) {
     static const int nt = [] {
         const char* e = getenv("ORBGPU_OCT_T");
         const int v = e ? atoi(e) : 512;
@@ -562,7 +568,7 @@
         hipLaunchKernelGGL(k_octree<256>, dim3(B * nlevels), dim3(256), 0, s, in, nlevels, lv, jobsel, jobcnt,
                            jcap, gscratch, gstride, err);
     hipLaunchKernelGGL(k_sel_build, dim3(B), dim3(64), 0, s, (const uint32_t*)jobsel, (const int*)jobcnt, nlevels,
-                       jcap, cap, sel, selcap, nout, err);
+                       jcap, cap, sel, selcap, nout, err, host_out);
     ORB_HIP_CHECK(hipGetLastError());
     return 0;
 }
diff --git a/c_orb_slam_amd/csrc/octree.hpp b/c_orb_slam_amd/csrc/octree.hpp
--- a/c_orb_slam_amd/csrc/octree.hpp
+++ b/c_orb_slam_amd/csrc/octree.hpp
@@ -29,6 +29,6 @@
 
 int octree_launch(const OctInput& in, int B, int nlevels, const OctLevelDev* lv, uint32_t* jobsel, int* jobcnt, int jcap,
                   uint16_t* gscratch, size_t gstride, int cap, int2* sel, int selcap, int* nout, int* err,
-                  hipStream_t s);
+                  int* host_out, hipStream_t s);
 
 }
diff --git a/c_orb_slam_amd/csrc/orb_extract.hip b/c_orb_slam_amd/csrc/orb_extract.hip
--- a/c_orb_slam_amd/csrc/orb_extract.hip
+++ b/c_orb_slam_amd/csrc/orb_extract.hip
@@ -1529,7 +1529,7 @@
     sel_cap_ = selcap_ * B;
     ORB_HIP_CHECK(hipMalloc(&d_sel_, (size_t)sel_cap_ * sizeof(int2)));
     if (h_nout_) (void)hipHostFree(h_nout_);
-    ORB_HIP_CHECK(hipHostMalloc((void**)&h_nout_, (size_t)(B + 1) * 4));
+    ORB_HIP_CHECK(hipHostMalloc((void**)&h_nout_, (size_t)B * 2 * 4, hipHostMallocCoherent));
     geomW_ = W;
     geomH_ = H;
     return 0;
@@ -1542,6 +1542,7 @@
     if (W > maxW_ || H > maxH_) return -1;
     if (int e = setup_geometry(W, H)) return e;
     hipStream_t s = stream_;
+    drained_.store(false, std::memory_order_release);
     const uint8_t* src = imgs;
     if (!imgs_on_device) {
         const size_t need = img_stride * (B - 1) + (size_t)step * (H - 1) + W;
@@ -1653,7 +1654,7 @@
                  (const int*)d_lcb_, ncells, (uint32_t*)d_packed_, d_gtotal_};
     if (int e = octree_launch(oin, B, nlevels_, (const OctLevelDev*)d_octlv_, (uint32_t*)d_jobsel_, (int*)d_jobcnt_,
                               jcap_, (uint16_t*)d_gscr_, (size_t)packed_cap_, cap, (int2*)d_sel_, selcap_,
-                              (int*)d_nout_, d_err, s))
+                              (int*)d_nout_, d_err, h_nout_, s))
         return e;
     ORB_HIP_CHECK(hipEventRecord(ev_[5], s));
     if (evBlur_)
@@ -1684,11 +1685,14 @@
                            (const int*)d_nout_, levelArgs_, okps, odesc, cap, gx, B);
     }
     ORB_HIP_CHECK(hipGetLastError());
-    ORB_HIP_CHECK(hipMemcpyAsync(h_nout_, d_nout_, (size_t)(B + 1) * 4, hipMemcpyDeviceToHost, s));
     ORB_HIP_CHECK(hipEventRecord(ev_[6], s));
     ORB_HIP_CHECK(stream_wait(s));
-    const int err = h_nout_[B];
-    for (int b = 0; b < B; b++) n_out[b] = h_nout_[b];
+    drained_.store(true, std::memory_order_release);
+    int err = 0;
+    for (int b = 0; b < B; b++) {
+        n_out[b] = h_nout_[b];
+        err |= h_nout_[B + b];
+    }
     if (err & 1) return -3;
     if (err) return -1;
     if (!out_on_device) {
diff --git a/c_orb_slam_amd/csrc/orb_extract.hpp b/c_orb_slam_amd/csrc/orb_extract.hpp
--- a/c_orb_slam_amd/csrc/orb_extract.hpp
+++ b/c_orb_slam_amd/csrc/orb_extract.hpp
@@ -93,6 +93,8 @@
     int timings(float* ms6);
     int corner_total(long long* total);
     hipStream_t stream() const { return stream_; }
+    bool drained() const { return drained_.load(std::memory_order_acquire); }
+    hipEvent_t done_event() const { return ev_[6]; }
     int reserve_cus(int one_in_n);
     int share_stream(Extractor* with);
     int build_work(int B);
@@ -149,6 +151,7 @@
     size_t img_bytes_ = 0, blur_bytes_ = 0, slots_per_image_ = 0;
     int packed_cap_ = 0, sel_cap_ = 0;
     int last_B_ = 0;
+    std::atomic<bool> drained_{false};
 
     hipStream_t stream_ = nullptr;
     bool ownStream_ = true;
diff --git a/c_orb_slam_amd/csrc/orb_match.hip b/c_orb_slam_amd/csrc/orb_match.hip
--- a/c_orb_slam_amd/csrc/orb_match.hip
+++ b/c_orb_slam_amd/csrc/orb_match.hip
@@ -781,6 +781,11 @@
         else if (lq >= 0) P.curMP[i] = LAST ? P.lastMP[lq] : P.mpIndex[lq];
     }
     if (tid == 0) *P.nmatches = s_nm - s_rmcnt;
+    if (!LAST && tid == 0 && list) {
+        if (P.nvisOut) *P.nvisOut = P.visCount[1];
+        P.visCount[0] = 0;
+        P.visCount[1] = 0;
+    }
     ORBGPU_PROF_MARK(LAST ? 3 : 11);
 }
 
@@ -983,9 +988,11 @@
 }
 
 Matcher::~Matcher() {
+    if (stream_) (void)hipStreamSynchronize(stream_);
     for (int i = 0; i < 16; i++)
         if (ev_[i]) (void)hipEventDestroy(ev_[i]);
     if (d_count_) (void)hipFree(d_count_);
+    if (d_ctr_) (void)hipFree(d_ctr_);
     if (d_cand_) (void)hipFree(d_cand_);
     if (d_dense_) (void)hipFree(d_dense_);
     if (d_scratch_) (void)hipFree(d_scratch_);
@@ -1044,17 +1051,20 @@
         if (vis) need += ((size_t)p.nq * 4 + 255) & ~(size_t)255;
         maxq = std::max(maxq, p.nq);
     }
-    if (vis) need += ((size_t)np * 4 + 255) & ~(size_t)255;
     if (need > scratch_cap_) {
         if (d_scratch_) (void)hipFree(d_scratch_);
         scratch_cap_ = need * 2;
         ORB_HIP_CHECK(hipMalloc(&d_scratch_, scratch_cap_));
     }
     char* s = (char*)d_scratch_;
-    int* visCounts = nullptr;
-    if (vis) {
-        visCounts = (int*)s;
-        s += ((size_t)np * 4 + 255) & ~(size_t)255;
+    if (vis && (size_t)np > ctr_cap_) {
+        if (d_ctr_) (void)hipFree(d_ctr_);
+        d_ctr_ = nullptr;
+        ctr_cap_ = 0;
+        const size_t cap = std::max<size_t>(2 * (size_t)np, 64);
+        ORB_HIP_CHECK(hipMalloc((void**)&d_ctr_, cap * 2 * sizeof(int)));
+        ORB_HIP_CHECK(hipMemsetAsync(d_ctr_, 0, cap * 2 * sizeof(int), stream_));
+        ctr_cap_ = cap;
     }
     for (size_t k = 0; k < probs.size(); k++) {
         SearchDev& p = probs[k];
@@ -1069,23 +1079,33 @@
         p.visCount = nullptr;
         if (vis) {
             p.visList = (int*)s;
-            p.visCount = visCounts + k;
+            p.visCount = d_ctr_ + 2 * k;
+            p.nvisOut = frustum_[k].nvisible;
+            frustum_[k].nvisible = p.visCount + 1;
             s += ((size_t)p.nq * 4 + 255) & ~(size_t)255;
         }
     }
-    if (vis) ORB_HIP_CHECK(hipMemsetAsync(visCounts, 0, (size_t)np * 4, stream_));
-    const size_t pb = sizeof(SearchDev) * np;
-    if (pb > probs_cap_) {
+    const size_t pb = sizeof(SearchDev) * np, fb = vis ? sizeof(FrustumDev) * np : 0;
+    static_assert(sizeof(SearchDev) % alignof(FrustumDev) == 0, "FrustumDev table behind the SearchDev table");
+    if (pb + fb > probs_cap_) {
         if (d_probs_) (void)hipFree(d_probs_);
-        probs_cap_ = pb * 2;
+        probs_cap_ = (pb + fb) * 2;
         ORB_HIP_CHECK(hipMalloc(&d_probs_, probs_cap_));
     }
-    ORB_HIP_CHECK(hipMemcpyAsync(d_probs_, h2d_src(probs.data(), pb), pb, hipMemcpyHostToDevice, stream_));
+    const void* src = probs.data();
+    if (vis) {
+        upload_.resize(pb + fb);
+        std::memcpy(upload_.data(), probs.data(), pb);
+        std::memcpy(upload_.data() + pb, frustum_, fb);
+        src = upload_.data();
+    }
+    ORB_HIP_CHECK(hipMemcpyAsync(d_probs_, h2d_src(src, pb + fb), pb + fb, hipMemcpyHostToDevice, stream_));
     SearchDev* dp = (SearchDev*)d_probs_;
-    if (frustum_ && maxq > 0) {
+    if (vis && maxq > 0) {
         mark(8);
         hipLaunchKernelGGL(k_frustum, cand_grid(maxq, 256, np), dim3(256), 0, stream_, (const SearchDev*)dp,
-                           frustum_, frustumCos_, frustumLsf_, np, cand_gx(maxq, 256));
+                           (const FrustumDev*)((const char*)d_probs_ + pb), frustumCos_, frustumLsf_, np,
+                           cand_gx(maxq, 256));
         mark(9);
     }
     if (timing_) {
@@ -1171,11 +1191,10 @@
     int maxq = 0;
     for (auto& p : probs) maxq = std::max(maxq, p.nq);
     if (maxq > 0) {
-        size_t need = sizeof(FrustumDev) * np + 256;
+        size_t need = 256;
         for (auto& p : probs) need += 7 * ((((size_t)p.nq * 4) + 255) & ~(size_t)255);
-        char* base = (char*)arena_alloc(need);
-        if (!base) return -2;
-        char* o = base + ((sizeof(FrustumDev) * np + 255) & ~(size_t)255);
+        char* o = (char*)arena_alloc(need);
+        if (!o) return -2;
         for (int k = 0; k < np; k++) {
             const size_t b = (((size_t)probs[k].nq * 4) + 255) & ~(size_t)255;
             FrustumDev& f = fr[k];
@@ -1190,9 +1209,7 @@
             P.inView = f.inView; P.projX = f.projX; P.projXR = f.projXR; P.projY = f.projY;
             P.level = f.level; P.viewCos = f.viewCos; P.mpIndex = f.mpIndex;
         }
-        ORB_HIP_CHECK(hipMemcpyAsync(base, h2d_src(fr.data(), sizeof(FrustumDev) * np), sizeof(FrustumDev) * np,
-                                     hipMemcpyHostToDevice, stream_));
-        frustum_ = (const FrustumDev*)base;
+        frustum_ = fr.data();
         frustumCos_ = viewingCosLimit;
         frustumLsf_ = logScaleFactor;
     }
diff --git a/c_orb_slam_amd/csrc/orb_match.hpp b/c_orb_slam_amd/csrc/orb_match.hpp
--- a/c_orb_slam_amd/csrc/orb_match.hpp
+++ b/c_orb_slam_amd/csrc/orb_match.hpp
@@ -51,6 +51,7 @@
     int2* hist;
     int* visList;
     int* visCount;
+    int* nvisOut;
 };
 
 struct FrustumDev {
@@ -121,6 +122,20 @@
     }
     float nnratio() const { return nnratio_; }
     bool check_ori() const { return checkOri_; }
+    std::vector<SearchDev>& search_table(size_t n) {
+        searchTab_.resize(n);
+        return searchTab_;
+    }
+    std::vector<FrustumDev>& frustum_table(size_t n) {
+        frustumTab_.resize(n);
+        return frustumTab_;
+    }
+    template <class T>
+    T* host_table(size_t n) {
+        static_assert(alignof(T) <= alignof(double), "host_table storage alignment");
+        hostTab_.resize((n * sizeof(T) + sizeof(double) - 1) / sizeof(double));
+        return reinterpret_cast<T*>(hostTab_.data());
+    }
 
     int area_candidates(const SearchDev& frame, const AreaQuery* d_q, int nq, const uint8_t* d_qdesc,
                         std::vector<int>& off, std::vector<int2>& cand);
@@ -152,7 +167,13 @@
     void* d_dense_ = nullptr;
     size_t dense_cap_ = 0;
     bool timing_ = false;
-    const FrustumDev* frustum_ = nullptr;
+    FrustumDev* frustum_ = nullptr;
+    std::vector<SearchDev> searchTab_;
+    std::vector<FrustumDev> frustumTab_;
+    std::vector<double> hostTab_;
+    std::vector<char> upload_;
+    int* d_ctr_ = nullptr;
+    size_t ctr_cap_ = 0;
     float frustumCos_ = 0.5f, frustumLsf_ = 0.f;
     hipEvent_t ev_[16] = {};
     bool evSet_[16] = {};
diff --git a/c_orb_slam_amd/csrc/pose_opt.hip b/c_orb_slam_amd/csrc/pose_opt.hip
--- a/c_orb_slam_amd/csrc/pose_opt.hip
+++ b/c_orb_slam_amd/csrc/pose_opt.hip
@@ -454,12 +454,69 @@
 }
 
 template <int NT>
-__global__ void __launch_bounds__(NT) k_pose_opt(PoseProbDev* probs, const PoseEdgeDev* __restrict__ Eall,
-                                                 double* errAll, uint8_t* outlAll) {
+__device__ __forceinline__ int pose_pack(PoseProbDev& P, PoseEdgeDev* E, int* wsum, int& base) {
+    const int N = P.N, tid = threadIdx.x;
+    if (tid == 0) {
+        base = 0;
+        double R[9];
+        for (int r = 0; r < 3; r++)
+            for (int c = 0; c < 3; c++) R[r * 3 + c] = (double)P.Tcw[r * 4 + c];
+        quat_from_R(R, P.T0.q);
+        for (int r = 0; r < 3; r++) P.T0.t[r] = (double)P.Tcw[r * 4 + 3];
+        P.T0.pad = 0;
+        se3_normalize(P.T0);
+    }
+    __syncthreads();
+    for (int c0 = 0; c0 < N; c0 += NT) {
+        const int i = c0 + tid;
+        const int f = i < N ? (P.mpidx ? (P.mpidx[i] >= 0 ? 1 : 0) : (P.has_mp[i] ? 1 : 0)) : 0;
+        int incl = f;
+        for (int o = 1; o < 64; o <<= 1) {
+            const int t = __shfl_up(incl, o, 64);
+            if ((tid & 63) >= o) incl += t;
+        }
+        if ((tid & 63) == 63) wsum[tid >> 6] = incl;
+        __syncthreads();
+        int off = base;
+        for (int w = 0; w < (tid >> 6); w++) off += wsum[w];
+        if (f) {
+            const int k = off + incl - 1;
+            if (k < kPoseMaxEdges) {
+                PoseEdgeDev e;
+                if (P.mpidx) {
+                    const size_t m = (size_t)P.mpidx[i];
+                    for (int j = 0; j < 3; j++) e.Xw[j] = P.mp_pos[3 * m + j];
+                    e.obs[0] = P.keys[7 * (size_t)i];
+                    e.obs[1] = P.keys[7 * (size_t)i + 1];
+                    e.obs[2] = P.uR[i];
+                    const int oct = min(max(__float_as_int(P.keys[7 * (size_t)i + 5]), 0), P.nlev - 1);
+                    e.info = P.isig_tab[oct];
+                } else {
+                    for (int j = 0; j < 3; j++) {
+                        e.Xw[j] = P.Xw[3 * i + j];
+                        e.obs[j] = P.obs[3 * i + j];
+                    }
+                    e.info = P.inv_sigma2[i];
+                }
+                e.meta = i | (!(e.obs[2] < 0) ? (int)0x80000000u : 0);
+                E[k] = e;
+            }
+        }
+        __syncthreads();
+        if (tid == NT - 1) base = off + incl;
+        __syncthreads();
+    }
+    const int ne = base > kPoseMaxEdges ? -1 : base;
+    if (tid == 0) P.ne = ne;
+    return ne;
+}
+
+template <int NT, bool PACK>
+__global__ void __launch_bounds__(NT) k_pose_opt(PoseProbDev* probs, PoseEdgeDev* __restrict__ Eall, double* errAll,
+                                                 uint8_t* outlAll) {
     ORBGPU_LATENCY_WAVE();
     constexpr int kPosePer = kPoseMaxEdges / NT;
     PoseProbDev& P = probs[blockIdx.x];
-    const int ne = P.ne;
     const PoseEdgeDev* E = Eall + P.e0;
     (void)errAll;
     uint8_t* outl = outlAll + P.e0;
@@ -475,7 +532,10 @@
     __shared__ double xs[6], Hs[21], bs[6], sysN[28];
     __shared__ double lambda, ni, currentChi, iniChi;
     __shared__ int nA, nBadLM, qmax, again, term, nBad, haveSys, specPass, wsum[16];
+    __shared__ int packBase;
+    static_assert(NT / 64 <= 16, "wsum holds one partial per wave");
     const int tid = threadIdx.x;
+    const int ne = PACK ? pose_pack<NT>(P, Eall + P.e0, wsum, packBase) : P.ne;
     const double dM = (double)(float)sqrt(5.991), dS = (double)(float)sqrt(7.815);
     if (ne < 0) {
         if (tid == 0 && P.ninl) *P.ninl = -1;
@@ -776,66 +836,6 @@
     }
 }
 
-constexpr int kPackThreads = 256;
-__global__ void __launch_bounds__(kPackThreads) k_pose_pack(PoseProbDev* probs, PoseEdgeDev* Eall) {
-    ORBGPU_LATENCY_WAVE();
-    PoseProbDev& P = probs[blockIdx.x];
-    const int N = P.N, tid = threadIdx.x;
-    PoseEdgeDev* E = Eall + P.e0;
-    __shared__ int wsum[kPackThreads / 64], base;
-    if (tid == 0) {
-        base = 0;
-        double R[9];
-        for (int r = 0; r < 3; r++)
-            for (int c = 0; c < 3; c++) R[r * 3 + c] = (double)P.Tcw[r * 4 + c];
-        quat_from_R(R, P.T0.q);
-        for (int r = 0; r < 3; r++) P.T0.t[r] = (double)P.Tcw[r * 4 + 3];
-        P.T0.pad = 0;
-        se3_normalize(P.T0);
-    }
-    __syncthreads();
-    for (int c0 = 0; c0 < N; c0 += kPackThreads) {
-        const int i = c0 + tid;
-        const int f = i < N ? (P.mpidx ? (P.mpidx[i] >= 0 ? 1 : 0) : (P.has_mp[i] ? 1 : 0)) : 0;
-        int incl = f;
-        for (int o = 1; o < 64; o <<= 1) {
-            const int t = __shfl_up(incl, o, 64);
-            if ((tid & 63) >= o) incl += t;
-        }
-        if ((tid & 63) == 63) wsum[tid >> 6] = incl;
-        __syncthreads();
-        int off = base;
-        for (int w = 0; w < (tid >> 6); w++) off += wsum[w];
-        if (f) {
-            const int k = off + incl - 1;
-            if (k < kPoseMaxEdges) {
-                PoseEdgeDev e;
-                if (P.mpidx) {
-                    const size_t m = (size_t)P.mpidx[i];
-                    for (int j = 0; j < 3; j++) e.Xw[j] = P.mp_pos[3 * m + j];
-                    e.obs[0] = P.keys[7 * (size_t)i];
-                    e.obs[1] = P.keys[7 * (size_t)i + 1];
-                    e.obs[2] = P.uR[i];
-                    const int oct = min(max(__float_as_int(P.keys[7 * (size_t)i + 5]), 0), P.nlev - 1);
-                    e.info = P.isig_tab[oct];
-                } else {
-                    for (int j = 0; j < 3; j++) {
-                        e.Xw[j] = P.Xw[3 * i + j];
-                        e.obs[j] = P.obs[3 * i + j];
-                    }
-                    e.info = P.inv_sigma2[i];
-                }
-                e.meta = i | (!(e.obs[2] < 0) ? (int)0x80000000u : 0);
-                E[k] = e;
-            }
-        }
-        __syncthreads();
-        if (tid == kPackThreads - 1) base = off + incl;
-        __syncthreads();
-    }
-    if (tid == 0) P.ne = base > kPoseMaxEdges ? -1 : base;
-}
-
 int PoseEngine::run_device(int count, const pose_problem* P, float* const* Tcw_out, uint8_t* const* outlier,
                            int* ninliers) {
     std::vector<int> Ns(count);
@@ -849,7 +849,8 @@
 
 int PoseEngine::run_frames_device(int count, const pose_frame* F, float* const* Tcw_out, uint8_t* const* outlier,
                                   int* ninliers, hipStream_t s, DeferredChain* chain) {
-    std::vector<int> Ns(count);
+    std::vector<int>& Ns = Ns_;
+    Ns.resize(count);
     for (int f = 0; f < count; f++) Ns[f] = F[f].N;
     return launch_device(count, Ns.data(), [&](int f, PoseProbDev& pp) {
         const pose_frame& Q = F[f];
@@ -883,11 +884,10 @@
     char* d = (char*)dArena_;
     int* dNin = chain ? (int*)chain->dev_counts(sizeof(int) * count) : (int*)(d + bProb + bEdge + bOut);
     if (!dNin) return -2;
-    std::vector<PoseProbDev> tmp;
     PoseProbDev* hp = (PoseProbDev*)hArena_;
     if (chain) {
-        tmp.resize(count);
-        hp = tmp.data();
+        hostTab_.resize((sizeof(PoseProbDev) * count + sizeof(double) - 1) / sizeof(double));
+        hp = (PoseProbDev*)hostTab_.data();
     }
     size_t e0 = 0;
     for (int f = 0; f < count; f++) {
@@ -905,17 +905,16 @@
     PoseEdgeDev* dE = (PoseEdgeDev*)(d + bProb);
     const void* src = chain ? chain->stage(hp, sizeof(PoseProbDev) * count) : (const void*)hp;
     if (!src) return -2;
-    if (lastUseSet_) ORB_HIP_CHECK(hipStreamWaitEvent(st, lastUse_, 0));
+    if (lastUseSet_ && lastStream_ != st) ORB_HIP_CHECK(hipStreamWaitEvent(st, lastUse_, 0));
     ORB_HIP_CHECK(hipMemcpyAsync(d, src, sizeof(PoseProbDev) * count, hipMemcpyHostToDevice, st));
-    hipLaunchKernelGGL(k_pose_pack, dim3(count), dim3(kPackThreads), 0, st, dp, dE);
     if (timing_) ORB_HIP_CHECK(hipEventRecord(tA_, st));
     if (count <= pose_wide_max())
-        hipLaunchKernelGGL(k_pose_opt<kPoseThreadsWide>, dim3(count), dim3(kPoseThreadsWide),
-                           pose_lds_pad((const void*)k_pose_opt<kPoseThreadsWide>), st, dp, (const PoseEdgeDev*)dE,
-                           nullptr, (uint8_t*)(d + bProb + bEdge));
+        hipLaunchKernelGGL((k_pose_opt<kPoseThreadsWide, true>), dim3(count), dim3(kPoseThreadsWide),
+                           pose_lds_pad((const void*)k_pose_opt<kPoseThreadsWide, true>), st, dp, dE, nullptr,
+                           (uint8_t*)(d + bProb + bEdge));
     else
-        hipLaunchKernelGGL(k_pose_opt<kPoseThreads>, dim3(count), dim3(kPoseThreads),
-                           pose_lds_pad((const void*)k_pose_opt<kPoseThreads>), st, dp, (const PoseEdgeDev*)dE, nullptr,
+        hipLaunchKernelGGL((k_pose_opt<kPoseThreads, true>), dim3(count), dim3(kPoseThreads),
+                           pose_lds_pad((const void*)k_pose_opt<kPoseThreads, true>), st, dp, dE, nullptr,
                            (uint8_t*)(d + bProb + bEdge));
     ORB_HIP_CHECK(hipGetLastError());
     if (timing_) {
@@ -926,11 +925,13 @@
         chain->land_dev(ninliers, dNin, sizeof(int) * count);
         ORB_HIP_CHECK(hipEventRecord(lastUse_, st));
         lastUseSet_ = true;
+        lastStream_ = st;
         return 0;
     }
     ORB_HIP_CHECK(hipMemcpyAsync(hp, d, bProb, hipMemcpyDeviceToHost, st));
     ORB_HIP_CHECK(hipEventRecord(lastUse_, st));
     lastUseSet_ = true;
+    lastStream_ = st;
     ORB_HIP_CHECK(stream_wait(st));
     int rc = 0;
     for (int f = 0; f < count; f++) {
@@ -1022,10 +1023,10 @@
     if (count > 0)
     {
         if (count <= pose_wide_max())
-            hipLaunchKernelGGL(k_pose_opt<kPoseThreadsWide>, dim3(count), dim3(kPoseThreadsWide), 0, stream_, dp, (const PoseEdgeDev*)(d + bProb),
+            hipLaunchKernelGGL((k_pose_opt<kPoseThreadsWide, false>), dim3(count), dim3(kPoseThreadsWide), 0, stream_, dp, (PoseEdgeDev*)(d + bProb),
                                (double*)(d + bProb + bEdge), (uint8_t*)(d + bProb + bEdge + bErr));
         else
-            hipLaunchKernelGGL(k_pose_opt<kPoseThreads>, dim3(count), dim3(kPoseThreads), 0, stream_, dp, (const PoseEdgeDev*)(d + bProb),
+            hipLaunchKernelGGL((k_pose_opt<kPoseThreads, false>), dim3(count), dim3(kPoseThreads), 0, stream_, dp, (PoseEdgeDev*)(d + bProb),
                                (double*)(d + bProb + bEdge), (uint8_t*)(d + bProb + bEdge + bErr));
     }
     ORB_HIP_CHECK(hipGetLastError());
@@ -1033,6 +1034,7 @@
     if (ne) ORB_HIP_CHECK(hipMemcpyAsync(hOut, d + bProb + bEdge + bErr, ne, hipMemcpyDeviceToHost, stream_));
     ORB_HIP_CHECK(hipEventRecord(lastUse_, stream_));
     lastUseSet_ = true;
+    lastStream_ = stream_;
     ORB_HIP_CHECK(hipStreamSynchronize(stream_));
     for (int f = 0; f < count; f++) {
         const pose_problem& Q = P[f];
```

Result: slower. 44180 (-1.2%).
